# ZKTLabs/zkt-plonk

Measured on AMD Instinct MI355X. Metric: proofs/sec (withdraw, n=2^20), higher is better.
Workload: dtype u32 limbs (256-bit Montgomery); 1 GPU; full prove, WithdrawCircuit INPUTS=8 HEIGHT=64 Poseidon x5 (1019498 gates, 538 Poseidon gadgets), bn254, n=2^20, TABLE_SIZE=1024, 12 public inputs; parallelism=proofs sharded across 1 GPU(s), chained=True, distinct_witnesses=2, witness_on_device=True, table_cached=True, proof_bytes=802

## Files before the change

### include/zkt_plonk.h

```cpp
#ifndef ZKT_PLONK_H
#define ZKT_PLONK_H

#include <stddef.h>
#include <stdint.h>

#ifdef __cplusplus
extern "C" {
#endif

typedef struct zkt_ctx zkt_ctx;

enum {
    ZKT_CURVE_BN254 = 0,
    ZKT_CURVE_BLS12_381 = 1
};

enum {
    ZKT_OK = 0,
    ZKT_ERR_INVALID_ARGUMENT = 1,
    ZKT_ERR_INVALID_DOMAIN_SIZE = 2,
    ZKT_ERR_HIP = 3,
    ZKT_ERR_NO_DEVICE = 4,
    ZKT_ERR_TOO_MANY_COEFFICIENTS = 5,
    ZKT_ERR_ZERO_DENOMINATOR = 6,
// ... 22 lines not shown
    int (*all_gather)(void* user, const void* send, void* recv, size_t bytes, int on_device, void* hip_stream);
    int (*all_gather_async)(void* user, const void* d_send, void* d_recv, size_t bytes, void* hip_stream);
} zkt_comm_vtable;
#define ZKT_QUOTIENT_CHUNKS 4
int zkt_ctx_set_comm(zkt_ctx* ctx, const zkt_comm_vtable* comm);
int zkt_shard_range(size_t total, int rank, int world, size_t* lo, size_t* hi);
int zkt_comm_stats(zkt_ctx* ctx, uint64_t* calls, uint64_t* bytes_sent);
int zkt_comm_selftest(const zkt_comm_vtable* comm, const void* send, void* recv, size_t bytes);

int zkt_dev_alloc(zkt_ctx* ctx, size_t bytes, void** dptr);
int zkt_dev_free(zkt_ctx* ctx, void* dptr);
int zkt_dev_upload(zkt_ctx* ctx, void* dptr, const void* host, size_t bytes);
int zkt_dev_download(zkt_ctx* ctx, void* host, const void* dptr, size_t bytes);

int zkt_ntt(zkt_ctx* ctx, int log_n, int inverse, int coset, const uint64_t* in, size_t in_len, uint64_t* out);
int zkt_ntt_dev(zkt_ctx* ctx, int log_n, int inverse, int coset, const void* d_in, size_t in_len, void* d_out);
int zkt_ntt_class(zkt_ctx* ctx, int log_n, int log_big, int cls, const uint64_t* in, size_t in_len, uint64_t* out);
int zkt_domain_group_gen(zkt_ctx* ctx, int log_n, uint64_t* out4);

int zkt_srs_load(zkt_ctx* ctx, const uint64_t* g1_xy_mont, size_t count);
int zkt_srs_load_dev(zkt_ctx* ctx, const void* d_g1_xy_mont, size_t count);
int zkt_srs_generate(zkt_ctx* ctx, const uint64_t* tau_canonical4, size_t count);
int zkt_srs_download(zkt_ctx* ctx, size_t offset, size_t count, uint64_t* out_xy_mont);
int zkt_srs_generate_g2(int curve_id, const uint64_t* tau_canonical4, uint64_t* out_h, uint64_t* out_beta_h);
int zkt_srs_load_slice(zkt_ctx* ctx, const uint64_t* g1_xy_mont_slice, size_t offset, size_t count, size_t total);
int zkt_srs_generate_slice(zkt_ctx* ctx, const uint64_t* tau_canonical4, size_t offset, size_t count, size_t total);
int zkt_msm_g1(zkt_ctx* ctx, const uint64_t* scalars, size_t len, size_t base_offset, int scalars_montgomery,
               uint64_t* out_xy_mont, int* out_is_infinity);
int zkt_msm_g1_dev(zkt_ctx* ctx, const void* d_scalars, size_t len, size_t base_offset, int scalars_montgomery,
                   void* out_xy_mont_host);
int zkt_msm_enqueue_dev(zkt_ctx* ctx, const void* d_scalars, size_t len, size_t base_offset, int scalars_montgomery);
int zkt_msm_info(zkt_ctx* ctx, int* window_bits, int* windows, size_t* srs_count);

#define ZKT_MSM_BASES_MAX ((size_t)1 << 22)
int zkt_msm_g1_bases(zkt_ctx* ctx, const uint64_t* bases_xy_mont, const uint64_t* scalars, size_t n,
                     int scalars_montgomery, uint64_t* out_xy_mont, int* out_is_infinity);
int zkt_msm_g1_bases_dev(zkt_ctx* ctx, const void* d_bases_xy_mont, const void* d_scalars, size_t n,
                         int scalars_montgomery, uint64_t* out_xy_mont_host, int* out_is_infinity);
int zkt_msm_bases_info(zkt_ctx* ctx, size_t n, int scalars_montgomery, int* window_bits, int* windows);

#define ZKT_KZG_BATCH_MAX 32
int zkt_kzg_commit_batch(zkt_ctx* ctx, const uint64_t* const* coeffs, const size_t* lens, int k,
                         int scalars_montgomery, uint64_t* out_xy_mont, int* out_is_infinity);
int zkt_kzg_commit_batch_dev(zkt_ctx* ctx, const void* const* d_coeffs, const size_t* lens, int k,
                             int scalars_montgomery, uint64_t* out_xy_mont, int* out_is_infinity);
int zkt_kzg_open(zkt_ctx* ctx, const uint64_t* const* coeffs, const size_t* lens, int k,
                 const uint64_t* challenges_mont, const uint64_t* point_mont,
                 uint64_t* out_w_xy_mont, int* out_w_is_infinity, uint64_t* out_evals_mont);
int zkt_kzg_open_dev(zkt_ctx* ctx, const void* const* d_coeffs, const size_t* lens, int k,
                     const uint64_t* challenges_mont, const uint64_t* point_mont,
                     uint64_t* out_w_xy_mont, int* out_w_is_infinity, uint64_t* out_evals_mont);

int zkt_ctx_set_lagrange(zkt_ctx* ctx, int on);
int zkt_lagrange_info(zkt_ctx* ctx, int* log_n, size_t* bases);
int zkt_commit_evals_dev(zkt_ctx* ctx, const void* d_evals, const uint64_t* blinders, int k, int path, uint64_t* out_xy_mont,
                         int* out_is_infinity);

enum {
    ZKT_TRANSCRIPT_MERLIN = 0,
    ZKT_TRANSCRIPT_ETHEREUM = 1
};
typedef struct zkt_transcript zkt_transcript;
zkt_transcript* zkt_transcript_new(int kind, const char* label);
void zkt_transcript_free(zkt_transcript* t);
void zkt_transcript_append_u64(zkt_transcript* t, const char* label, uint64_t v);
void zkt_transcript_append_scalars(zkt_transcript* t, const char* label, const uint8_t* le32, size_t count, int single);
void zkt_transcript_append_commitment(zkt_transcript* t, const char* label, const uint8_t* x_le, const uint8_t* y_le,
                                      size_t fq_bytes, int is_infinity);
void zkt_transcript_challenge_scalar(zkt_transcript* t, const char* label, int fr_bits, uint8_t out_le32[32]);
void zkt_transcript_seed(zkt_transcript* t, uint64_t circuit_size, const uint8_t* xy_le, const uint8_t* is_infinity,
                         size_t fq_bytes);
int zkt_transcript_append_message(zkt_transcript* t, const char* label, const uint8_t* msg, size_t len);
int zkt_transcript_challenge_bytes(zkt_transcript* t, const char* label, uint8_t* out, size_t len);

typedef struct {
    void* user;
    void (*append_u64)(void* user, const char* label, uint64_t v);
    void (*append_scalars)(void* user, const char* label, const uint64_t* fr_mont, size_t count, int single);
    void (*append_commitment)(void* user, const char* label, const uint64_t* g1_xy_mont, int is_infinity);
    void (*challenge_scalar)(void* user, const char* label, uint64_t* fr_mont_out4);
} zkt_transcript_vtable;

int zkt_circuit_load(zkt_ctx* ctx, int log_n, const uint64_t* const* pk_polys, const size_t* pk_lens);

int zkt_circuit_setup(zkt_ctx* ctx, int log_n, const uint64_t* const* evals, const size_t* eval_lens, int evals_on_device,
                      uint64_t* out_commitments, int* out_is_infinity);

int zkt_circuit_sigma_dev(zkt_ctx* ctx, int log_n, const uint32_t* d_w_l, const uint32_t* d_w_r, const uint32_t* d_w_o,
                          size_t n_rows, size_t n_vars, void* const* d_sigma);
int zkt_circuit_setup_wiring(zkt_ctx* ctx, int log_n, const uint64_t* const* evals, const size_t* eval_lens,
                             int evals_on_device, const uint32_t* w_l, const uint32_t* w_r, const uint32_t* w_o,
                             size_t n_rows, size_t n_vars, int wiring_on_device,
                             uint64_t* out_commitments, int* out_is_infinity);

typedef struct {
    const uint64_t* a_evals;
    const uint64_t* b_evals;
    const uint64_t* c_evals;
    size_t n_rows;
    const uint64_t* table;
    size_t table_len;
    const size_t* pi_pos;
    const uint64_t* pi_vals;
    size_t n_pi;
    const uint64_t* blinders;
    int wires_on_device;
// ... 98 lines not shown

int zkt_verify_batch(int curve_id, const zkt_verify_inputs* ins, zkt_transcript* const* transcripts, size_t count,
                     const uint64_t* h_g2_mont, const uint64_t* beta_h_g2_mont, int* accepted);

#define ZKT_G1_DECOMPRESS_MAX ((size_t)1 << 22)
enum {
    ZKT_G1_VALID = 0,
    ZKT_G1_IDENTITY = 1,
    ZKT_G1_NOT_CANONICAL = 2,
    ZKT_G1_BOTH_FLAGS = 3,
    ZKT_G1_NOT_ON_CURVE = 4,
    ZKT_G1_NOT_IN_SUBGROUP = 5
};
int zkt_g1_decompress(zkt_ctx* ctx, const uint8_t* compressed, size_t n, uint64_t* out_xy_mont, uint8_t* out_status);
int zkt_g1_decompress_dev(zkt_ctx* ctx, const void* d_compressed, size_t n, void* d_out_xy_mont, void* d_out_status);

#define ZKT_VERIFY_BATCH_DEV_MAX (ZKT_MSM_BASES_MAX / 24)
int zkt_verify_batch_prepare_dev(zkt_ctx* ctx, const zkt_verify_inputs* ins, zkt_transcript* const* transcripts, size_t count,
                                 const uint64_t* h_g2_mont, const uint64_t* beta_h_g2_mont, uint64_t* out_ab,
                                 int* out_ab_is_infinity, uint64_t* out_rho);
int zkt_verify_batch_dev(zkt_ctx* ctx, const zkt_verify_inputs* ins, zkt_transcript* const* transcripts, size_t count,
                         const uint64_t* h_g2_mont, const uint64_t* beta_h_g2_mont, int* accepted);

int zkt_g1_msm_host(int curve_id, const uint64_t* points_xy_mont, const uint64_t* scalars, size_t n, int scalars_montgomery,
                    uint64_t* out_xy_mont, int* out_is_infinity);

int zkt_keyfile_committer_key(const char* path, int curve_id, size_t max_powers, uint64_t* out_xy_mont, size_t* n_powers);
int zkt_keyfile_prover_key(const char* path, int curve_id, uint64_t* const* out_polys, size_t* lens10);
int zkt_keyfile_verifier_key(const char* path, int curve_id, uint64_t* n, uint64_t* pi_roots_mont, size_t pi_cap, size_t* n_pi,
                             uint64_t* commitments_xy_mont, int* is_infinity10);
#define ZKT_EPK_VECTORS 17
int zkt_keyfile_extended_prover_key(const char* path, int curve_id, int which, uint64_t* out_mont, size_t cap, size_t* lens17);
int zkt_circuit_check_epk_file(zkt_ctx* ctx, const char* epk_path, int* first_mismatch_vector, size_t* mismatch_at);
int zkt_srs_load_file(zkt_ctx* ctx, const char* ck_path, size_t max_powers);
int zkt_circuit_load_file(zkt_ctx* ctx, const char* pk_path, int log_n);

int zkt_debug_params(zkt_ctx* ctx, int which, uint32_t* out, size_t out_words);
int zkt_host_field_op(int curve_id, int which, int op, const uint32_t* a, const uint32_t* b, uint32_t* out);
int zkt_g1_sum_host(int curve_id, const uint64_t* points_xy_mont, size_t count, uint64_t* out_xy_mont, int* out_is_infinity);
int zkt_debug_fr_mul(zkt_ctx* ctx, const uint64_t* a, const uint64_t* b, size_t n, uint64_t* out);
int zkt_debug_ntt_batch(zkt_ctx* ctx, int log_n, int inverse, int coset, int nb, const void* const* d_in, const size_t* in_len,
                        void* const* d_out);
int zkt_debug_ntt_split(zkt_ctx* ctx, int npass, const int* log_r);
int zkt_debug_pairing_selftest(int curve_id);
int zkt_debug_quotient(zkt_ctx* ctx, const uint64_t* challenges, const uint64_t* const* wit, const uint64_t* pi_pos,
                       const uint64_t* pi_vals, size_t n_pi, uint64_t* out);
int zkt_debug_grand_products(zkt_ctx* ctx, const uint64_t* challenges, const uint64_t* const* vectors, uint64_t* out_z1,
                             uint64_t* out_z2);
int zkt_debug_combine_split(zkt_ctx* ctx, const uint64_t* table, size_t table_len, const uint64_t* f, int fresh,
                            uint64_t* h1_out, uint64_t* h2_out);
int zkt_debug_commit_wires_dev(zkt_ctx* ctx, const void* d_variables, size_t n_vars, const uint32_t* d_w_l, const uint32_t* d_w_r,
                               const uint32_t* d_w_o, size_t n_rows, const uint64_t* blinders, int route, uint64_t* out_xy_mont,
                               int* out_is_infinity, int* out_route);
int zkt_debug_open_witness(zkt_ctx* ctx, const uint64_t* coeffs, size_t len, const uint64_t* z4, uint64_t* out);
int zkt_debug_eval_lincomb(zkt_ctx* ctx, const uint64_t* const* polys, const size_t* lens, int k, const uint64_t* points,
                           const uint64_t* scalars, uint64_t* out_evals, uint64_t* out_lincomb, size_t out_len);

enum zkt_fx_op {
    ZKT_FX_UNPACK = 0, ZKT_FX_UNPACK_SHIFT = 1, ZKT_FX_PACK = 2, ZKT_FX_FROM_ARK = 3, ZKT_FX_TO_ARK = 4,
    ZKT_FX_NORMALIZE = 5, ZKT_FX_ADD = 6, ZKT_FX_DBL = 7, ZKT_FX_SUB_1 = 8, ZKT_FX_SUB_2 = 9, ZKT_FX_SUB_4 = 10,
    ZKT_FX_SUB_8 = 11, ZKT_FX_SUB2_6 = 12, ZKT_FX_ADD_LAZY = 13, ZKT_FX_SUB_LAZY_3 = 14, ZKT_FX_SUB_LAZY_4 = 15,
    ZKT_FX_SUB_LAZY_5 = 16, ZKT_FX_SUB_LAZY_9 = 17, ZKT_FX_SUB_LAZY_WIDE_8_30 = 18, ZKT_FX_MUL = 19, ZKT_FX_MUL_INL = 20,
    ZKT_FX_SQR = 21, ZKT_FX_SQR_INL = 22, ZKT_FX_MUL2_INL = 23, ZKT_FX_MUL_SHOUP = 24 ,
    ZKT_FX_MUL_LOW = 25, ZKT_FX_REDUCE_SMALL = 26, ZKT_FX_REDUCE_LAZY = 27 ,
    ZKT_FX_COND_SUB_P = 28, ZKT_FX_CANON = 29, ZKT_FX_IS_ZERO_CANON = 30, ZKT_FX_IS_ZERO_LT2P = 31, ZKT_FX_OP_COUNT = 32
};
enum zkt_xyzz_op {
    ZKT_XYZZ_ADD_MIXED = 0, ZKT_XYZZ_ADD_MIXED_INL = 1, ZKT_XYZZ_ADD = 2, ZKT_XYZZ_ADD_INL = 3, ZKT_XYZZ_DOUBLE = 4,
    ZKT_XYZZ_DOUBLE_AFFINE = 5, ZKT_XYZZ_OP_COUNT = 6
};
int zkt_debug_fx_layout(int curve_id, int which, int* limbs, int* limb_bits, int* sh);
int zkt_host_fx_op(int curve_id, int which, int op, const uint32_t* in, size_t n, uint32_t* out);
int zkt_debug_fx_op(zkt_ctx* ctx, int which, int op, const uint32_t* in, size_t n, uint32_t* out);
int zkt_host_xyzz_op(int curve_id, int op, const uint32_t* in, size_t n, uint32_t* out);
int zkt_debug_xyzz_op(zkt_ctx* ctx, int op, const uint32_t* in, size_t n, uint32_t* out);

#ifdef __cplusplus
}
#endif
#endif
```

### shim/src/ffi.rs

```rust
use std::os::raw::{c_char, c_int, c_void};

#[repr(C)]
pub struct ZktCtx {
    _private: [u8; 0],
}

#[repr(C)]
pub struct ZktTranscriptVtable {
    pub user: *mut c_void,
    pub append_u64: extern "C" fn(*mut c_void, *const c_char, u64),
    pub append_scalars: extern "C" fn(*mut c_void, *const c_char, *const u64, usize, c_int),
    pub append_commitment: extern "C" fn(*mut c_void, *const c_char, *const u64, c_int),
    pub challenge_scalar: extern "C" fn(*mut c_void, *const c_char, *mut u64),
}

#[repr(C)]
pub struct ZktCommVtable {
    pub user: *mut c_void,
    pub rank: c_int,
    pub world: c_int,
    pub device_buffers: c_int,
    pub all_gather: extern "C" fn(*mut c_void, *const c_void, *mut c_void, usize, c_int, *mut c_void) -> c_int,
    pub all_gather_async: Option<extern "C" fn(*mut c_void, *const c_void, *mut c_void, usize, *mut c_void) -> c_int>,
}
// ... 16 lines not shown
    pub w_l: *const u32,
    pub w_r: *const u32,
    pub w_o: *const u32,
}

#[repr(C)]
pub struct ZktWitnessReport {
    pub satisfied: c_int,
    pub checked: c_int,
    pub n_arithmetic: u64,
    pub first_arithmetic: u64,
    pub residual: [u64; 4],
    pub n_lookup: u64,
    pub first_lookup: u64,
    pub n_wiring: u64,
    pub first_wiring_row: u64,
    pub first_wiring_column: c_int,
}

pub const ZKT_CHECK_WIRING: c_int = 1;
pub const ZKT_CHECK_NONE: u64 = u64::MAX;
pub const ZKT_VARIABLE_ZERO: u32 = 0xFFFF_FFFF;
pub const ZKT_CURVE_BN254: c_int = 0;
pub const ZKT_CURVE_BLS12_381: c_int = 1;
pub const ZKT_KZG_BATCH_MAX: usize = 32;

extern "C" {
    pub fn zkt_ctx_create(curve_id: c_int, device_id: c_int, out: *mut *mut ZktCtx) -> c_int;
    pub fn zkt_ctx_destroy(ctx: *mut ZktCtx);
    pub fn zkt_last_error(ctx: *const ZktCtx) -> *const c_char;
    pub fn zkt_ctx_set_comm(ctx: *mut ZktCtx, comm: *const ZktCommVtable) -> c_int;
    pub fn zkt_shard_range(total: usize, rank: c_int, world: c_int, lo: *mut usize, hi: *mut usize) -> c_int;
    pub fn zkt_ntt(ctx: *mut ZktCtx, log_n: c_int, inverse: c_int, coset: c_int, input: *const u64, in_len: usize,
                   out: *mut u64) -> c_int;
    pub fn zkt_srs_load(ctx: *mut ZktCtx, g1_xy_mont: *const u64, count: usize) -> c_int;
    pub fn zkt_srs_load_slice(ctx: *mut ZktCtx, g1_xy_mont: *const u64, offset: usize, count: usize, total: usize) -> c_int;
    pub fn zkt_srs_load_file(ctx: *mut ZktCtx, ck_path: *const c_char, max_powers: usize) -> c_int;
    pub fn zkt_msm_g1(ctx: *mut ZktCtx, scalars: *const u64, len: usize, base_offset: usize, scalars_montgomery: c_int,
                      out_xy_mont: *mut u64, out_is_infinity: *mut c_int) -> c_int;
    pub fn zkt_ctx_fork(ctx: *mut ZktCtx, out: *mut *mut ZktCtx) -> c_int;
    pub fn zkt_kzg_commit_batch(ctx: *mut ZktCtx, coeffs: *const *const u64, lens: *const usize, k: c_int,
                                scalars_montgomery: c_int, out_xy_mont: *mut u64, out_is_infinity: *mut c_int) -> c_int;
    pub fn zkt_kzg_commit_batch_dev(ctx: *mut ZktCtx, d_coeffs: *const *const c_void, lens: *const usize, k: c_int,
                                    scalars_montgomery: c_int, out_xy_mont: *mut u64, out_is_infinity: *mut c_int) -> c_int;
    pub fn zkt_kzg_open(ctx: *mut ZktCtx, coeffs: *const *const u64, lens: *const usize, k: c_int, challenges_mont: *const u64,
                        point_mont: *const u64, out_w_xy_mont: *mut u64, out_w_is_infinity: *mut c_int,
                        out_evals_mont: *mut u64) -> c_int;
    pub fn zkt_kzg_open_dev(ctx: *mut ZktCtx, d_coeffs: *const *const c_void, lens: *const usize, k: c_int,
                            challenges_mont: *const u64, point_mont: *const u64, out_w_xy_mont: *mut u64,
                            out_w_is_infinity: *mut c_int, out_evals_mont: *mut u64) -> c_int;
    pub fn zkt_commit_evals_dev(ctx: *mut ZktCtx, d_evals: *const c_void, blinders: *const u64, k: c_int, path: c_int,
                                out_xy_mont: *mut u64, out_is_infinity: *mut c_int) -> c_int;
    pub fn zkt_ctx_set_lagrange(ctx: *mut ZktCtx, on: c_int) -> c_int;
    pub fn zkt_lagrange_info(ctx: *mut ZktCtx, log_n: *mut c_int, bases: *mut usize) -> c_int;
    pub fn zkt_circuit_load(ctx: *mut ZktCtx, log_n: c_int, pk_polys: *const *const u64, pk_lens: *const usize) -> c_int;
    pub fn zkt_circuit_load_file(ctx: *mut ZktCtx, pk_path: *const c_char, log_n: c_int) -> c_int;
    pub fn zkt_keyfile_extended_prover_key(path: *const c_char, curve_id: c_int, which: c_int, out_mont: *mut u64, cap: usize,
                                           lens17: *mut usize) -> c_int;
    pub fn zkt_circuit_check_epk_file(ctx: *mut ZktCtx, epk_path: *const c_char, first_mismatch_vector: *mut c_int,
                                      mismatch_at: *mut usize) -> c_int;
    pub fn zkt_circuit_setup(ctx: *mut ZktCtx, log_n: c_int, evals: *const *const u64, eval_lens: *const usize,
                             evals_on_device: c_int, out_commitments: *mut u64, out_is_infinity: *mut c_int) -> c_int;
    pub fn zkt_circuit_sigma_dev(ctx: *mut ZktCtx, log_n: c_int, d_w_l: *const u32, d_w_r: *const u32, d_w_o: *const u32,
                                 n_rows: usize, n_vars: usize, d_sigma: *const *mut c_void) -> c_int;
    pub fn zkt_circuit_setup_wiring(ctx: *mut ZktCtx, log_n: c_int, evals: *const *const u64, eval_lens: *const usize,
                                    evals_on_device: c_int, w_l: *const u32, w_r: *const u32, w_o: *const u32, n_rows: usize,
                                    n_vars: usize, wiring_on_device: c_int, out_commitments: *mut u64,
                                    out_is_infinity: *mut c_int) -> c_int;
    pub fn zkt_prove_with(ctx: *mut ZktCtx, inputs: *const ZktProveInputs, transcript: *const ZktTranscriptVtable,
                          proof_out: *mut u8, proof_cap: usize, proof_len: *mut usize) -> c_int;
    pub fn zkt_prove_set_next(ctx: *mut ZktCtx, next: *const ZktProveInputs) -> c_int;
    pub fn zkt_circuit_check_witness(ctx: *mut ZktCtx, inputs: *const ZktProveInputs, flags: c_int,
                                     out: *mut ZktWitnessReport) -> c_int;
    pub fn zkt_g1_msm_host(curve_id: c_int, points_xy_mont: *const u64, scalars: *const u64, n: usize, scalars_montgomery: c_int,
                           out_xy_mont: *mut u64, out_is_infinity: *mut c_int) -> c_int;
    pub fn zkt_msm_g1_bases(ctx: *mut ZktCtx, bases_xy_mont: *const u64, scalars: *const u64, n: usize,
                            scalars_montgomery: c_int, out_xy_mont: *mut u64, out_is_infinity: *mut c_int) -> c_int;
    pub fn zkt_msm_g1_bases_dev(ctx: *mut ZktCtx, d_bases_xy_mont: *const c_void, d_scalars: *const c_void, n: usize,
                                scalars_montgomery: c_int, out_xy_mont_host: *mut u64, out_is_infinity: *mut c_int) -> c_int;
    pub fn zkt_verify(curve_id: c_int, inputs: *const ZktVerifyInputs, transcript: *mut c_void, h_g2_mont: *const u64,
                      beta_h_g2_mont: *const u64, accepted: *mut c_int) -> c_int;
    pub fn zkt_verify_batch(curve_id: c_int, inputs: *const ZktVerifyInputs, transcripts: *const *mut c_void, count: usize,
                            h_g2_mont: *const u64, beta_h_g2_mont: *const u64, accepted: *mut c_int) -> c_int;
    pub fn zkt_verify_batch_prepare_dev(ctx: *mut ZktCtx, inputs: *const ZktVerifyInputs, transcripts: *const *mut c_void, count: usize,
                                        h_g2_mont: *const u64, beta_h_g2_mont: *const u64, out_ab: *mut u64,
                                        out_ab_is_infinity: *mut c_int, out_rho: *mut u64) -> c_int;
    pub fn zkt_verify_batch_dev(ctx: *mut ZktCtx, inputs: *const ZktVerifyInputs, transcripts: *const *mut c_void, count: usize,
                                h_g2_mont: *const u64, beta_h_g2_mont: *const u64, accepted: *mut c_int) -> c_int;
    pub fn zkt_g1_decompress(ctx: *mut ZktCtx, compressed: *const u8, n: usize, out_xy_mont: *mut u64, out_status: *mut u8) -> c_int;
    pub fn zkt_g1_decompress_dev(ctx: *mut ZktCtx, d_compressed: *const c_void, n: usize, d_out_xy_mont: *mut c_void,
                                 d_out_status: *mut c_void) -> c_int;
    pub fn zkt_poseidon_load(ctx: *mut ZktCtx, params: *const ZktPoseidonParams, out: *mut *mut c_void) -> c_int;
    pub fn zkt_poseidon_free(ctx: *mut ZktCtx, params: *mut c_void);
    pub fn zkt_poseidon_hash_batch_dev(ctx: *mut ZktCtx, params: *const c_void, d_inputs: *const c_void, batch: usize,
                                       arity: c_int, d_out_hashes: *mut c_void, d_out_states: *mut c_void) -> c_int;
    pub fn zkt_poseidon_gadget_vars_per_hash(params: *const c_void) -> usize;
    pub fn zkt_poseidon_gadget_witness_dev(ctx: *mut ZktCtx, params: *const c_void, args: *const ZktPoseidonGadgetArgs) -> c_int;
    pub fn zkt_poseidon_gadget_check(ctx: *mut ZktCtx, params: *const c_void) -> c_int;
    pub fn zkt_merkle_path_vars_per_level(params: *const c_void) -> usize;
    pub fn zkt_poseidon_merkle_path_witness_dev(ctx: *mut ZktCtx, params: *const c_void, args: *const ZktMerklePathArgs) -> c_int;
    pub fn zkt_poseidon_merkle_path_validate(ctx: *mut ZktCtx, params: *const c_void, args: *const ZktMerklePathArgs) -> c_int;
    pub fn zkt_dev_alloc(ctx: *mut ZktCtx, bytes: usize, dptr: *mut *mut c_void) -> c_int;
    pub fn zkt_dev_free(ctx: *mut ZktCtx, dptr: *mut c_void) -> c_int;
    pub fn zkt_dev_upload(ctx: *mut ZktCtx, dptr: *mut c_void, host: *const c_void, bytes: usize) -> c_int;
}

// ... 61 lines not shown
```

### zkt-plonk_amd/_lib.py

```python
from __future__ import annotations

import ctypes
import os
import re
from typing import Optional

import numpy as np

_HERE = os.path.dirname(os.path.abspath(__file__))
_LIB = os.environ.get("ZKT_LIB_PATH") or os.path.join(_HERE, "libzkt_plonk_hip.so")
_HEADER = os.path.join(_HERE, "..", "include", "zkt_plonk.h")

MSM_BASES_MAX = 1 << 22
G1_DECOMPRESS_MAX = 1 << 22
VERIFY_BATCH_DEV_MAX = MSM_BASES_MAX // 24
KZG_BATCH_MAX = 32
CURVE_BN254 = 0
CURVE_BLS12_381 = 1
_CURVES = {"bn254": 0, "bls12_381": 1, "bls12-381": 1, 0: 0, 1: 1}

_lib = None


class ZktError(RuntimeError):
# ... 462 lines not shown
def host_fx_op(curve, which: int, op: int, records) -> np.ndarray:
    L_ = fx_layout(curve, which)[0]
    rec = _records(records, 4 * L_)
    out = np.zeros_like(rec)
    rc = lib().zkt_host_fx_op(curve_id(curve), which, op, _u32p(rec), rec.shape[0], _u32p(out))
    if rc:
        raise ZktError(rc, "zkt_host_fx_op")
    return out


def host_xyzz_op(curve, op: int, records) -> np.ndarray:
    w = 4 * fx_layout(curve, 1)[0] + 1
    rec = _records(records, 2 * w)
    out = np.zeros((rec.shape[0], w), dtype=np.uint32)
    rc = lib().zkt_host_xyzz_op(curve_id(curve), op, _u32p(rec), rec.shape[0], _u32p(out))
    if rc:
        raise ZktError(rc, "zkt_host_xyzz_op")
    return out


def srs_generate_g2(curve, tau: int):
    L = lib()
    cid = curve_id(curve)
    words = 8 if cid == CURVE_BN254 else 12
    t = np.array([(int(tau) >> (64 * i)) & 0xFFFFFFFFFFFFFFFF for i in range(4)], dtype=np.uint64)
    h = np.zeros(2 * words, dtype=np.uint64)
    bh = np.zeros(2 * words, dtype=np.uint64)
    P64 = ctypes.POINTER(ctypes.c_uint64)
    L.zkt_srs_generate_g2.argtypes = [ctypes.c_int, P64, P64, P64]
    rc = L.zkt_srs_generate_g2(cid, u64p(t), u64p(h), u64p(bh))
    if rc:
        raise ZktError(rc, "zkt_srs_generate_g2")
    return h, bh


def g1_msm_host(curve, points, scalars, montgomery: bool = True) -> tuple:
    L = lib()
    cid = curve_id(curve)
    words = 8 if cid == CURVE_BN254 else 12
    pts = np.ascontiguousarray(points, dtype=np.uint64).reshape(-1, words)
    sc = np.ascontiguousarray(scalars, dtype=np.uint64).reshape(-1, 4)
    assert pts.shape[0] == sc.shape[0]
    out = np.zeros(words, dtype=np.uint64)
    inf = ctypes.c_int(0)
    P64 = ctypes.POINTER(ctypes.c_uint64)
    L.zkt_g1_msm_host.argtypes = [ctypes.c_int, P64, P64, ctypes.c_size_t, ctypes.c_int, P64, ctypes.POINTER(ctypes.c_int)]
    rc = L.zkt_g1_msm_host(cid, u64p(pts) if pts.size else None, u64p(sc) if sc.size else None, pts.shape[0], int(montgomery),
                           u64p(out), ctypes.byref(inf))
    if rc:
        raise ZktError(rc, "zkt_g1_msm_host")
    return out, bool(inf.value)


class Transcript:

    def __init__(self, kind: str = "merlin", label: str = "ZKT Plonk", fr_bits: int = 254, fq_bytes: int = 32):
        self._L = lib()
        self._h = ctypes.c_void_p(self._L.zkt_transcript_new(0 if kind == "merlin" else 1, label.encode()))
        self.fr_bits = fr_bits
        self.fq_bytes = fq_bytes

    def __del__(self):
        if getattr(self, "_h", None):
            self._L.zkt_transcript_free(self._h)
            self._h = None

    @property
    def handle(self):
        return self._h

    def append_u64(self, label: str, v: int):
        self._L.zkt_transcript_append_u64(self._h, label.encode(), v)

    def append_scalar(self, label: str, v: int):
        self._L.zkt_transcript_append_scalars(self._h, label.encode(), int(v).to_bytes(32, "little"), 1, 1)

    def append_scalars(self, label: str, vals):
        vals = list(vals)
        self._L.zkt_transcript_append_scalars(self._h, label.encode(),
                                              b"".join(int(v).to_bytes(32, "little") for v in vals), len(vals), 0)

    def append_commitment(self, label: str, point):
        nb = self.fq_bytes
        if point is None:
            self._L.zkt_transcript_append_commitment(self._h, label.encode(), bytes(nb), bytes(nb), nb, 1)
        else:
            self._L.zkt_transcript_append_commitment(self._h, label.encode(), int(point[0]).to_bytes(nb, "little"),
                                                     int(point[1]).to_bytes(nb, "little"), nb, 0)

    def seed(self, circuit_size: int, points):
        nb = self.fq_bytes
        buf = b"".join(bytes(2 * nb) if p is None else int(p[0]).to_bytes(nb, "little") + int(p[1]).to_bytes(nb, "little")
                       for p in points)
        inf = bytes(1 if p is None else 0 for p in points)
        self._L.zkt_transcript_seed(self._h, circuit_size, buf, inf, nb)

    def challenge_scalar(self, label: str) -> int:
        out = (ctypes.c_uint8 * 32)()
        self._L.zkt_transcript_challenge_scalar(self._h, label.encode(), self.fr_bits, out)
        return int.from_bytes(bytes(out), "little")

    def append_message(self, label: bytes, msg: bytes):
        assert self._L.zkt_transcript_append_message(self._h, label, msg, len(msg)) == 0

    def challenge_bytes(self, label: bytes, n: int) -> bytes:
        out = (ctypes.c_uint8 * n)()
# ... 327 lines not shown
    @staticmethod
    def _kzg_lens(lens):
        return (ctypes.c_size_t * max(len(lens), 1))(*[int(n) for n in lens])

    def _kzg_points(self, out, inf, k):
        W = 2 * self.fq_limbs
        return [(out[j * W:(j + 1) * W].copy(), bool(inf[j])) for j in range(k)]

    def kzg_commit_batch(self, polys, montgomery: bool = True):
        arrs, ptrs, lens = self._kzg_polys(polys)
        k = len(arrs)
        out = np.zeros(max(k, 1) * 2 * self.fq_limbs, dtype=np.uint64)
        inf = (ctypes.c_int * max(k, 1))()
        self.check(self._L.zkt_kzg_commit_batch(self._h, ptrs, lens, k, int(montgomery), u64p(out), inf))
        return self._kzg_points(out, inf, k)

    def kzg_commit_batch_dev(self, d_ptrs, lens, montgomery: bool = True):
        k = len(lens)
        ptrs = (ctypes.c_void_p * max(k, 1))(*[int(d) if d else None for d in d_ptrs])
        out = np.zeros(max(k, 1) * 2 * self.fq_limbs, dtype=np.uint64)
        inf = (ctypes.c_int * max(k, 1))()
        self.check(self._L.zkt_kzg_commit_batch_dev(self._h, ptrs, self._kzg_lens(lens), k, int(montgomery), u64p(out), inf))
        return self._kzg_points(out, inf, k)

    def _kzg_open_call(self, fn, ptrs, lens, k, challenges, z, evals):
        ch = np.ascontiguousarray(challenges, dtype=np.uint64).reshape(-1, 4)
        if ch.shape[0] != k:
            raise ValueError("kzg_open: %d polynomials, %d challenges" % (k, ch.shape[0]))
        zz = np.ascontiguousarray(z, dtype=np.uint64).reshape(4)
        w = np.zeros(2 * self.fq_limbs, dtype=np.uint64)
        inf = ctypes.c_int(0)
        ev = np.zeros((max(k, 1), 4), dtype=np.uint64)
        self.check(fn(self._h, ptrs, lens, k, u64p(ch) if k else None, u64p(zz), u64p(w), ctypes.byref(inf),
                      u64p(ev) if evals else None))
        return (w, bool(inf.value)), (ev[:k].copy() if evals else None)

    def kzg_open(self, polys, challenges, z, evals: bool = True):
        arrs, ptrs, lens = self._kzg_polys(polys)
        return self._kzg_open_call(self._L.zkt_kzg_open, ptrs, lens, len(arrs), challenges, z, evals)

    def kzg_open_dev(self, d_ptrs, lens, challenges, z, evals: bool = True):
        k = len(lens)
        ptrs = (ctypes.c_void_p * max(k, 1))(*[int(d) if d else None for d in d_ptrs])
        return self._kzg_open_call(self._L.zkt_kzg_open_dev, ptrs, self._kzg_lens(lens), k, challenges, z, evals)

    def msm_info(self):
        c, w, n = ctypes.c_int(0), ctypes.c_int(0), ctypes.c_size_t(0)
        self.check(self._L.zkt_msm_info(self._h, ctypes.byref(c), ctypes.byref(w), ctypes.byref(n)))
        return dict(window_bits=c.value, windows=w.value, srs_count=n.value)

    def set_lagrange(self, on: bool = True):
        self._L.zkt_ctx_set_lagrange.argtypes = [ctypes.c_void_p, ctypes.c_int]
        self.check(self._L.zkt_ctx_set_lagrange(self._h, int(on)))

    def lagrange_info(self):
        self._L.zkt_lagrange_info.argtypes = [ctypes.c_void_p, ctypes.POINTER(ctypes.c_int), ctypes.POINTER(ctypes.c_size_t)]
        lg, nb = ctypes.c_int(0), ctypes.c_size_t(0)
        self.check(self._L.zkt_lagrange_info(self._h, ctypes.byref(lg), ctypes.byref(nb)))
        return dict(log_n=lg.value, bases=nb.value)

    def commit_evals_dev(self, d_evals: int, blinders=None, path: int = 1):
        self._L.zkt_commit_evals_dev.argtypes = [ctypes.c_void_p, ctypes.c_void_p, ctypes.POINTER(ctypes.c_uint64), ctypes.c_int,
                                                 ctypes.c_int, ctypes.POINTER(ctypes.c_uint64), ctypes.POINTER(ctypes.c_int)]
        k = 0 if blinders is None else int(np.asarray(blinders).reshape(-1, 4).shape[0])
        bl = np.ascontiguousarray(blinders, dtype=np.uint64).reshape(-1, 4) if k else None
        out = np.zeros(2 * self.fq_limbs, dtype=np.uint64)
        inf = ctypes.c_int(0)
        self.check(self._L.zkt_commit_evals_dev(self._h, ctypes.c_void_p(d_evals), u64p(bl) if k else None, k, int(path),
                                                u64p(out), ctypes.byref(inf)))
        return out, bool(inf.value)

    def circuit_load(self, log_n: int, pk_polys):
        arrs = [np.ascontiguousarray(p, dtype=np.uint64).reshape(-1, 4) for p in pk_polys]
        assert len(arrs) == 10
        ptrs = (ctypes.POINTER(ctypes.c_uint64) * 10)(*[u64p(a) if a.size else ctypes.POINTER(ctypes.c_uint64)() for a in arrs])
        lens = (ctypes.c_size_t * 10)(*[a.shape[0] for a in arrs])
        self.check(self._L.zkt_circuit_load(self._h, log_n, ptrs, lens))
        self.circuit_log_n = log_n

    def circuit_setup(self, log_n: int, evals):
        arrs = [np.ascontiguousarray(p, dtype=np.uint64).reshape(-1, 4) for p in evals]
        assert len(arrs) == 10
        ptrs = (ctypes.POINTER(ctypes.c_uint64) * 10)(*[u64p(a) if a.size else ctypes.POINTER(ctypes.c_uint64)() for a in arrs])
        lens = (ctypes.c_size_t * 10)(*[a.shape[0] for a in arrs])
        out = np.zeros((10, 2 * self.fq_limbs), dtype=np.uint64)
        inf = (ctypes.c_int * 10)()
        self.check(self._L.zkt_circuit_setup(self._h, log_n, ptrs, lens, 0, u64p(out), inf))
        self.circuit_log_n = log_n
        return out, np.array([bool(x) for x in inf])

    def circuit_sigma(self, log_n: int, d_w_l: int, d_w_r: int, d_w_o: int, n_rows: int, n_vars: int, d_sigma=None):
        n = 1 << log_n if 0 <= log_n <= 25 else 0
        own = d_sigma is None
        if own:
            d_sigma = [self.alloc(max(n, 1) * 32) for _ in range(3)]
        try:
            ptrs = (ctypes.c_void_p * 3)(*d_sigma)
            self.check(self._L.zkt_circuit_sigma_dev(self._h, log_n, ctypes.c_void_p(d_w_l), ctypes.c_void_p(d_w_r),
                                                     ctypes.c_void_p(d_w_o), n_rows, n_vars, ptrs))
            return [self.download(p, (n, 4)) for p in d_sigma] if own else None
        finally:
            if own:
                for p in d_sigma:
                    self.free(p)

    def circuit_setup_wiring(self, log_n: int, evals, w_l, w_r, w_o, n_vars: int, n_rows: int = None):
# ... 96 lines not shown
        lens = (ctypes.c_size_t * len(in_len))(*in_len)
        self.check(self._L.zkt_debug_ntt_batch(self._h, log_n, int(inverse), int(coset), nb, ins, lens, outs))

    def debug_ntt_split(self, log_r=()):
        lr = (ctypes.c_int * max(len(log_r), 3))(*log_r)
        self.check(self._L.zkt_debug_ntt_split(self._h, len(log_r), lr))

    def debug_fr_mul(self, a: np.ndarray, b: np.ndarray) -> np.ndarray:
        a = np.ascontiguousarray(a, dtype=np.uint64).reshape(-1, 4)
        b = np.ascontiguousarray(b, dtype=np.uint64).reshape(-1, 4)
        out = np.empty_like(a)
        self.check(self._L.zkt_debug_fr_mul(self._h, u64p(a), u64p(b), a.shape[0], u64p(out)))
        return out

    def debug_fx_op(self, which: int, op: int, records) -> np.ndarray:
        L_ = fx_layout(self.curve, which)[0]
        rec = _records(records, 4 * L_)
        out = np.zeros_like(rec)
        self.check(self._L.zkt_debug_fx_op(self._h, which, op, _u32p(rec), rec.shape[0], _u32p(out)))
        return out

    def debug_xyzz_op(self, op: int, records) -> np.ndarray:
        w = 4 * fx_layout(self.curve, 1)[0] + 1
        rec = _records(records, 2 * w)
        out = np.zeros((rec.shape[0], w), dtype=np.uint32)
        self.check(self._L.zkt_debug_xyzz_op(self._h, op, _u32p(rec), rec.shape[0], _u32p(out)))
        return out

    def debug_grand_products(self, n: int, challenges, vectors):
        ch = np.ascontiguousarray(challenges, dtype=np.uint64).reshape(4, 4)
        keep = [np.ascontiguousarray(w, dtype=np.uint64).reshape(n, 4) for w in vectors]
        assert len(keep) == 7
        ptrs = (ctypes.c_void_p * 7)(*[w.ctypes.data for w in keep])
        z1, z2 = np.empty((n, 4), dtype=np.uint64), np.empty((n, 4), dtype=np.uint64)
        self._L.zkt_debug_grand_products.argtypes = [ctypes.c_void_p, ctypes.POINTER(ctypes.c_uint64), ctypes.POINTER(ctypes.c_void_p),
                                                     ctypes.POINTER(ctypes.c_uint64), ctypes.POINTER(ctypes.c_uint64)]
        self.check(self._L.zkt_debug_grand_products(self._h, u64p(ch), ptrs, u64p(z1), u64p(z2)))
        return z1, z2

    def debug_combine_split(self, table, f, fresh: bool = True):
        t = np.ascontiguousarray(table, dtype=np.uint64).reshape(-1, 4)
        ff = np.ascontiguousarray(f, dtype=np.uint64).reshape(-1, 4)
        if self.circuit_log_n is None or ff.shape[0] != 1 << self.circuit_log_n:
            raise ValueError("f must hold the n elements of a circuit loaded through this Context")
        n = ff.shape[0]
        h1, h2 = np.empty((n, 4), dtype=np.uint64), np.empty((n, 4), dtype=np.uint64)
        P64 = ctypes.POINTER(ctypes.c_uint64)
        self._L.zkt_debug_combine_split.argtypes = [ctypes.c_void_p, P64, ctypes.c_size_t, P64, ctypes.c_int, P64, P64]
        self.check(self._L.zkt_debug_combine_split(self._h, u64p(t) if t.shape[0] else None, t.shape[0], u64p(ff),
                                                   1 if fresh else 0, u64p(h1), u64p(h2)))
        return h1, h2

    def debug_commit_wires_dev(self, d_variables: int, n_vars: int, d_w_l: int, d_w_r: int, d_w_o: int, n_rows: int, blinders,
                               route: int = 1):
        bl = np.ascontiguousarray(blinders, dtype=np.uint64).reshape(6, 4)
        out = np.zeros((3, 2 * self.fq_limbs), dtype=np.uint64)
        inf = (ctypes.c_int * 3)()
        took = (ctypes.c_int * 3)()
        self._L.zkt_debug_commit_wires_dev.argtypes = [ctypes.c_void_p, ctypes.c_void_p, ctypes.c_size_t, ctypes.c_void_p,
                                                       ctypes.c_void_p, ctypes.c_void_p, ctypes.c_size_t,
                                                       ctypes.POINTER(ctypes.c_uint64), ctypes.c_int,
                                                       ctypes.POINTER(ctypes.c_uint64), ctypes.POINTER(ctypes.c_int),
                                                       ctypes.POINTER(ctypes.c_int)]
        self.check(self._L.zkt_debug_commit_wires_dev(self._h, ctypes.c_void_p(d_variables), n_vars, ctypes.c_void_p(d_w_l),
                                                      ctypes.c_void_p(d_w_r), ctypes.c_void_p(d_w_o), n_rows, u64p(bl), int(route),
                                                      u64p(out), inf, took))
        return out, [bool(x) for x in inf], [int(x) for x in took]

    def check_epk_file(self, path: str):
        self._L.zkt_circuit_check_epk_file.argtypes = [ctypes.c_void_p, ctypes.c_char_p, ctypes.POINTER(ctypes.c_int),
                                                       ctypes.POINTER(ctypes.c_size_t)]
        vec, at = ctypes.c_int(0), ctypes.c_size_t(0)
        self.check(self._L.zkt_circuit_check_epk_file(self._h, path.encode(), ctypes.byref(vec), ctypes.byref(at)))
        if vec.value < 0:
            return None
        return vec.value, (-1 if at.value == ctypes.c_size_t(-1).value else at.value)

    def debug_eval_lincomb(self, polys, points, scalars, out_len: int):
        keep = [np.ascontiguousarray(p_, dtype=np.uint64).reshape(-1, 4) for p_ in polys]
        k = len(keep)
        P64 = ctypes.POINTER(ctypes.c_uint64)
        ptrs = (P64 * k)(*[u64p(a) for a in keep])
        lens = (ctypes.c_size_t * k)(*[a.shape[0] for a in keep])
        pts = np.ascontiguousarray(points, dtype=np.uint64).reshape(k, 4)
        scs = np.ascontiguousarray(scalars, dtype=np.uint64).reshape(k, 4)
        ev = np.empty((k, 4), dtype=np.uint64)
        lc = np.empty((out_len, 4), dtype=np.uint64)
        self._L.zkt_debug_eval_lincomb.argtypes = [ctypes.c_void_p, ctypes.POINTER(P64), ctypes.POINTER(ctypes.c_size_t), ctypes.c_int,
                                                   P64, P64, P64, P64, ctypes.c_size_t]
        self.check(self._L.zkt_debug_eval_lincomb(self._h, ptrs, lens, k, u64p(pts), u64p(scs), u64p(ev), u64p(lc), out_len))
        return ev, lc

    def debug_open_witness(self, coeffs, z) -> np.ndarray:
        p_ = np.ascontiguousarray(coeffs, dtype=np.uint64).reshape(-1, 4)
        zz = np.ascontiguousarray(z, dtype=np.uint64).reshape(4)
        out = np.empty((p_.shape[0] - 1, 4), dtype=np.uint64)
        self._L.zkt_debug_open_witness.argtypes = [ctypes.c_void_p, ctypes.POINTER(ctypes.c_uint64), ctypes.c_size_t,
                                                   ctypes.POINTER(ctypes.c_uint64), ctypes.POINTER(ctypes.c_uint64)]
        self.check(self._L.zkt_debug_open_witness(self._h, u64p(p_), p_.shape[0], u64p(zz), u64p(out)))
        return out

    def debug_quotient(self, n: int, challenges, wit, pi_pos=(), pi_vals=None) -> np.ndarray:
        ch = np.ascontiguousarray(challenges, dtype=np.uint64).reshape(5, 4)
        keep = [None if w is None else np.ascontiguousarray(w, dtype=np.uint64).reshape(4 * n, 4) for w in wit]
        assert len(keep) == 9
        ptrs = (ctypes.c_void_p * 9)(*[None if w is None else w.ctypes.data for w in keep])
        pos = np.ascontiguousarray(list(pi_pos), dtype=np.uint64)
        vals = np.ascontiguousarray(pi_vals if len(pos) else np.zeros((0, 4)), dtype=np.uint64).reshape(-1, 4)
        out = np.empty((4 * n, 4), dtype=np.uint64)
        self.check(self._L.zkt_debug_quotient(self._h, u64p(ch), ptrs, u64p(pos) if len(pos) else None,
                                              u64p(vals) if len(pos) else None, len(pos), u64p(out)))
# ... 2 lines not shown
```

### zkt-plonk_amd/csrc/capi.hip

```cpp
#include "ctx.hpp"

#include <cstdlib>
#include "hostinv.hpp"
#include "ec.hpp"
#include "hostec.hpp"
#include "fx_test.hpp"
#include "msm.hpp"

#include <cstring>

namespace zkt {

const char* exp_env(const char* name) {
#ifdef ZKT_EXPERIMENTS
    return getenv(name);
#else
    (void)name;
    return nullptr;
#endif
}

int set_err(zkt_ctx* c, int code, const std::string& msg) {
    if (c) c->err = msg;
    return code;
// ... 149 lines not shown

template <class P>
static int dump_params(uint32_t* out, size_t words) {
    const int N = P::N;
    if (words < (size_t)(3 * N + 1)) return -1;
    for (int i = 0; i < N; ++i) out[i] = P::mod(i);
    out[N] = P::INV;
    for (int i = 0; i < N; ++i) out[N + 1 + i] = P::one(i);
    for (int i = 0; i < N; ++i) out[2 * N + 1 + i] = P::r2(i);
    return N;
}

}

using namespace zkt;

extern "C" {

const char* zkt_version(void) { return "zkt-plonk_amd 0.1 (gfx950)"; }

int zkt_ctx_create(int curve_id, int device_id, zkt_ctx** out) {
    if (!out) return ZKT_ERR_INVALID_ARGUMENT;
    *out = nullptr;
    if (curve_id != ZKT_CURVE_BN254 && curve_id != ZKT_CURVE_BLS12_381) return ZKT_ERR_INVALID_ARGUMENT;
    int count = 0;
    if (hipGetDeviceCount(&count) != hipSuccess || count <= 0 || device_id < 0 || device_id >= count)
        return ZKT_ERR_NO_DEVICE;
    if (hipSetDevice(device_id) != hipSuccess) return ZKT_ERR_NO_DEVICE;
    zkt_ctx* c = new zkt_ctx();
    c->batch_off = exp_env("ZKT_MSM_NO_BATCH") != nullptr;
    c->aux_off = exp_env("ZKT_NO_AUX") != nullptr;
    c->curve = curve_id;
    c->device = device_id;
    if (hipStreamCreateWithFlags(&c->stream, hipStreamNonBlocking) != hipSuccess) {
        delete c;
        return ZKT_ERR_HIP;
    }
    c->own_stream = true;
    *out = c;
    return ZKT_OK;
}

int zkt_ctx_fork(zkt_ctx* parent, zkt_ctx** out) {
    if (!parent || !out) return ZKT_ERR_INVALID_ARGUMENT;
    *out = nullptr;
    if (parent->sharded()) return set_err(parent, ZKT_ERR_INVALID_ARGUMENT, "zkt_ctx_fork: not for a context with a communicator");
    if (parent->zombie) return set_err(parent, ZKT_ERR_INVALID_ARGUMENT, "zkt_ctx_fork: the context has been destroyed");
    zkt_ctx* root = parent->parent ? parent->parent : parent;
    zkt_ctx* c = nullptr;
    int rc = zkt_ctx_create(parent->curve, parent->device, &c);
    if (rc) return rc;
    (void)hipStreamSynchronize(parent->stream);
    c->lagrange_off = parent->lagrange_off;
    c->batch_off = parent->batch_off;
    c->aux_off = parent->aux_off;
    c->ntt_plans = parent->ntt_plans;
    c->parent = root;
    root->forks.fetch_add(1);
    if ((rc = msm_fork(c, parent)) || (rc = circuit_fork(c, parent))) {
        parent->err = c->err;
        zkt_ctx_destroy(c);
        return rc;
    }
    *out = c;
    return ZKT_OK;
}

void zkt_ctx_destroy(zkt_ctx* c) {
    if (!c) return;
    (void)hipSetDevice(c->device);
    (void)hipStreamSynchronize(c->stream);
    if (c->forks.load() > 0) {
        c->zombie = true;
        return;
    }
    zkt_ctx* const owner = c->parent;
    circuit_release(c);
    msm_release(c);
    prof_resolve(c);
    for (hipEvent_t e : c->event_pool) (void)hipEventDestroy(e);
    c->event_pool.clear();
    c->ntt_plans.clear();
    c->msm.reset();
    c->msmb.reset();
    c->kzg.reset();
    c->circuit.reset();
    if (c->comm.pinned) (void)hipHostFree(c->comm.pinned);
    for (void* p : c->owned) (void)hipFree(p);
    c->owned.clear();
    if (c->own_stream && c->stream) (void)hipStreamDestroy(c->stream);
    delete c;
    if (owner && owner->forks.fetch_sub(1) == 1 && owner->zombie) {
        owner->zombie = false;
        zkt_ctx_destroy(owner);
    }
}

int zkt_ctx_set_comm(zkt_ctx* c, const zkt_comm_vtable* comm) {
    if (!c) return ZKT_ERR_INVALID_ARGUMENT;
    if (int rf = refuse_if_forked(c, "zkt_ctx_set_comm")) return rf;
    if (c->parent && comm && comm->world > 1) return set_err(c, ZKT_ERR_INVALID_ARGUMENT, "a forked context cannot take a communicator");
    if (comm && comm->world > 1) {
        const int w = comm->world;
        if ((w != 2 && w != 4 && w != 8) || comm->rank < 0 || comm->rank >= w || !comm->all_gather)
            return set_err(c, ZKT_ERR_INVALID_ARGUMENT, "communicator: world must be 1, 2, 4 or 8 with a valid rank and callback");
    }
// ... 372 lines not shown
```

### zkt-plonk_amd/csrc/check.hip

```cpp
#include "poly.hpp"

#include <algorithm>
#include <cstring>
#include <numeric>
#include <vector>

namespace zkt {

constexpr int CK_THREADS = 256;
constexpr int CK_ROWS_PER_THREAD = 4;
constexpr unsigned CK_MAX_BLOCKS = 2048;
constexpr uint32_t CK_NONE32 = 0xFFFFFFFFu;
enum { CK_N_ARITH = 0, CK_FIRST_ARITH, CK_N_LOOKUP, CK_FIRST_LOOKUP, CK_N_WIRING, CK_FIRST_WIRING, CK_BAD_INDEX, CK_PAD, CK_RESIDUAL,
       CK_WORDS = CK_RESIDUAL + 4 };

struct CheckArgs {
    const void *q_m, *q_l, *q_r, *q_o, *q_c, *q_lookup;
    const void *a, *b, *c;
    const void* variables;
    const uint32_t *w_l, *w_r, *w_o;
    uint32_t n, n_rows, n_vars;
    const uint32_t* pi_pos;
    const void* pi_vals;
    uint32_t n_pi;
// ... 94 lines not shown
                while (lo < hi) {
                    const uint32_t mid = lo + (hi - lo) / 2;
                    if (ck_cmp<P>(fe_load<P>(tab + mid), f) < 0) lo = mid + 1;
                    else hi = mid;
                }
                if (lo >= q.table_len || ck_cmp<P>(fe_load<P>(tab + lo), f) != 0) {
                    ++n_lookup;
                    first_lookup = i < first_lookup ? i : first_lookup;
                }
            }
        }
    }
    ck_block_reduce(n_arith, first_arith, q.status + CK_N_ARITH, q.status + CK_FIRST_ARITH, sh_cnt, sh_min);
    ck_block_reduce(n_lookup, first_lookup, q.status + CK_N_LOOKUP, q.status + CK_FIRST_LOOKUP, sh_cnt, sh_min);
}

template <class P, bool VARS>
__global__ void k_check_residual(CheckArgs q) {
    if (blockIdx.x || threadIdx.x) return;
    const unsigned long long first = q.status[CK_FIRST_ARITH];
    if (first >= q.n) return;
    const uint32_t i = (uint32_t)first;
    const Fe<P> t = ck_gate<P>(q, i, ck_wire<P, VARS>(q, q.a, q.w_l, i), ck_wire<P, VARS>(q, q.b, q.w_r, i),
                               ck_wire<P, VARS>(q, q.c, q.w_o, i));
#pragma unroll
    for (int k = 0; k < 4; ++k) q.status[CK_RESIDUAL + k] = (unsigned long long)t.v[2 * k] | ((unsigned long long)t.v[2 * k + 1] << 32);
}

template <class P>
__global__ __launch_bounds__(CK_THREADS) void k_check_sigma(const Fe<P>* m0, const Fe<P>* m1, const Fe<P>* m2, const Fe<P>* k0,
                                                            const Fe<P>* k1, const Fe<P>* k2, uint32_t n, unsigned long long* status) {
    __shared__ uint32_t sh_cnt[CK_THREADS / 64], sh_min[CK_THREADS / 64];
    const Fe<P>* const made[3] = {m0, m1, m2};
    const Fe<P>* const key[3] = {k0, k1, k2};
    uint32_t cnt = 0, first = CK_NONE32;
    const uint32_t stride = gridDim.x * CK_THREADS;
#pragma unroll 1
    for (uint32_t g = blockIdx.x * CK_THREADS + threadIdx.x; g < n; g += stride) {
#pragma unroll
        for (uint32_t col = 0; col < 3; ++col) {
            if (!fe_eq<P>(fe_load<P>(made[col] + g), fe_load<P>(key[col] + g))) {
                ++cnt;
                const uint32_t p = 3 * g + col;
                first = p < first ? p : first;
            }
        }
    }
    ck_block_reduce(cnt, first, status + CK_N_WIRING, status + CK_FIRST_WIRING, sh_cnt, sh_min);
}

static unsigned ck_blocks(size_t n) {
    const size_t per = (size_t)CK_THREADS * CK_ROWS_PER_THREAD;
    return (unsigned)std::min<size_t>(std::max<size_t>((n + per - 1) / per, 1), CK_MAX_BLOCKS);
}

template <class P>
static int witness_check_t(zkt_ctx* c, const WitnessCheckKeys& K, const zkt_prove_inputs& in, int flags, zkt_witness_report* out) {
    using F = Fe<P>;
    static_assert(sizeof(F) == 32, "scalar field element = 8 words");
    const int log_n = K.log_n;
    const size_t n = (size_t)1 << log_n;
    const bool vars = in.a_evals == nullptr;
    const bool wiring = (flags & ZKT_CHECK_WIRING) != 0;
    const bool on_device = in.wires_on_device != 0;
    const size_t rows = in.n_rows, n_pi = in.n_pi, tl = in.table_len;

    std::vector<F> sorted(tl);
    if (tl) {
        const F* t = reinterpret_cast<const F*>(in.table);
        std::vector<uint32_t> order(tl);
        std::iota(order.begin(), order.end(), 0u);
        std::sort(order.begin(), order.end(), [&](uint32_t x, uint32_t y) { return ck_cmp<P>(t[x], t[y]) < 0; });
        for (size_t i = 0; i < tl; ++i) sorted[i] = t[order[i]];
        for (size_t i = 1; i < tl; ++i)
            if (ck_cmp<P>(sorted[i - 1], sorted[i]) == 0)
                return set_err(c, ZKT_ERR_INVALID_ARGUMENT, "lookup table holds a repeated value");
    }
    std::vector<uint32_t> pos(n_pi);
    std::vector<F> pvals(n_pi);
    if (n_pi) {
        std::vector<uint32_t> order(n_pi);
        std::iota(order.begin(), order.end(), 0u);
        std::stable_sort(order.begin(), order.end(), [&](uint32_t x, uint32_t y) { return in.pi_pos[x] < in.pi_pos[y]; });
        for (size_t i = 0; i < n_pi; ++i) {
            pos[i] = (uint32_t)in.pi_pos[order[i]];
            pvals[i] = reinterpret_cast<const F*>(in.pi_vals)[order[i]];
        }
    }

    size_t at = 0;
    auto take = [&](size_t bytes) {
        const size_t here = at;
        at += (bytes + 255) / 256 * 256;
        return here;
    };
    const size_t o_status = take(CK_WORDS * 8);
    size_t o_sel[5];
    for (size_t& o : o_sel) o = take(n * 32);
    const size_t o_pos = take(n_pi * 4), o_pvals = take(n_pi * 32), o_table = take(tl * 32);
    size_t o_wit[3] = {}, o_vars = 0, o_idx[3] = {};
    if (!on_device) {
        if (vars) {
            o_vars = take(in.n_vars * 32);
            for (size_t& o : o_idx) o = take(rows * 4);
        } else {
            for (size_t& o : o_wit) o = take(rows * 32);
// ... 7 lines not shown
    int rc = ensure_buffer(c, &c->check_scratch, &c->check_scratch_bytes, at);
    if (rc) return rc;
    char* const base = (char*)c->check_scratch;
    unsigned long long* const d_status = (unsigned long long*)(base + o_status);

    unsigned long long h_status[CK_WORDS] = {};
    struct Drain {
        zkt_ctx* c;
        bool done = false;
        ~Drain() {
            if (!done) (void)hipStreamSynchronize(c->stream);
        }
    } drain{c};
    h_status[CK_FIRST_ARITH] = h_status[CK_FIRST_LOOKUP] = h_status[CK_FIRST_WIRING] = ~0ull;
    ZKT_HIP(c, hipMemcpyAsync(d_status, h_status, sizeof(h_status), hipMemcpyHostToDevice, c->stream));
    if (n_pi) {
        ZKT_HIP(c, hipMemcpyAsync(base + o_pos, pos.data(), n_pi * 4, hipMemcpyHostToDevice, c->stream));
        ZKT_HIP(c, hipMemcpyAsync(base + o_pvals, pvals.data(), n_pi * 32, hipMemcpyHostToDevice, c->stream));
    }
    if (tl) ZKT_HIP(c, hipMemcpyAsync(base + o_table, sorted.data(), tl * 32, hipMemcpyHostToDevice, c->stream));

    CheckArgs q{};
    q.a = in.a_evals; q.b = in.b_evals; q.c = in.c_evals;
    q.variables = in.variables;
    q.w_l = in.w_l; q.w_r = in.w_r; q.w_o = in.w_o;
    if (!on_device) {
        if (vars) {
            if (in.n_vars) ZKT_HIP(c, hipMemcpyAsync(base + o_vars, in.variables, in.n_vars * 32, hipMemcpyHostToDevice, c->stream));
            q.variables = base + o_vars;
            const uint32_t* src[3] = {in.w_l, in.w_r, in.w_o};
            const uint32_t** dst[3] = {&q.w_l, &q.w_r, &q.w_o};
            for (int k = 0; k < 3; ++k) {
                if (rows) ZKT_HIP(c, hipMemcpyAsync(base + o_idx[k], src[k], rows * 4, hipMemcpyHostToDevice, c->stream));
                *dst[k] = (const uint32_t*)(base + o_idx[k]);
            }
        } else {
            const uint64_t* src[3] = {in.a_evals, in.b_evals, in.c_evals};
            const void** dst[3] = {&q.a, &q.b, &q.c};
            for (int k = 0; k < 3; ++k) {
                if (rows) ZKT_HIP(c, hipMemcpyAsync(base + o_wit[k], src[k], rows * 32, hipMemcpyHostToDevice, c->stream));
                *dst[k] = base + o_wit[k];
            }
        }
    }
    q.q_m = base + o_sel[0]; q.q_l = base + o_sel[1]; q.q_r = base + o_sel[2]; q.q_o = base + o_sel[3]; q.q_c = base + o_sel[4];
    q.q_lookup = K.q_lookup_ev;
    q.n = (uint32_t)n; q.n_rows = (uint32_t)rows; q.n_vars = (uint32_t)in.n_vars;
    q.pi_pos = (const uint32_t*)(base + o_pos); q.pi_vals = base + o_pvals; q.n_pi = (uint32_t)n_pi;
    q.table = base + o_table; q.table_len = (uint32_t)tl;
    q.status = d_status;

    {
        ProfScope prof(c, "check_witness");
        const void* ins[5];
        void* outs[5];
        size_t lens[5];
        for (int k = 0; k < 5; ++k) {
            ins[k] = K.pk[k];
            lens[k] = n;
            outs[k] = base + o_sel[k];
        }
        static_assert(NTT_MAX_BATCH >= 4, "four selectors in one batch");
        if ((rc = ntt_run_batch(c, log_n, 0, 0, 4, ins, lens, outs))) return rc;
        if ((rc = ntt_run_batch(c, log_n, 0, 0, 1, ins + 4, lens + 4, outs + 4))) return rc;

        if (vars) {
            hipLaunchKernelGGL((k_check_gates<P, true>), dim3(ck_blocks(n)), dim3(CK_THREADS), 0, c->stream, q);
            hipLaunchKernelGGL((k_check_residual<P, true>), dim3(1), dim3(64), 0, c->stream, q);
        } else {
            hipLaunchKernelGGL((k_check_gates<P, false>), dim3(ck_blocks(n)), dim3(CK_THREADS), 0, c->stream, q);
            hipLaunchKernelGGL((k_check_residual<P, false>), dim3(1), dim3(64), 0, c->stream, q);
        }
        ZKT_HIP(c, hipGetLastError());
        if (wiring) {
            void* made[3] = {base + o_made[0], base + o_made[1], base + o_made[2]};
            if ((rc = sigma_enqueue(c, log_n, q.w_l, q.w_r, q.w_o, rows, in.n_vars, made, base + o_sigma,
                                    (uint32_t*)(d_status + CK_BAD_INDEX))))
                return rc;
            hipLaunchKernelGGL(k_check_sigma<P>, dim3(ck_blocks(n)), dim3(CK_THREADS), 0, c->stream, (const F*)made[0], (const F*)made[1],
                               (const F*)made[2], (const F*)K.sigma_ev[0], (const F*)K.sigma_ev[1], (const F*)K.sigma_ev[2], (uint32_t)n,
                               d_status);
            ZKT_HIP(c, hipGetLastError());
        }
    }
    ZKT_HIP(c, hipMemcpyAsync(h_status, d_status, sizeof(h_status), hipMemcpyDeviceToHost, c->stream));
    ZKT_HIP(c, hipStreamSynchronize(c->stream));
    drain.done = true;
    if (h_status[CK_BAD_INDEX])
        return set_err(c, ZKT_ERR_INVALID_ARGUMENT, "wire index outside the variable map: every entry must be < n_vars or ZKT_VARIABLE_ZERO");

    zkt_witness_report r;
    memset(&r, 0, sizeof(r));
    r.checked = 3 | (wiring ? 4 : 0);
    r.n_arithmetic = h_status[CK_N_ARITH];
    r.first_arithmetic = h_status[CK_FIRST_ARITH];
    for (int k = 0; k < 4; ++k) r.residual[k] = h_status[CK_RESIDUAL + k];
    r.n_lookup = h_status[CK_N_LOOKUP];
    r.first_lookup = h_status[CK_FIRST_LOOKUP];
    r.n_wiring = h_status[CK_N_WIRING];
    r.first_wiring_row = ZKT_CHECK_NONE;
    r.first_wiring_column = -1;
    if (h_status[CK_FIRST_WIRING] != ~0ull) {
        r.first_wiring_row = h_status[CK_FIRST_WIRING] / 3;
        r.first_wiring_column = (int)(h_status[CK_FIRST_WIRING] % 3);
    }
    r.satisfied = !r.n_arithmetic && !r.n_lookup && !r.n_wiring;
    memcpy(out, &r, sizeof(r));
    return ZKT_OK;
}

int witness_check(zkt_ctx* c, const WitnessCheckKeys& keys, const zkt_prove_inputs& in, int flags, zkt_witness_report* out) {
    return c->curve == ZKT_CURVE_BN254 ? witness_check_t<Bn254Fr>(c, keys, in, flags, out)
                                       : witness_check_t<Bls381Fr>(c, keys, in, flags, out);
}

}
```

### zkt-plonk_amd/csrc/ctx.hpp

```cpp
#pragma once
#include <hip/hip_runtime.h>
#include <stdint.h>
#include <stddef.h>
#include <map>
#include <string>
#include <tuple>
#include <vector>
#include <memory>
#include <atomic>

#include "../../include/zkt_plonk.h"
#include "fp.hpp"
#include "fx.hpp"
#include "ntt.hpp"

namespace zkt {

struct MsmState;
struct MsmBasesState;
struct KzgState;
struct CircuitState;

}

struct zkt_ctx {
    int curve = 0;
    int device = 0;
    hipStream_t stream = nullptr;
    bool own_stream = false;
    std::string err;

    std::map<std::tuple<int, int, int, int>, std::shared_ptr<void>> ntt_plans;
    int ntt_split_npass = 0;
    int ntt_split_log_r[3] = {0, 0, 0};
    void* ntt_scratch = nullptr;
    size_t ntt_scratch_bytes = 0;
    void* io_a = nullptr;
    size_t io_a_bytes = 0;
    void* io_b = nullptr;
    size_t io_b_bytes = 0;
    void* check_scratch = nullptr;
    size_t check_scratch_bytes = 0;
    void* verify_scratch = nullptr;
    size_t verify_scratch_bytes = 0;

    int prof_on = 0;
    struct ProfSlot {
        std::vector<std::pair<hipEvent_t, hipEvent_t>> pending;
        double total_ms = 0.0;
        uint64_t calls = 0;
        uint64_t launches = 0;
    };
    std::map<std::string, ProfSlot> prof;
    std::vector<hipEvent_t> event_pool;

    struct Comm {
        zkt_comm_vtable vt{};
        void* pinned = nullptr;
        size_t pinned_bytes = 0;
        uint64_t calls = 0, bytes = 0;
    } comm;
    bool sharded() const { return comm.vt.world > 1; }

    std::shared_ptr<zkt::MsmState> msm;
    std::shared_ptr<zkt::MsmBasesState> msmb;
    std::shared_ptr<zkt::KzgState> kzg;
    uint64_t msm_epoch = 0;
    uint64_t srs_generation = 0;
    zkt_ctx* parent = nullptr;
    std::atomic<int> forks{0};
    bool zombie = false;
    bool aux_off = false;
    bool batch_off = false;
    bool lagrange_off = false;
    std::shared_ptr<zkt::CircuitState> circuit;
    std::vector<void*> owned;
};

namespace zkt {

const char* exp_env(const char* name);

int set_err(zkt_ctx* c, int code, const std::string& msg);
int refuse_if_forked(zkt_ctx* c, const char* what);
int hip_fail(zkt_ctx* c, hipError_t e, const char* what);

#define ZKT_HIP(c, call)                                        \
    do {                                                        \
        hipError_t _e = (call);                                 \
        if (_e != hipSuccess) return zkt::hip_fail((c), _e, #call); \
    } while (0)

struct ProfScope {
    zkt_ctx* c;
    zkt_ctx::ProfSlot* slot = nullptr;
    hipEvent_t e0 = nullptr, e1 = nullptr;
    hipStream_t stream = nullptr;
    uint64_t count = 1;
    ProfScope(zkt_ctx* ctx, const char* name, hipStream_t on_stream = nullptr, uint64_t units = 1);
    ~ProfScope();
};

int comm_all_gather_host(zkt_ctx* c, const void* send, void* recv, size_t bytes);
int comm_all_gather_dev(zkt_ctx* c, const void* d_send, void* d_recv, size_t bytes);
bool comm_async_available(const zkt_ctx* c);
int comm_all_gather_async(zkt_ctx* c, const void* d_send, void* d_recv, size_t bytes, hipStream_t st);

int ensure_buffer(zkt_ctx* c, void** p, size_t* cur, size_t bytes);
struct DevBuf {
    void* p = nullptr;
    size_t bytes = 0;
};
inline int grow(zkt_ctx* c, DevBuf& b, size_t bytes) { return ensure_buffer(c, &b.p, &b.bytes, bytes); }
int dev_alloc(zkt_ctx* c, void** p, size_t bytes);
void dev_free(zkt_ctx* c, void* p);

template <class P>
Fe<P> root_of_unity(int log_n);
int ntt_run(zkt_ctx* c, int log_n, int inverse, int coset, const void* d_in, size_t in_len, void* d_out);
int ntt_run_batch(zkt_ctx* c, int log_n, int inverse, int coset, int nb, const void* const* d_in, const size_t* in_len,
                  void* const* d_out);
int ntt_class_code(int log_big, int cls);
int ntt_force_split(zkt_ctx* c, int npass, const int* log_r);
int ntt_run_class(zkt_ctx* c, int log_n, int log_big, int cls, const void* d_in, size_t in_len, void* d_out, void* d_fold);

void circuit_release(zkt_ctx* c);
int circuit_fork(zkt_ctx* child, const zkt_ctx* parent);
// ... 3 lines not shown
```

### zkt-plonk_amd/csrc/lagrange.hip

```cpp
#include "ctx.hpp"
#include "ec.hpp"
#include "hostec.hpp"
#include "msm.hpp"

#include <algorithm>
#include <cstdio>
#include <cstdlib>
#include <vector>

namespace zkt {

template <class C>
__global__ void k_lag_init(const Affine<typename C::Fq>* table, Xyzz<typename C::Fq>* A, size_t n) {
    using Q = typename C::Fq;
    const size_t j = (size_t)blockIdx.x * blockDim.x + threadIdx.x;
    if (j >= n) return;
    Affine<Q> p = aff_load<Q>(table + j);
    if (!aff_is_inf<Q>(p)) {
        p.x = fx_to_ark<Q>(fx_unpack<Q>(p.x));
        p.y = fx_to_ark<Q>(fx_unpack<Q>(p.y));
    }
    xyzz_store<Q>(A + j, xyzz_from_affine<Q>(p));
}

template <class R>
__global__ void k_lag_twiddles(Fe<R>* tw, size_t half, Fe<R> w) {
    const size_t j = (size_t)blockIdx.x * blockDim.x + threadIdx.x;
    if (j >= half) return;
    fe_store<R>(tw + j, fe_from_mont<R>(fe_pow_u64<R>(w, (uint64_t)j)));
}

template <class Q>
ZKT_HD Xyzz<Q> xyzz_neg(const Xyzz<Q>& p) {
    Xyzz<Q> r = p;
    r.y = fe_neg<Q>(p.y);
    return r;
}

template <class Q, class R>
ZKT_D Xyzz<Q> xyzz_scalar_mul(const Xyzz<Q>& P, const Fe<R>& k) {
    constexpr int N = R::N;
    uint32_t h[N + 1];
    uint32_t carry = 0;
#pragma unroll
    for (int i = 0; i < N; ++i) {
        const uint64_t t = (uint64_t)k.v[i] * 3u + carry;
        h[i] = (uint32_t)t;
        carry = (uint32_t)(t >> 32);
    }
    h[N] = carry;
    const Xyzz<Q> Pn = xyzz_neg<Q>(P);
    Xyzz<Q> acc = xyzz_identity<Q>();
#pragma unroll 1
    for (int li = N; li >= 0; --li) {
        const uint32_t hw = h[li], kw = li < N ? k.v[li] : 0u;
        if (li == N && hw == 0u) continue;
#pragma unroll 1
        for (int b = (li == N ? 1 : 31); b >= (li == 0 ? 1 : 0); --b) {
            acc = xyzz_double<Q>(acc);
// ... 202 lines not shown
        const Affine<Q> hi = wire_load_base<Q>(pre + i);
        if (!aff_is_inf<Q>(hi)) acc = xyzz_add_mixed<Q>(acc, hi);
        if (i) {
            Affine<Q> lo = wire_load_base<Q>(pre + i - 1);
            if (!aff_is_inf<Q>(lo)) {
                lo.y = fe_neg<Q>(lo.y);
                acc = xyzz_add_mixed<Q>(acc, lo);
            }
        }
    }
    if (xyzz_is_identity<Q>(acc)) atomicOr(bad, 1u);
    aff_store<Q>(out + j, xyzz_to_affine<Q>(acc));
}
template <class C>
__global__ void k_wire_blinder_points(const Affine<typename C::Fq>* pre, size_t n, size_t cnt, Affine<typename C::Fq>* out) {
    using Q = typename C::Fq;
    if (threadIdx.x < 2) aff_store<Q>(out + cnt + threadIdx.x, wire_load_base<Q>(pre + n + threadIdx.x));
}

ZKT_HD uint64_t wire_mix(uint64_t x) {
    x ^= x >> 30; x *= 0xbf58476d1ce4e5b9ull;
    x ^= x >> 27; x *= 0x94d049bb133111ebull;
    return x ^ (x >> 31);
}
__global__ __launch_bounds__(256) void k_wire_digest(const uint32_t* w0, const uint32_t* w1, const uint32_t* w2, size_t rows,
                                                     unsigned long long* out) {
    __shared__ unsigned long long sh[2][256];
    unsigned long long a = 0, b = 0;
    const size_t total = 3 * rows;
    for (size_t e = (size_t)blockIdx.x * blockDim.x + threadIdx.x; e < total; e += (size_t)gridDim.x * blockDim.x) {
        const size_t k = e / rows, i = e - k * rows;
        const uint32_t v = (k == 0 ? w0 : k == 1 ? w1 : w2)[i];
        const uint64_t x = ((uint64_t)e << 32) | v;
        a += wire_mix(x + 0x9e3779b97f4a7c15ull);
        b += wire_mix(~x * 0xd6e8feb86659fd93ull);
    }
    sh[0][threadIdx.x] = a;
    sh[1][threadIdx.x] = b;
    __syncthreads();
    for (unsigned s = 128; s; s >>= 1) {
        if (threadIdx.x < s) {
            sh[0][threadIdx.x] += sh[0][threadIdx.x + s];
            sh[1][threadIdx.x] += sh[1][threadIdx.x + s];
        }
        __syncthreads();
    }
    if (threadIdx.x == 0) {
        atomicAdd(out, sh[0][0]);
        atomicAdd(out + 1, sh[1][0]);
    }
}

template <class P>
__global__ void k_wire_scalars(const Fe<P>* vars, const uint32_t* u, size_t cnt, const Fe<P>* bl, Fe<P> ninv, Fe<P>* out) {
    const size_t j = (size_t)blockIdx.x * blockDim.x + threadIdx.x;
    if (j >= cnt + 2) return;
    fe_store<P>(out + j, j < cnt ? fe_mul<P>(fe_load<P>(vars + u[j]), ninv) : fe_load<P>(bl + (j - cnt)));
}

void wire_bases_drop(zkt_ctx* c) {
    if (!c->msm) return;
    WireBases& wb = c->msm->wb;
    if (!wb.borrowed && wb.built) {
        (void)hipStreamSynchronize(c->stream);
        for (int k = 0; k < 3; ++k) {
            dev_free(c, wb.table[k]);
            dev_free(c, wb.u[k]);
        }
    }
    wb = WireBases{};
}

static int wire_digest_enqueue(zkt_ctx* c, const uint32_t* const* d_idx, size_t n_rows) {
    MsmState& st = *c->msm;
    if (!st.wb_dig)
        if (int rc = dev_alloc(c, (void**)&st.wb_dig, 16)) return rc;
    if (!st.wb_pin) ZKT_HIP(c, hipHostMalloc((void**)&st.wb_pin, 64));
    ZKT_HIP(c, hipMemsetAsync(st.wb_dig, 0, 16, c->stream));
    if (n_rows) {
        const size_t blocks = std::min<size_t>((3 * n_rows + 2047) / 2048, 4096);
        hipLaunchKernelGGL(k_wire_digest, dim3((unsigned)blocks), dim3(256), 0, c->stream, d_idx[0], d_idx[1], d_idx[2], n_rows,
                           (unsigned long long*)st.wb_dig);
        ZKT_HIP(c, hipGetLastError());
    }
    ZKT_HIP(c, hipMemcpyAsync(st.wb_pin, st.wb_dig, 16, hipMemcpyDeviceToHost, c->stream));
    return ZKT_OK;
}

template <class C>
static int wire_bases_build_wire(zkt_ctx* c, int log_n, int k, const uint32_t* d_idx, size_t n_rows, size_t n_vars, double frac) {
    using Q = typename C::Fq;
    MsmState& st = *c->msm;
    WireBases& wb = st.wb;
    const size_t n = (size_t)1 << log_n;
    void *d_cnt = nullptr, *d_start = nullptr, *d_grouped = nullptr, *d_ofs = nullptr, *d_bad = nullptr, *table = nullptr, *d_u = nullptr;
    auto done = [&](bool keep) {
        dev_free(c, d_cnt); dev_free(c, d_start); dev_free(c, d_grouped); dev_free(c, d_ofs); dev_free(c, d_bad);
        if (!keep) { dev_free(c, table); dev_free(c, d_u); }
        (void)hipGetLastError();
        return ZKT_OK;
    };
    if (dev_alloc(c, &d_cnt, (n_vars + 1) * 4)) return done(false);
    ZKT_HIP(c, hipMemsetAsync(d_cnt, 0, (n_vars + 1) * 4, c->stream));
    const unsigned rb = (unsigned)((n_rows + 255) / 256);
    if (n_rows) hipLaunchKernelGGL(k_wire_count, dim3(rb), dim3(256), 0, c->stream, d_idx, n_rows, (uint32_t)n_vars, (uint32_t*)d_cnt);
    std::vector<uint32_t> cnt(n_vars + 1);
    if (hipMemcpyAsync(cnt.data(), d_cnt, n_vars * 4, hipMemcpyDeviceToHost, c->stream) != hipSuccess ||
        hipStreamSynchronize(c->stream) != hipSuccess)
        return done(false);
    std::vector<uint32_t> u, ofs;
    uint32_t at = 0;
    for (size_t v = 0; v < n_vars; ++v) {
        const uint32_t m = cnt[v];
        cnt[v] = at;
        if (m) {
            u.push_back((uint32_t)v);
            ofs.push_back(at);
            at += m;
        }
    }
    ofs.push_back(at);
    const size_t d = u.size();
    if ((double)d >= frac * (double)n_rows || (uint64_t)st.plan.W * (d + 2) >= ((uint64_t)1 << 31)) return done(false);
    if (dev_alloc(c, &table, (size_t)st.plan.W * (d + 2) * sizeof(Affine<Q>)) || dev_alloc(c, &d_u, (d + 1) * 4) ||
        dev_alloc(c, &d_start, (n_vars + 1) * 4) || dev_alloc(c, &d_grouped, ((size_t)at + 1) * 4) || dev_alloc(c, &d_ofs, (d + 1) * 4) ||
        dev_alloc(c, &d_bad, 4))
        return done(false);
    ZKT_HIP(c, hipMemcpyAsync(d_start, cnt.data(), n_vars * 4, hipMemcpyHostToDevice, c->stream));
    ZKT_HIP(c, hipMemcpyAsync(d_u, u.data(), d * 4, hipMemcpyHostToDevice, c->stream));
    ZKT_HIP(c, hipMemcpyAsync(d_ofs, ofs.data(), (d + 1) * 4, hipMemcpyHostToDevice, c->stream));
    ZKT_HIP(c, hipMemsetAsync(d_cnt, 0, (n_vars + 1) * 4, c->stream));
    ZKT_HIP(c, hipMemsetAsync(d_bad, 0, 4, c->stream));
    if (n_rows)
        hipLaunchKernelGGL(k_wire_fill, dim3(rb), dim3(256), 0, c->stream, d_idx, n_rows, (uint32_t)n_vars, (const uint32_t*)d_start,
                           (uint32_t*)d_cnt, (uint32_t*)d_grouped);
    if (d)
        hipLaunchKernelGGL(k_wire_sum<C>, dim3((unsigned)((d + 63) / 64)), dim3(64), 0, c->stream, (const Affine<Q>*)st.table2,
                           (const uint32_t*)d_grouped, (const uint32_t*)d_ofs, d, (Affine<Q>*)table, (uint32_t*)d_bad);
    hipLaunchKernelGGL(k_wire_blinder_points<C>, dim3(1), dim3(64), 0, c->stream, (const Affine<Q>*)st.table2, n, d, (Affine<Q>*)table);
    uint32_t bad = 0;
    if (hipGetLastError() != hipSuccess || hipMemcpyAsync(&bad, d_bad, 4, hipMemcpyDeviceToHost, c->stream) != hipSuccess ||
        hipStreamSynchronize(c->stream) != hipSuccess)
        return done(false);
    if (bad || msm_table_finish(c, table, d + 2)) return done(false);
    wb.table[k] = table;
    wb.u[k] = (uint32_t*)d_u;
    wb.cnt[k] = d;
    wb.use[k] = true;
    return done(true);
}

int wire_bases_prepare(zkt_ctx* c, int log_n, const uint32_t* const* d_idx, size_t n_rows, size_t n_vars) {
    if (!c->msm) return ZKT_OK;
    MsmState& st = *c->msm;
    WireBases& wb = st.wb;
    const size_t n = (size_t)1 << log_n;
    const bool possible = lagrange_ready(c, log_n) && !c->sharded() && !c->lagrange_off && st.count2 >= n + 2 && n_rows <= n &&
                          n_vars <= 0xFFFFFFFEull && !(exp_env("ZKT_WIRE_BASES") && atoi(exp_env("ZKT_WIRE_BASES")) == 0);
    const bool same = wb.built && !wb.stale && wb.w[0] == d_idx[0] && wb.w[1] == d_idx[1] && wb.w[2] == d_idx[2] &&
                      wb.n_rows == n_rows && wb.n_vars == n_vars && wb.log_n == log_n && wb.srs_generation == c->srs_generation;
    if (possible && same) return ZKT_OK;
    if (wb.built && !wb.borrowed && c->forks.load() > 0) {
        if (!same || !possible) wb.stale = true;
        return ZKT_OK;
    }
    wire_bases_drop(c);
    if (!possible) return ZKT_OK;
    double frac = WIRE_BASES_MAX_FRAC;
    if (const char* e = exp_env("ZKT_WIRE_BASES_FRAC")) frac = atof(e);
    hipEvent_t e0 = nullptr, e1 = nullptr;
    const bool trace = exp_env("ZKT_HOST_TRACE") != nullptr;
    if (trace) {
        (void)hipEventCreate(&e0); (void)hipEventCreate(&e1);
        (void)hipEventRecord(e0, c->stream);
    }
    for (int k = 0; k < 3; ++k) {
        const int rc = c->curve == ZKT_CURVE_BN254 ? wire_bases_build_wire<Bn254Curve>(c, log_n, k, d_idx[k], n_rows, n_vars, frac)
                                                    : wire_bases_build_wire<Bls381Curve>(c, log_n, k, d_idx[k], n_rows, n_vars, frac);
        if (rc) return rc;
    }
    if (int rc = wire_digest_enqueue(c, d_idx, n_rows)) return rc;
    ZKT_HIP(c, hipStreamSynchronize(c->stream));
    if (trace) {
        float ms = 0;
        (void)hipEventRecord(e1, c->stream); (void)hipEventSynchronize(e1); (void)hipEventElapsedTime(&ms, e0, e1);
        fprintf(stderr, "[zkt host] wire base tables: %zu / %zu / %zu distinct of %zu rows (0 = dense), %.1f ms\n",
                wb.use[0] ? wb.cnt[0] : 0, wb.use[1] ? wb.cnt[1] : 0, wb.use[2] ? wb.cnt[2] : 0, n_rows, ms);
        (void)hipEventDestroy(e0); (void)hipEventDestroy(e1);
    }
    wb.digest[0] = st.wb_pin[0];
    wb.digest[1] = st.wb_pin[1];
    for (int k = 0; k < 3; ++k) wb.w[k] = d_idx[k];
    wb.n_rows = n_rows; wb.n_vars = n_vars; wb.log_n = log_n; wb.srs_generation = c->srs_generation;
    wb.built = true;
    ++c->msm_epoch;
    return ZKT_OK;
}

bool wire_bases_use(const zkt_ctx* c, int k) {
    return c->msm && c->msm->wb.built && !c->msm->wb.stale && c->msm->wb.use[k];
}
int wire_bases_digest(zkt_ctx* c, const uint32_t* const* d_idx, size_t n_rows) { return wire_digest_enqueue(c, d_idx, n_rows); }
int wire_bases_lens(zkt_ctx* c, const uint32_t* d_lens) {
    ZKT_HIP(c, hipMemcpyAsync(c->msm->wb_pin + 2, d_lens, 12, hipMemcpyDeviceToHost, c->stream));
    return ZKT_OK;
}

template <class C>
static int wire_scalars_t(zkt_ctx* c, int k, const void* d_vars, const void* d_bl, size_t n, const void** out, size_t* len) {
    using R = typename C::Fr;
    MsmState& st = *c->msm;
    const size_t cnt = st.wb.cnt[k];
    if (int rc = grow(c, st.wb_scalars[k], (cnt + 2) * sizeof(Fe<R>))) return rc;
    Fe<R> nn = fe_zero<R>();
    nn.v[0] = (uint32_t)(n & 0xffffffffu);
    nn.v[1] = (uint32_t)((uint64_t)n >> 32);
    const Fe<R> ninv = fe_inv_host<R>(fe_to_mont<R>(nn));
    hipLaunchKernelGGL(k_wire_scalars<R>, dim3((unsigned)((cnt + 2 + 255) / 256)), dim3(256), 0, c->stream, (const Fe<R>*)d_vars,
                       (const uint32_t*)st.wb.u[k], cnt, (const Fe<R>*)d_bl, ninv, (Fe<R>*)st.wb_scalars[k].p);
    ZKT_HIP(c, hipGetLastError());
    *out = st.wb_scalars[k].p;
    *len = cnt + 2;
    return ZKT_OK;
}
int wire_bases_scalars(zkt_ctx* c, int k, const void* d_vars, const void* d_blinders, size_t n, const void** out, size_t* len) {
    if (c->curve == ZKT_CURVE_BN254) return wire_scalars_t<Bn254Curve>(c, k, d_vars, d_blinders, n, out, len);
    return wire_scalars_t<Bls381Curve>(c, k, d_vars, d_blinders, n, out, len);
}

bool wire_bases_check(zkt_ctx* c, int k, size_t n) {
    MsmState& st = *c->msm;
    if (st.wb_pin[0] != st.wb.digest[0] || st.wb_pin[1] != st.wb.digest[1]) {
        st.wb.stale = true;
        return false;
    }
    return ((const uint32_t*)(st.wb_pin + 2))[k] == (uint32_t)n;
}

}
```

### zkt-plonk_amd/csrc/msm.hpp

```cpp
#pragma once
#include "ctx.hpp"

#include <functional>

namespace zkt {

constexpr int MSM_CHUNK_MIN = 16;
constexpr int MSM_R2_BLOCKS = 1;
constexpr int MSM_MAX_Y = 24;

struct MsmWindows {
    int W;
    uint8_t width[40];
    uint16_t start[40];
};

struct MsmPlan {
    MsmWindows win{};
    int W = 0, c = 0;
    int dig = 0;
    uint32_t Bw = 0;
    uint32_t keys = 0;
    uint32_t lb = 8;
    int lcols = 8;
    bool packed = false;
    uint32_t nb1 = 0;
    uint32_t l1_scalars = 0;
    uint32_t l2_items = 0;
};

constexpr int MSM_BATCH = 3;
struct MsmBatch {
    const void* scalars[MSM_BATCH];
    uint64_t n[MSM_BATCH];
    uint64_t base_off[MSM_BATCH];
    const void* table[MSM_BATCH];
    uint64_t tcount[MSM_BATCH];
    uint32_t* heavy[MSM_BATCH];
    uint32_t* params[MSM_BATCH];
    uint32_t* offsets[MSM_BATCH];
    void* pieces[MSM_BATCH];
    uint64_t s_bin_offs, s_bin_aux, s_bin, s_tile_desc, s_cnt, s_pairs_bytes, s_vals, s_chunk;
    uint32_t vb_stride;
};

constexpr int MSM_TAIL_BATCH = 6;
struct MsmTailBatch {
    const uint32_t* offsets[MSM_TAIL_BATCH];
    const uint32_t* params[MSM_TAIL_BATCH];
    const void* pieces[MSM_TAIL_BATCH];
    void* buckets[MSM_TAIL_BATCH];
    uint32_t* heavy[MSM_TAIL_BATCH];
    void* rowcol[MSM_TAIL_BATCH];
    void* partials[MSM_TAIL_BATCH];
};

constexpr int MSM_HEAVY = 32;
constexpr int MSM_HEAVY_BLOCKS = 64;

struct WireBases {
    void* table[3] = {};
    uint32_t* u[3] = {};
    size_t cnt[3] = {};
    bool use[3] = {};
    bool built = false;
    bool borrowed = false;
    bool stale = false;
    const void* w[3] = {};
    size_t n_rows = 0, n_vars = 0;
    int log_n = -1;
    uint64_t srs_generation = 0;
    uint64_t digest[2] = {};
};
constexpr int MSM_TBL_WIRE = 2;

struct MsmState {
    size_t count = 0;
    size_t slice_off = 0, total = 0;
    MsmPlan plan;
    uint32_t* heavy[11] = {};
    void* table = nullptr;
    void* table2 = nullptr;
    size_t count2 = 0;
    int lag_log_n = -1;
    bool lag_failed = false;
    bool table_borrowed = false, table2_borrowed = false;
    WireBases wb;
    DevBuf wb_scalars[3];
    uint64_t* wb_dig = nullptr;
    uint64_t* wb_pin = nullptr;
    const void* tbl_table(int tbl) const { return tbl >= MSM_TBL_WIRE ? wb.table[tbl - MSM_TBL_WIRE] : tbl ? table2 : table; }
    size_t tbl_count(int tbl) const { return tbl >= MSM_TBL_WIRE ? wb.cnt[tbl - MSM_TBL_WIRE] + 2 : tbl ? count2 : count; }
    uint32_t* params[11] = {};
    uint32_t* vals2 = nullptr;
    void* pairs = nullptr;
    uint32_t* bin_offs = nullptr;
    uint32_t* bin_aux = nullptr;
    uint32_t *bin_start = nullptr, *tile_start = nullptr;
    void* tile_desc = nullptr;
    uint32_t *cnt2 = nullptr, *pos2 = nullptr;
    uint32_t* chunk_bucket = nullptr;
    MsmBatch strides{};
    uint32_t* offsets[11] = {};
    void* pieces[11] = {};
    static constexpr int SLOTS = 11;
    void* buckets[SLOTS] = {};
    void* rowcol[SLOTS] = {};
    void* host_result[SLOTS] = {};
    void* host_result_dev[SLOTS] = {};
    size_t acc_lds = 0;
    size_t acc_threads = 196608;
    hipStream_t side = nullptr;
    hipEvent_t ev_main[SLOTS] = {}, ev_done[SLOTS] = {};
    bool pending[SLOTS] = {};
    bool defer_tails = false;
    int tail_wait[SLOTS] = {};
    int n_tail_wait = 0;
    ~MsmState() {
        for (int i = 0; i < SLOTS; ++i) {
            if (host_result[i]) (void)hipHostFree(host_result[i]);
            if (ev_main[i]) (void)hipEventDestroy(ev_main[i]);
            if (ev_done[i]) (void)hipEventDestroy(ev_done[i]);
        }
        if (side) (void)hipStreamDestroy(side);
        if (wb_pin) (void)hipHostFree(wb_pin);
    }
};

struct MsmBasesState {
    DevBuf bases;
    DevBuf scalars;
    DevBuf vals, pairs, bin_offs, bin_aux, bin_start, tile_start, tile_desc, cnt2, pos2, chunk_bucket;
    DevBuf offsets, heavy, params, pieces, buckets, rowcol;
    void* partials = nullptr;
    void* partials_dev = nullptr;
    size_t acc_lds = 0, acc_threads = 0;
    ~MsmBasesState() {
        if (partials) (void)hipHostFree(partials);
    }
};

constexpr size_t MSM_DEFER_MAX = ((size_t)1 << 16) + 64;
constexpr size_t MSM_TAIL_INL_MAX = ((size_t)1 << 18) + 64;

int srs_load(zkt_ctx* c, const void* src, size_t count, bool on_device, size_t slice_off = 0, size_t total = 0);
int srs_generate(zkt_ctx* c, const uint64_t* tau4, size_t count, size_t slice_off = 0, size_t total = 0);
void msm_release(zkt_ctx* c);
int msm_table_finish(zkt_ctx* c, void* table, size_t count);
int msm_fork(zkt_ctx* child, const zkt_ctx* parent);
void msm_slice(zkt_ctx* c, size_t* off, size_t* count, size_t* total);
int msm_g1_dev(zkt_ctx* c, const void* d_scalars, size_t n, size_t base_off, int mont, uint64_t* out_xy, int* out_inf);
int msm_bases(zkt_ctx* c, const void* bases, bool bases_on_device, const void* scalars, bool scalars_on_device, size_t n, int mont,
              uint64_t* out_xy, int* out_inf);
int msm_begin(zkt_ctx* c, const void* d_scalars, size_t n, size_t base_off, int mont, int slot, int tbl = 0);
int msm_begin_batch(zkt_ctx* c, int k, const void* const* d_scalars, const size_t* ns, int mont, const int* slots, const int* tbls);
int msm_begin_many(zkt_ctx* c, int k, const void* const* d_scalars, const size_t* ns, int mont, const int* slots, const int* tbls,
                   bool grouped, const std::function<int(int)>& ready = {});
int msm_end(zkt_ctx* c, int slot, uint64_t* out_xy);
int msm_end_sharded(zkt_ctx* c, const int* slots, const bool* have, int k, uint64_t* out_xy );
int msm_flush_tails(zkt_ctx* c);
bool msm_defers_tails(const zkt_ctx* c);
bool msm_batches_grouping(const zkt_ctx* c);

int lagrange_ensure(zkt_ctx* c, int log_n);
bool lagrange_ready(const zkt_ctx* c, int log_n);
size_t lagrange_bases(const zkt_ctx* c);
int wire_bases_prepare(zkt_ctx* c, int log_n, const uint32_t* const* d_idx, size_t n_rows, size_t n_vars);
bool wire_bases_use(const zkt_ctx* c, int k);
int wire_bases_digest(zkt_ctx* c, const uint32_t* const* d_idx, size_t n_rows);
int wire_bases_lens(zkt_ctx* c, const uint32_t* d_lens);
int wire_bases_scalars(zkt_ctx* c, int k, const void* d_vars, const void* d_blinders, size_t n, const void** out, size_t* len);
bool wire_bases_check(zkt_ctx* c, int k, size_t n);
void wire_bases_drop(zkt_ctx* c);

}
```

### zkt-plonk_amd/csrc/poly.hpp

```cpp
#pragma once
#include "ctx.hpp"

namespace zkt {

constexpr int LC_MAX_TERMS = 16;
struct LinCombArgs {
    const void* poly[LC_MAX_TERMS];
    uint64_t len[LC_MAX_TERMS];
    uint32_t scalar[LC_MAX_TERMS][8];
    int nterms;
};

constexpr int EVAL_MAX = 16;
struct EvalArgs {
    const void* poly[EVAL_MAX];
    uint64_t len[EVAL_MAX];
    uint32_t point[EVAL_MAX][8];
    int count;
};

struct QuotientArgs {
    const void *a, *b, *c, *pi, *z1, *z2, *t, *h1, *h2;
    const void *q_m, *q_l, *q_r, *q_o, *q_c, *q_lookup, *q_table, *sigma1, *sigma2, *sigma3, *x, *l1;
    void* out;
// ... 7 lines not shown
    uint64_t first, count;
};
constexpr int QUOTIENT_PI_DIRECT_MAX = 16;

struct ZTermsArgs {
    const void *a, *b, *c, *s1, *s2, *s3, *roots;
    const void *f, *t, *h1, *h2;
    void *num, *den;
    uint32_t beta[8], gamma[8], delta[8], epsilon[8];
    uint64_t n;
};

int poly_mul_vec(zkt_ctx* c, const void* a, const void* b, void* out, size_t n);
int poly_set_zero(zkt_ctx* c, void* p, size_t n_elems);
int poly_trim_len(zkt_ctx* c, const void* p, size_t n, uint32_t* d_len, void* zero_at = nullptr, int zero_count = 0);
int poly_copy_pad(zkt_ctx* c, const void* d_in, size_t len, void* out, size_t n);
int poly_gather_pad(zkt_ctx* c, const void* d_values, size_t n_vars, const uint32_t* d_idx, size_t rows, void* out, size_t n,
                    uint32_t* d_status);
int poly_add_blinders(zkt_ctx* c, void* p, const uint32_t* d_len, const void* d_blinders, int k, size_t cap);
int poly_lincomb(zkt_ctx* c, const LinCombArgs& a, void* out, size_t n);
int lagrange_scalars(zkt_ctx* c, const void* ev, size_t n, const uint32_t* d_len, const void* d_blinders, int k, const void* d_roots,
                     void* out);
int poly_eval_many(zkt_ctx* c, const EvalArgs& a, void* d_partials, void* d_results, void* d_powers);
int z1_terms(zkt_ctx* c, const ZTermsArgs& a);
int z2_terms(zkt_ctx* c, const ZTermsArgs& a);
int scan_mul(zkt_ctx* c, const void* in, void* out, size_t n, bool reverse, void* d_tmp );
int scan_add(zkt_ctx* c, const void* in, void* out, size_t n, bool reverse, void* d_tmp);
int z_combine(zkt_ctx* c, const void* pn, const void* sd, const uint32_t inv_total[8], void* out, size_t n);
int quotient_pointwise(zkt_ctx* c, const QuotientArgs& a);
int to_hat_form(zkt_ctx* c, void* v, size_t n, int k32);
int quotient_interleave(zkt_ctx* c, const void* in, void* out, size_t n4, uint32_t G, uint32_t chunks = 1);
int quotient_split_blind(zkt_ctx* c, const void* q, size_t n, const void* d_b0b1, void* q_lo, void* q_mid, void* q_hi,
                         uint32_t* d_status);
int open_witness(zkt_ctx* c, const void* p, size_t len, const uint32_t z[8], const uint32_t z_inv[8], void* d_tmp_a, void* d_tmp_b,
                 void* d_scan_tmp, void* out, void* d_powers );
size_t open_witness_powers(size_t maxlen);
constexpr int OPEN_PW_ROW = 257;
int open_elems(size_t len);
size_t open_blocks(size_t len);
int open_pow_tables(zkt_ctx* c, const uint32_t z[8], const uint32_t z_inv[8], void* d_powers, size_t len);
int open_divide(zkt_ctx* c, const void* t, size_t len, void* d_tmp, void* d_scan_tmp, void* out, const void* d_powers);
int poly_sum_rows(zkt_ctx* c, const void* d_partials, int nblk, int rows, void* d_out);
int sigma_build(zkt_ctx* c, int log_n, const uint32_t* d_w_l, const uint32_t* d_w_r, const uint32_t* d_w_o, size_t n_rows, size_t n_vars,
                void* const* d_sigma);
size_t sigma_scratch_bytes(int log_n, size_t n_rows);
int sigma_enqueue(zkt_ctx* c, int log_n, const uint32_t* d_w_l, const uint32_t* d_w_r, const uint32_t* d_w_o, size_t n_rows, size_t n_vars,
                  void* const* d_sigma, void* d_scratch, uint32_t* d_flag);
struct WitnessCheckKeys {
    int log_n;
    const void* pk[5];
    const void* q_lookup_ev;
    const void* sigma_ev[3];
};
int witness_check(zkt_ctx* c, const WitnessCheckKeys& keys, const zkt_prove_inputs& in, int flags, zkt_witness_report* out);
int gen_powers(zkt_ctx* c, void* out, size_t n, const uint32_t base[8], const uint32_t scale[8]);
int lookup_count(zkt_ctx* c, const void* f, size_t n, const void* d_sorted_keys, const uint32_t* d_perm, uint32_t nkeys,
                 uint32_t* d_counts, uint32_t* d_status);
int lookup_starts(zkt_ctx* c, const uint32_t* d_base_counts, uint32_t* d_hits, uint32_t nkeys, size_t n, uint32_t* d_even,
                  uint32_t* d_odd, uint32_t* d_status);
int lookup_expand(zkt_ctx* c, const void* d_keys_insertion, const uint32_t* d_starts, uint32_t nkeys, void* out, size_t n);

}
```

### zkt-plonk_amd/csrc/prover.hip

```cpp
#include "ctx.hpp"
#include "hostinv.hpp"
#include <chrono>
#include <cstdio>
#include <cstdlib>
#include "ec.hpp"
#include "keyfile.hpp"
#include "msm.hpp"
#include "poly.hpp"
#include "transcript.hpp"

#include <algorithm>
#include <functional>
#include <cstring>
#include <memory>
#include <optional>
#include <vector>

namespace zkt {

enum { PK_QM = 0, PK_QL, PK_QR, PK_QO, PK_QC, PK_S1, PK_S2, PK_S3, PK_QLOOKUP, PK_QTABLE, PK_COUNT };
enum { CS_QM = 0, CS_QL, CS_QR, CS_QO, CS_QC, CS_QLOOKUP, CS_QTABLE, CS_S1, CS_S2, CS_S3, CS_X, CS_L1, CS_COUNT };
enum { W_A = 0, W_B, W_C, W_PI, W_Z1, W_Z2, W_T, W_H1, W_H2, W_COUNT };

struct CircuitState {
// ... 2 lines not shown
    int G = 1, cls = 0, log_m = 0;
    size_t m = 0;
    void* wnext[4] = {};
    void* fold = nullptr;
    void* qgather = nullptr;
    bool have[16] = {};
    void* pk[PK_COUNT] = {};
    size_t pk_len[PK_COUNT] = {};
    void* coset[CS_COUNT] = {};
    void* sigma_ev[3] = {};
    void* q_lookup_ev = nullptr;
    void* roots = nullptr;
    uint32_t zh_inv[4][8] = {};
    void* ev[8] = {};
    void* sc[4] = {};
    void* scan_tmp = nullptr;
    void* poly[13] = {};
    void* wcos[W_COUNT] = {};
    void* qev = nullptr;
    void* lag_scalars = nullptr;
    void* lag_scalars_q[3] = {};
    void* small = nullptr;
    uint32_t* status = nullptr;
    uint32_t* lk_u32 = nullptr;
    uint32_t lk_nkeys = 0;
    std::vector<uint32_t> lk_host_keys, lk_host_sorted, lk_host_counts, lk_host_order;
    bool has_next = false, prefetch_same_table = false;
    int prefetch_stage = 0;
    uint64_t prefetch_epoch = 0;
    zkt_prove_inputs next_in{}, prefetch_in{};
    void* poly_alt[3] = {};
    uint32_t* status_alt = nullptr;
    void* lk_keys = nullptr;
    size_t lk_cap = 0;
    void* pinned = nullptr;
    hipStream_t comm_stream = nullptr;
    hipEvent_t ev_piece[ZKT_QUOTIENT_CHUNKS] = {}, ev_gathered = nullptr;
    hipStream_t aux_stream = nullptr;
    hipEvent_t ev_aux_go = nullptr, ev_aux_done = nullptr;
    void* aux_scan_tmp = nullptr;
    void* aux_pw = nullptr;
    hipStream_t copy_stream = nullptr;
    hipEvent_t ev_copy[4] = {};
    void* pinned_pi = nullptr;
    uint32_t* pi_tab = nullptr;
    void* eval_pw = nullptr;
    std::vector<uint64_t> cached_table;
    bool t_cached = false, t_coset_valid = false;
    uint64_t t_srs_generation = 0;
    uint64_t t_commit_xy[12] = {};
    bool keys_borrowed = false;
    bool wire_route[3] = {};
    bool wire_dense_only = false;
};

template <class P>
struct HostF {
    using F = Fe<P>;
    static F from_words(const uint64_t* w) {
        F r;
        memcpy(r.v, w, 32);
        return r;
    }
    static void to_le_bytes(const F& mont, uint8_t out[32]) {
        F c = fe_from_mont<P>(mont);
        memcpy(out, c.v, 32);
    }
    static F from_le_bytes(const uint8_t in[32]) {
        F c;
        memcpy(c.v, in, 32);
        return fe_to_mont<P>(c);
    }
    static F pow_u64(F a, uint64_t e) { return fe_pow_u64<P>(a, e); }
};

template <class Q>
static void fq_to_le(const Fe<Q>& mont, uint8_t* out) {
    Fe<Q> c = fe_from_mont<Q>(mont);
    memcpy(out, c.v, Q::N * 4);
}

template <class Q>
static void serialize_point(const Affine<Q>& p, std::vector<uint8_t>& out) {
    const size_t nb = Q::N * 4;
    std::vector<uint8_t> b(nb, 0);
    if (aff_is_inf<Q>(p)) {
        b[nb - 1] |= 0x40;
    } else {
        fq_to_le<Q>(p.x, b.data());
        Fe<Q> y = fe_from_mont<Q>(p.y);
        Fe<Q> ny = fe_from_mont<Q>(fe_neg<Q>(p.y));
        bool greater = false;
        for (int i = Q::N - 1; i >= 0; --i) {
            if (y.v[i] != ny.v[i]) {
                greater = y.v[i] > ny.v[i];
                break;
            }
        }
        if (greater) b[nb - 1] |= 0x80;
    }
    out.insert(out.end(), b.begin(), b.end());
}

template <class C>
struct Prover {
    using R = typename C::Fr;
    using Q = typename C::Fq;
    using F = Fe<R>;
    using H = HostF<R>;

    zkt_ctx* c;
    CircuitState& S;
    HostTranscript& tr;
    Prover(zkt_ctx* ctx, CircuitState& st, HostTranscript& t) : c(ctx), S(st), tr(t) {
        trace_on = exp_env("ZKT_HOST_TRACE") != nullptr;
    }
    bool copy_fenced = false;
    bool trace_on = false;
    std::vector<std::pair<const char*, std::chrono::steady_clock::time_point>> marks;
    void mark(const char* what) {
        if (trace_on) marks.emplace_back(what, std::chrono::steady_clock::now());
    }
    void dump_marks() {
        if (!trace_on || marks.empty()) return;
        for (size_t i = 1; i < marks.size(); ++i)
            fprintf(stderr, "[zkt host] %-28s %8.1f us\n", marks[i].first,
                    std::chrono::duration<double, std::micro>(marks[i].second - marks[i - 1].second).count());
        marks.clear();
    }

    void tr_commit(const char* label, const Affine<Q>& p) {
        uint8_t x[64], y[64];
        bool inf = aff_is_inf<Q>(p);
        if (!inf) {
            fq_to_le<Q>(p.x, x);
            fq_to_le<Q>(p.y, y);
        }
        tr.append_commitment(label, x, y, Q::N * 4, inf);
    }
    void tr_scalar(const char* label, const F& v) {
        uint8_t b[32];
        H::to_le_bytes(v, b);
        tr.append_scalars(label, b, 1, 32, true);
    }
    F tr_challenge(const char* label) {
        uint8_t b[32];
        tr.challenge_scalar(label, R::BITS, b);
        return H::from_le_bytes(b);
    }
    static void put(uint32_t dst[8], const F& v) { memcpy(dst, v.v, 32); }

    std::optional<ProfScope> idle;
    void wait_begin() {
        if (c->prof_on && !idle) idle.emplace(c, "host_wait");
    }
    void wait_end() { idle.reset(); }
// ... 38 lines not shown
    int commit_begin_many(void* const* d_polys, const size_t* lens, const int* slots, int k) {
        for (int j = 0; j < k; ++j) {
            const int rc = queueing() ? commit_push(d_polys[j], lens[j], slots[j], 0) : commit_begin(d_polys[j], lens[j], slots[j]);
            if (rc) return rc;
        }
        return ZKT_OK;
    }
    int commit_evals_begin(const void* ev, const void* d_poly, int blinder_off, int k, int len_slot, int slot) {
        const bool q = queueing();
        if (!lagrange_ready(c, S.log_n) || c->lagrange_off)
            return q ? commit_push(d_poly, S.n + (size_t)k, slot, 0) : commit_begin(d_poly, S.n + (size_t)k, slot);
        if (q && n_lag_queued == 3)
            if (int rc0 = commit_flush()) return rc0;
        void* d = q ? S.lag_scalars_q[n_lag_queued] : S.lag_scalars;
        int rc = lagrange_scalars(c, ev, S.n, S.status + 8 + len_slot, (const char*)S.small + (size_t)blinder_off * 32, k, S.roots, d);
        if (rc) return rc;
        if (!q) return msm_begin(c, d, S.n + (size_t)k, 0, 1, slot, 1);
        ++n_lag_queued;
        return commit_push(d, S.n + (size_t)k, slot, 1);
    }
    int commit_collect(const int* slots, const bool* skip, int k, Affine<Q>* out) {
        wait_begin();
        if (!c->sharded()) {
            for (int j = 0; j < k; ++j) {
                if (skip && skip[j]) continue;
                uint64_t xy[12];
                int rc = msm_end(c, slots[j], xy);
                if (rc) return rc;
                memcpy(out[j].x.v, xy, Q::N * 4);
                memcpy(out[j].y.v, xy + Q::N / 2, Q::N * 4);
            }
            return ZKT_OK;
        }
        bool have[16];
        uint64_t xy[16 * 12];
        for (int j = 0; j < k; ++j) have[j] = !(skip && skip[j]) && S.have[slots[j]];
        int rc = msm_end_sharded(c, slots, have, k, xy);
        if (rc) return rc;
        for (int j = 0; j < k; ++j) {
            if (skip && skip[j]) continue;
            memcpy(out[j].x.v, xy + 12 * j, Q::N * 4);
            memcpy(out[j].y.v, xy + 12 * j + Q::N / 2, Q::N * 4);
        }
        return ZKT_OK;
    }

    int collect_wires(Affine<Q>* cm, int* took = nullptr) {
        for (int k = 0; k < 3; ++k) {
            const bool routed = S.wire_route[k];
            S.wire_route[k] = false;
            if (took) took[k] = 0;
            if (!routed) continue;
            if (wire_bases_check(c, k, S.n)) {
                if (took) took[k] = 1;
                continue;
            }
            static const int slot[1] = {0};
            int rc = msm_begin(c, S.poly[k], S.n + 2, 0, 1, 0);
            if (rc || (rc = commit_collect(slot, nullptr, 1, cm + k))) return rc;
        }
        return ZKT_OK;
    }

    struct PolyJob {
        const void* ev;
        void* poly;
        int blinder_off, k, len_slot;
    };
    int evals_to_blinded_polys(const PolyJob* jobs, int nb) {
        const size_t n = S.n;
        int rc;
        const void* ins[NTT_MAX_BATCH];
        void* outs[NTT_MAX_BATCH];
        size_t lens[NTT_MAX_BATCH];
        for (int y = 0; y < nb; ++y) {
            ins[y] = jobs[y].ev;
            outs[y] = jobs[y].poly;
            lens[y] = n;
        }
        if ((rc = ntt_run_batch(c, S.log_n, 1, 0, nb, ins, lens, outs))) return rc;
        for (int y = 0; y < nb; ++y) {
            void* poly = jobs[y].poly;
            if (jobs[y].k > 0) {
                if ((rc = poly_trim_len(c, poly, n, S.status + 8 + jobs[y].len_slot, (char*)poly + n * 32, 8))) return rc;
                if ((rc = poly_add_blinders(c, poly, S.status + 8 + jobs[y].len_slot,
                                            (const char*)S.small + (size_t)jobs[y].blinder_off * 32, jobs[y].k, n + 8)))
                    return rc;
            } else {
                ZKT_HIP(c, hipMemsetAsync((char*)poly + n * 32, 0, 8 * 32, c->stream));
            }
        }
        return ZKT_OK;
    }
    int evals_to_blinded_poly(const void* ev, void* poly, int blinder_off, int k, int len_slot) {
        const PolyJob j{ev, poly, blinder_off, k, len_slot};
        return evals_to_blinded_polys(&j, 1);
    }

    int check_status() {
        uint32_t st = 0;
        ZKT_HIP(c, hipMemcpyAsync(&st, S.status, 4, hipMemcpyDeviceToHost, c->stream));
        wait_begin();
        ZKT_HIP(c, hipStreamSynchronize(c->stream));
        if (st & 16u) return set_err(c, ZKT_ERR_INVALID_ARGUMENT, "wire index outside the variable map");
        if (st & 4u) return set_err(c, ZKT_ERR_NOT_IN_TABLE, "ElementNotIndexedInTable: a looked-up value is not in the table");
        if (st & 8u) return set_err(c, ZKT_ERR_INVALID_ARGUMENT, "combine_split: h1/h2 length differs from n");
        if (st & 2u) return set_err(c, ZKT_ERR_QUOTIENT_TOO_SHORT, "quotient degree exceeds 3n+5: the circuit is not satisfied");
// ... 103 lines not shown
        size_t lens[NTT_MAX_BATCH];
        int nb = 0;
        for (int k : ks) {
            ins[nb] = S.poly[coset_src[k]];
            outs[nb] = S.wcos[k];
            lens[nb] = S.n + 8;
            ++nb;
        }
        return nb ? ntt_run_batch(c, S.log_n + 2, 0, 1, nb, ins, lens, outs) : ZKT_OK;
    }

    void swap_work_sets() {
        for (int k = 0; k < 3; ++k) std::swap(S.poly[k], S.poly_alt[k]);
        std::swap(S.status, S.status_alt);
    }

    int enqueue_round_1(const zkt_prove_inputs& in) {
        const size_t n = S.n;
        int rc;
        ProfScope prof_round(c, "round1");
        if (in.n_rows > n) return set_err(c, ZKT_ERR_INVALID_ARGUMENT, "more rows than the circuit bound");
        if (in.table_len >= n) return set_err(c, ZKT_ERR_INVALID_ARGUMENT, "max table size is equal or larger than n");
        if (n < 8) return set_err(c, ZKT_ERR_INVALID_ARGUMENT, "circuit bound below 8");
        if (!in.blinders) return set_err(c, ZKT_ERR_INVALID_ARGUMENT, "null blinders");
        ZKT_HIP(c, hipMemsetAsync(S.status, 0, 64 * 4, c->stream));
        ZKT_HIP(c, hipMemcpyAsync(S.small, in.blinders, 19 * 32, hipMemcpyHostToDevice, c->stream));

        const uint64_t* wires[3] = {in.a_evals, in.b_evals, in.c_evals};
        const bool from_vars = in.a_evals == nullptr && in.variables != nullptr;
        const void* d_vars = in.variables;
        const uint32_t* d_idx[3] = {in.w_l, in.w_r, in.w_o};
        if (from_vars) {
            if (in.n_rows && (!in.w_l || !in.w_r || !in.w_o)) return set_err(c, ZKT_ERR_INVALID_ARGUMENT, "null wire index vector");
            if (in.n_vars > 0xFFFFFFFEull) return set_err(c, ZKT_ERR_INVALID_ARGUMENT, "too many variables");
            if (!in.wires_on_device) {
                if (in.n_vars > 4 * n || 3 * in.n_rows * 4 > (n + 8) * 32)
                    return set_err(c, ZKT_ERR_INVALID_ARGUMENT, "witness larger than the staging buffers");
                if (in.n_vars)
                    ZKT_HIP(c, hipMemcpyAsync(S.qev, in.variables, in.n_vars * 32, hipMemcpyHostToDevice, c->stream));
                d_vars = S.qev;
                for (int k = 0; k < 3; ++k) {
                    uint32_t* dst = (uint32_t*)S.poly[12] + (size_t)k * in.n_rows;
                    if (in.n_rows)
                        ZKT_HIP(c, hipMemcpyAsync(dst, d_idx[k], in.n_rows * 4, hipMemcpyHostToDevice, c->stream));
                    d_idx[k] = dst;
                }
            }
        }
        const bool host_wires = !from_vars && !in.wires_on_device;
        for (bool& r : S.wire_route) r = false;
        bool wire_tables = from_vars && in.wires_on_device && !c->sharded() && !c->lagrange_off && !S.wire_dense_only &&
                           lagrange_ready(c, S.log_n) && in.n_rows > 0;
        if (wire_tables) {
            if ((rc = wire_bases_prepare(c, S.log_n, d_idx, in.n_rows, in.n_vars))) return rc;
            wire_tables = wire_bases_use(c, 0) || wire_bases_use(c, 1) || wire_bases_use(c, 2);
            if (wire_tables && (rc = wire_bases_digest(c, d_idx, in.n_rows))) return rc;
        }
        if (host_wires) {
            if (!copy_fenced) {
                ZKT_HIP(c, hipEventRecord(S.ev_copy[3], c->stream));
                ZKT_HIP(c, hipStreamWaitEvent(S.copy_stream, S.ev_copy[3], 0));
            }
            copy_fenced = false;
            for (int k = 0; k < 3; ++k) {
                if (in.n_rows < n)
                    ZKT_HIP(c, hipMemsetAsync((char*)S.ev[k] + in.n_rows * 32, 0, (n - in.n_rows) * 32, S.copy_stream));
                if (in.n_rows)
                    ZKT_HIP(c, hipMemcpyAsync(S.ev[k], wires[k], in.n_rows * 32, hipMemcpyHostToDevice, S.copy_stream));
                ZKT_HIP(c, hipEventRecord(S.ev_copy[k], S.copy_stream));
                ZKT_HIP(c, hipStreamWaitEvent(c->stream, S.ev_copy[k], 0));
                if ((rc = evals_to_blinded_poly(S.ev[k], S.poly[k], 2 * k, 2, k))) return rc;
                if ((rc = commit_begin(S.poly[k], n + 2, k))) return rc;
            }
        } else {
            for (int k = 0; k < 3; ++k) {
                if (from_vars) {
                    if ((rc = poly_gather_pad(c, d_vars, in.n_vars, d_idx[k], in.n_rows, S.ev[k], n, S.status))) return rc;
                } else {
                    if ((rc = poly_copy_pad(c, wires[k], in.n_rows, S.ev[k], n))) return rc;
                }
            }
            const PolyJob jobs[3] = {{S.ev[0], S.poly[0], 0, 2, 0}, {S.ev[1], S.poly[1], 2, 2, 1}, {S.ev[2], S.poly[2], 4, 2, 2}};
            if ((rc = evals_to_blinded_polys(jobs, 3))) return rc;
            if (wire_tables && (rc = wire_bases_lens(c, S.status + 8))) return rc;
            for (int k = 0; k < 3; ++k) {
                const void* sc = S.poly[k];
                size_t len = n + 2;
                int tbl = 0;
                if (wire_tables && wire_bases_use(c, k)) {
                    if ((rc = wire_bases_scalars(c, k, d_vars, (const char*)S.small + (size_t)(2 * k) * 32, n, &sc, &len))) return rc;
                    tbl = MSM_TBL_WIRE + k;
                    S.wire_route[k] = true;
                }
                rc = queueing() ? commit_push(sc, len, k, tbl) : tbl ? msm_begin(c, sc, len, 0, 1, k, tbl) : commit_begin(sc, len, k);
                if (rc) return rc;
            }
        }
        if ((rc = commit_flush())) return rc;
        return to_coset_many({W_A, W_B, W_C});
    }

    bool table_is_cached(const zkt_prove_inputs& in) const {
        return S.t_cached && S.t_srs_generation == c->srs_generation && S.cached_table.size() == 4 * in.table_len &&
               (in.table_len == 0 || memcmp(S.cached_table.data(), in.table, in.table_len * 32) == 0);
    }
    int enqueue_table(const zkt_prove_inputs& in, bool with_coset) {
        const size_t n = S.n;
// ... 945 lines not shown
        return set_err(c, ZKT_ERR_INVALID_ARGUMENT,
                       "sharded proof: this rank must load powers zkt_shard_range(total, rank, world) with zkt_srs_load_slice");
    if (c->circuit && c->circuit->G != c->comm.vt.world)
        return set_err(c, ZKT_ERR_NOT_LOADED, "the circuit was loaded for another communicator");
    return ZKT_OK;
}

static int prove_impl(zkt_ctx* c, const zkt_prove_inputs* in, HostTranscript& tr, uint8_t* out, size_t cap, size_t* len) {
    if (!c->circuit) return set_err(c, ZKT_ERR_NOT_LOADED, "no circuit loaded (zkt_circuit_load)");
    if (!c->msm) return set_err(c, ZKT_ERR_NOT_LOADED, "no SRS loaded (zkt_srs_load)");
    if (int rc0 = check_sharded_key(c)) return rc0;
    (void)hipSetDevice(c->device);
    if (!c->lagrange_off)
        if (int rc1 = lagrange_ensure(c, c->circuit->log_n)) return rc1;
    std::vector<uint8_t> proof;
    int rc;
    if (c->curve == ZKT_CURVE_BN254) {
        Prover<Bn254Curve> p(c, *c->circuit, tr);
        rc = p.run(*in, proof);
        if (rc) {
            (void)hipStreamSynchronize(c->circuit->copy_stream);
            if (c->circuit->comm_stream) (void)hipStreamSynchronize(c->circuit->comm_stream);
            if (c->circuit->aux_stream) (void)hipStreamSynchronize(c->circuit->aux_stream);
            (void)hipStreamSynchronize(c->stream);
        }
    } else {
        Prover<Bls381Curve> p(c, *c->circuit, tr);
        rc = p.run(*in, proof);
        if (rc) {
            (void)hipStreamSynchronize(c->circuit->copy_stream);
            if (c->circuit->comm_stream) (void)hipStreamSynchronize(c->circuit->comm_stream);
            if (c->circuit->aux_stream) (void)hipStreamSynchronize(c->circuit->aux_stream);
            (void)hipStreamSynchronize(c->stream);
        }
    }
    if (rc) {
        c->circuit->has_next = false;
        c->circuit->prefetch_stage = 0;
        return rc;
    }
    if (len) *len = proof.size();
    if (proof.size() > cap) return set_err(c, ZKT_ERR_INVALID_ARGUMENT, "proof buffer too small");
    memcpy(out, proof.data(), proof.size());
    return ZKT_OK;
}

int zkt_ctx_set_lagrange(zkt_ctx* c, int on) {
    if (!c) return ZKT_ERR_INVALID_ARGUMENT;
    c->lagrange_off = !on;
    ++c->msm_epoch;
    return ZKT_OK;
}

int zkt_lagrange_info(zkt_ctx* c, int* log_n, size_t* bases) {
    if (!c) return ZKT_ERR_INVALID_ARGUMENT;
    const bool ready = c->circuit && lagrange_ready(c, c->circuit->log_n) && !c->lagrange_off;
    if (log_n) *log_n = ready ? c->circuit->log_n : -1;
    if (bases) *bases = ready ? lagrange_bases(c) : 0;
    return ZKT_OK;
}

int zkt_commit_evals_dev(zkt_ctx* c, const void* d_evals, const uint64_t* blinders, int k, int path, uint64_t* out_xy,
                         int* out_is_infinity) {
    if (!c || !d_evals || !out_xy || (k > 0 && !blinders)) return set_err(c, ZKT_ERR_INVALID_ARGUMENT, "null pointer");
    if (k < 0 || k > 3) return set_err(c, ZKT_ERR_INVALID_ARGUMENT, "0 .. 3 blinders");
    if (!c->circuit) return set_err(c, ZKT_ERR_NOT_LOADED, "no circuit loaded (the domain comes from it)");
    if (!c->msm) return set_err(c, ZKT_ERR_NOT_LOADED, "no SRS loaded (zkt_srs_load)");
    if (c->sharded()) return set_err(c, ZKT_ERR_INVALID_ARGUMENT, "not available on a sharded key");
    (void)hipSetDevice(c->device);
    CircuitState& S = *c->circuit;
    const size_t n = S.n;
    int rc;
    if (path == 1) {
        if ((rc = lagrange_ensure(c, S.log_n))) return rc;
        if (!lagrange_ready(c, S.log_n)) return set_err(c, ZKT_ERR_NOT_LOADED, "the key is too short for the Lagrange-basis table");
    } else if (path != 0) {
        return set_err(c, ZKT_ERR_INVALID_ARGUMENT, "path: 0 coefficients, 1 Lagrange basis");
    }
    c->circuit->prefetch_stage = 0;
    uint32_t* d_len = S.status + 8 + 12;
    void* d_bl = (char*)S.lag_scalars + (n + 8) * 32;
    void* poly = S.poly[12];
    ZKT_HIP(c, hipMemsetAsync(d_len, 0, 4, c->stream));
    if (k) ZKT_HIP(c, hipMemcpyAsync(d_bl, blinders, (size_t)k * 32, hipMemcpyHostToDevice, c->stream));
    if ((rc = ntt_run(c, S.log_n, 1, 0, d_evals, n, poly))) return rc;
    if ((rc = poly_trim_len(c, poly, n, d_len, (char*)poly + n * 32, 8))) return rc;
    if (k && (rc = poly_add_blinders(c, poly, d_len, d_bl, k, n + 8))) return rc;
    if (path == 0) return msm_g1_dev(c, poly, n + (size_t)k, 0, 1, out_xy, out_is_infinity);
    if ((rc = lagrange_scalars(c, d_evals, n, d_len, d_bl, k, S.roots, S.lag_scalars))) return rc;
    if ((rc = msm_begin(c, S.lag_scalars, n + (size_t)k, 0, 1, 0, 1))) return rc;
    uint64_t xy[12] = {};
    if ((rc = msm_end(c, 0, xy))) return rc;
    const size_t words = c->curve == ZKT_CURVE_BN254 ? 8 : 12;
    memcpy(out_xy, xy, words * 8);
    if (out_is_infinity) {
        bool any = false;
        for (size_t i = 0; i < words; ++i) any = any || xy[i] != 0;
        *out_is_infinity = any ? 0 : 1;
    }
    return ZKT_OK;
}

int zkt_circuit_setup(zkt_ctx* c, int log_n, const uint64_t* const* evals, const size_t* eval_lens, int evals_on_device,
                      uint64_t* out_commitments, int* out_is_infinity) {
    if (!c || !evals || !eval_lens || !out_commitments) return set_err(c, ZKT_ERR_INVALID_ARGUMENT, "null pointer");
    if (!c->msm) return set_err(c, ZKT_ERR_NOT_LOADED, "no SRS loaded (zkt_srs_load)");
// ... 215 lines not shown
        ea.len[j] = lc.len[j] = lens[j];
        memcpy(ea.point[j], points + 4 * j, 32);
        memcpy(lc.scalar[j], scalars + 4 * j, 32);
    }
    void* d_partials = (char*)S.small + 64 * 32;
    void* d_results = (char*)S.small + 32 * 32;
    int rc = poly_eval_many(c, ea, d_partials, d_results, S.eval_pw);
    if (rc) return rc;
    if ((rc = poly_lincomb(c, lc, S.sc[0], out_len))) return rc;
    ZKT_HIP(c, hipMemcpyAsync(out_evals, d_results, (size_t)k * 32, hipMemcpyDeviceToHost, c->stream));
    ZKT_HIP(c, hipMemcpyAsync(out_lincomb, S.sc[0], out_len * 32, hipMemcpyDeviceToHost, c->stream));
    ZKT_HIP(c, hipStreamSynchronize(c->stream));
    return ZKT_OK;
}

int zkt_debug_open_witness(zkt_ctx* c, const uint64_t* coeffs, size_t len, const uint64_t* z4, uint64_t* out) {
    if (!c || !coeffs || !z4 || !out) return set_err(c, ZKT_ERR_INVALID_ARGUMENT, "null pointer");
    if (!c->circuit) return set_err(c, ZKT_ERR_NOT_LOADED, "no circuit loaded (zkt_circuit_load)");
    CircuitState& S = *c->circuit;
    if (len < 2 || len > S.n + 8) return set_err(c, ZKT_ERR_INVALID_ARGUMENT, "2 .. n + 8 coefficients");
    (void)hipSetDevice(c->device);
    c->circuit->prefetch_stage = 0;
    uint32_t z[8], zi[8];
    memcpy(z, z4, 32);
    bool zero = true;
    for (int i = 0; i < 8; ++i) zero = zero && z[i] == 0;
    if (zero) return set_err(c, ZKT_ERR_ZERO_DENOMINATOR, "evaluation point is zero");
    if (c->curve == ZKT_CURVE_BN254) {
        Fe<Bn254Fr> x;
        memcpy(x.v, z, 32);
        x = fe_inv_host<Bn254Fr>(x);
        memcpy(zi, x.v, 32);
    } else {
        Fe<Bls381Fr> x;
        memcpy(x.v, z, 32);
        x = fe_inv_host<Bls381Fr>(x);
        memcpy(zi, x.v, 32);
    }
    ZKT_HIP(c, hipMemcpyAsync(S.sc[0], coeffs, len * 32, hipMemcpyHostToDevice, c->stream));
    int rc = open_witness(c, S.sc[0], len, z, zi, S.sc[1], S.sc[2], S.scan_tmp, S.sc[3], S.eval_pw);
    if (rc) return rc;
    ZKT_HIP(c, hipMemcpyAsync(out, S.sc[3], (len - 1) * 32, hipMemcpyDeviceToHost, c->stream));
    ZKT_HIP(c, hipStreamSynchronize(c->stream));
    return ZKT_OK;
}

extern "C++" template <class C>
static int debug_commit_wires_t(zkt_ctx* c, const zkt_prove_inputs& in, int route, uint64_t* out_xy, int* out_inf, int* out_route) {
    using Q = typename C::Fq;
    CircuitState& S = *c->circuit;
    MerlinHostTranscript tr("zkt_debug_commit_wires_dev");
    Prover<C> p(c, S, tr);
    S.wire_dense_only = route == 0;
    int rc = p.enqueue_round_1(in);
    S.wire_dense_only = false;
    Affine<Q> cm[3];
    static const int slots[3] = {0, 1, 2};
    int took[3] = {0, 0, 0};
    if (!rc) rc = p.commit_collect(slots, nullptr, 3, cm);
    if (!rc) rc = p.collect_wires(cm, took);
    p.wait_end();
    if (!rc) rc = p.check_status();
    if (rc) {
        for (bool& r : S.wire_route) r = false;
        (void)hipStreamSynchronize(c->stream);
        return rc;
    }
    for (int k = 0; k < 3; ++k) {
        memcpy(out_xy + (size_t)k * Q::N, cm[k].x.v, Q::N * 4);
        memcpy(out_xy + (size_t)k * Q::N + Q::N / 2, cm[k].y.v, Q::N * 4);
        if (out_inf) out_inf[k] = aff_is_inf<Q>(cm[k]) ? 1 : 0;
        if (out_route) out_route[k] = took[k];
    }
    return ZKT_OK;
}

int zkt_debug_commit_wires_dev(zkt_ctx* c, const void* d_variables, size_t n_vars, const uint32_t* d_w_l, const uint32_t* d_w_r,
                               const uint32_t* d_w_o, size_t n_rows, const uint64_t* blinders, int route, uint64_t* out_xy,
                               int* out_is_infinity, int* out_route) {
    if (!c || !d_variables || !blinders || !out_xy) return set_err(c, ZKT_ERR_INVALID_ARGUMENT, "null pointer");
    if (route != 0 && route != 1) return set_err(c, ZKT_ERR_INVALID_ARGUMENT, "route: 0 coefficients, 1 wire base tables");
    if (!c->circuit) return set_err(c, ZKT_ERR_NOT_LOADED, "no circuit loaded (the domain comes from it)");
    if (!c->msm) return set_err(c, ZKT_ERR_NOT_LOADED, "no SRS loaded (zkt_srs_load)");
    if (c->sharded()) return set_err(c, ZKT_ERR_INVALID_ARGUMENT, "not available on a sharded key");
    CircuitState& S = *c->circuit;
    if (S.has_next) return set_err(c, ZKT_ERR_INVALID_ARGUMENT, "zkt_debug_commit_wires_dev: a next proof is announced");
    (void)hipSetDevice(c->device);
    S.prefetch_stage = 0;
    if (route == 1 && !c->lagrange_off)
        if (int rc1 = lagrange_ensure(c, S.log_n)) return rc1;
    uint64_t bl[19 * 4] = {};
    memcpy(bl, blinders, 6 * 32);
    zkt_prove_inputs in{};
    in.variables = (const uint64_t*)d_variables;
    in.n_vars = n_vars;
    in.w_l = d_w_l; in.w_r = d_w_r; in.w_o = d_w_o;
    in.n_rows = n_rows;
    in.wires_on_device = 1;
    in.blinders = bl;
    if (c->curve == ZKT_CURVE_BN254) return debug_commit_wires_t<Bn254Curve>(c, in, route, out_xy, out_is_infinity, out_route);
    return debug_commit_wires_t<Bls381Curve>(c, in, route, out_xy, out_is_infinity, out_route);
}

int zkt_prove_set_next(zkt_ctx* c, const zkt_prove_inputs* next) {
    if (!c) return ZKT_ERR_INVALID_ARGUMENT;
    if (!c->circuit) return set_err(c, ZKT_ERR_NOT_LOADED, "no circuit loaded (zkt_circuit_load)");
    c->circuit->has_next = next != nullptr;
    if (next) c->circuit->next_in = *next;
    return ZKT_OK;
}

int zkt_prove(zkt_ctx* c, const zkt_prove_inputs* in, zkt_transcript* tr, uint8_t* proof_out, size_t proof_cap,
              size_t* proof_len) {
    if (!c || !in || !tr || !proof_out) return set_err(c, ZKT_ERR_INVALID_ARGUMENT, "null pointer");
    return prove_impl(c, in, *tr->impl, proof_out, proof_cap, proof_len);
}

int zkt_prove_with(zkt_ctx* c, const zkt_prove_inputs* in, const zkt_transcript_vtable* vt, uint8_t* proof_out,
                   size_t proof_cap, size_t* proof_len) {
    if (!c || !in || !vt || !proof_out) return set_err(c, ZKT_ERR_INVALID_ARGUMENT, "null pointer");
    if (c->curve == ZKT_CURVE_BN254) {
        VtableAdapter<Bn254Curve> a(vt);
        return prove_impl(c, in, a, proof_out, proof_cap, proof_len);
    }
    VtableAdapter<Bls381Curve> a(vt);
    return prove_impl(c, in, a, proof_out, proof_cap, proof_len);
}

}
```

Measured before the change: 55.38 proofs/s.

## Eliminate linearly-defined wire variables when building Lagrange wire base tables

Adds a host-side elimination pass that finds output wires defined by linear gates (q_m=0, q_o=±1) and rewrites them as short linear combinations of free variables plus a constant. The wire base tables are then built over the free variables only, with the constant carried as an extra scalar. The aim is to cut the number of distinct points in the wire commitment MSM. This is enabled automatically above a log_n threshold. In exchange it adds a host analysis pass, extra selector NTTs and table rebuild complexity, and these costs may fall on the prove path.

```diff
diff --git a/include/zkt_plonk.h b/include/zkt_plonk.h
--- a/include/zkt_plonk.h
+++ b/include/zkt_plonk.h
@@ -98,6 +98,7 @@
                      uint64_t* out_w_xy_mont, int* out_w_is_infinity, uint64_t* out_evals_mont);
 
 int zkt_ctx_set_lagrange(zkt_ctx* ctx, int on);
+int zkt_ctx_set_wire_elimination(zkt_ctx* ctx, int mode);
 int zkt_lagrange_info(zkt_ctx* ctx, int* log_n, size_t* bases);
 int zkt_commit_evals_dev(zkt_ctx* ctx, const void* d_evals, const uint64_t* blinders, int k, int path, uint64_t* out_xy_mont,
                          int* out_is_infinity);
@@ -302,6 +303,13 @@
 int zkt_debug_commit_wires_dev(zkt_ctx* ctx, const void* d_variables, size_t n_vars, const uint32_t* d_w_l, const uint32_t* d_w_r,
                                const uint32_t* d_w_o, size_t n_rows, const uint64_t* blinders, int route, uint64_t* out_xy_mont,
                                int* out_is_infinity, int* out_route);
+int zkt_debug_commit_wires_pi_dev(zkt_ctx* ctx, const void* d_variables, size_t n_vars, const uint32_t* d_w_l, const uint32_t* d_w_r,
+                                  const uint32_t* d_w_o, size_t n_rows, const uint64_t* blinders, int route, const size_t* pi_pos,
+                                  size_t n_pi, uint64_t* out_xy_mont, int* out_is_infinity, int* out_route);
+int zkt_debug_wire_elimination(int curve, const uint64_t* const* selectors, const uint32_t* w_l, const uint32_t* w_r, const uint32_t* w_o,
+                               size_t n_rows, size_t n_vars, const size_t* pi_pos, size_t n_pi, int K, uint8_t* out_kind,
+                               uint32_t* out_free, size_t* out_n_free, uint32_t* out_term_v, uint32_t* out_term_f,
+                               uint64_t* out_term_coef, size_t* out_n_terms, uint64_t* out_kappa);
 int zkt_debug_open_witness(zkt_ctx* ctx, const uint64_t* coeffs, size_t len, const uint64_t* z4, uint64_t* out);
 int zkt_debug_eval_lincomb(zkt_ctx* ctx, const uint64_t* const* polys, const size_t* lens, int k, const uint64_t* points,
                            const uint64_t* scalars, uint64_t* out_evals, uint64_t* out_lincomb, size_t out_len);
diff --git a/shim/src/ffi.rs b/shim/src/ffi.rs
--- a/shim/src/ffi.rs
+++ b/shim/src/ffi.rs
@@ -92,6 +92,7 @@
     pub fn zkt_commit_evals_dev(ctx: *mut ZktCtx, d_evals: *const c_void, blinders: *const u64, k: c_int, path: c_int,
                                 out_xy_mont: *mut u64, out_is_infinity: *mut c_int) -> c_int;
     pub fn zkt_ctx_set_lagrange(ctx: *mut ZktCtx, on: c_int) -> c_int;
+    pub fn zkt_ctx_set_wire_elimination(ctx: *mut ZktCtx, mode: c_int) -> c_int;
     pub fn zkt_lagrange_info(ctx: *mut ZktCtx, log_n: *mut c_int, bases: *mut usize) -> c_int;
     pub fn zkt_circuit_load(ctx: *mut ZktCtx, log_n: c_int, pk_polys: *const *const u64, pk_lens: *const usize) -> c_int;
     pub fn zkt_circuit_load_file(ctx: *mut ZktCtx, pk_path: *const c_char, log_n: c_int) -> c_int;
diff --git a/zkt-plonk_amd/_lib.py b/zkt-plonk_amd/_lib.py
--- a/zkt-plonk_amd/_lib.py
+++ b/zkt-plonk_amd/_lib.py
@@ -538,6 +538,35 @@
     return out, bool(inf.value)
 
 
+def wire_elimination(curve, selectors, w_l, w_r, w_o, n_vars: int, pi_pos=(), K: int = 16):
+    L = lib()
+    sel = [np.ascontiguousarray(q, dtype=np.uint64).reshape(-1, 4) for q in selectors]
+    w = [np.ascontiguousarray(x, dtype=np.uint32) for x in (w_l, w_r, w_o)]
+    n_rows = len(w[0])
+    assert len(sel) == 5 and all(q.shape[0] == n_rows for q in sel) and all(len(x) == n_rows for x in w)
+    pi = (ctypes.c_size_t * max(len(pi_pos), 1))(*[int(x) for x in pi_pos])
+    cap = max(K * n_vars, 1)
+    kind = np.zeros(max(n_vars, 1), dtype=np.uint8)
+    free = np.zeros(max(n_vars, 1), dtype=np.uint32)
+    tv, tf = np.zeros(cap, dtype=np.uint32), np.zeros(cap, dtype=np.uint32)
+    tc = np.zeros((cap, 4), dtype=np.uint64)
+    kappa = np.zeros((max(n_vars, 1), 4), dtype=np.uint64)
+    n_free, n_terms = ctypes.c_size_t(0), ctypes.c_size_t(0)
+    P64, P32 = ctypes.POINTER(ctypes.c_uint64), ctypes.POINTER(ctypes.c_uint32)
+    sp = (P64 * 5)(*[u64p(q) for q in sel])
+    L.zkt_debug_wire_elimination.argtypes = [ctypes.c_int, ctypes.POINTER(P64), P32, P32, P32, ctypes.c_size_t, ctypes.c_size_t,
+                                             ctypes.POINTER(ctypes.c_size_t), ctypes.c_size_t, ctypes.c_int,
+                                             ctypes.POINTER(ctypes.c_uint8), P32, ctypes.POINTER(ctypes.c_size_t), P32, P32, P64,
+                                             ctypes.POINTER(ctypes.c_size_t), P64]
+    rc = L.zkt_debug_wire_elimination(curve_id(curve), sp, _u32p(w[0]), _u32p(w[1]), _u32p(w[2]), n_rows, n_vars, pi, len(pi_pos),
+                                      int(K), kind.ctypes.data_as(ctypes.POINTER(ctypes.c_uint8)), _u32p(free), ctypes.byref(n_free),
+                                      _u32p(tv), _u32p(tf), u64p(tc), ctypes.byref(n_terms), u64p(kappa))
+    if rc:
+        raise ZktError(rc, "zkt_debug_wire_elimination")
+    nt = n_terms.value
+    return kind[:n_vars], free[:n_free.value].copy(), tv[:nt].copy(), tf[:nt].copy(), tc[:nt].copy(), kappa[:n_vars]
+
+
 class Transcript:
 
     def __init__(self, kind: str = "merlin", label: str = "ZKT Plonk", fr_bits: int = 254, fq_bytes: int = 32):
@@ -971,6 +1000,10 @@
     def set_lagrange(self, on: bool = True):
         self._L.zkt_ctx_set_lagrange.argtypes = [ctypes.c_void_p, ctypes.c_int]
         self.check(self._L.zkt_ctx_set_lagrange(self._h, int(on)))
+
+    def set_wire_elimination(self, mode: int = 1):
+        self._L.zkt_ctx_set_wire_elimination.argtypes = [ctypes.c_void_p, ctypes.c_int]
+        self.check(self._L.zkt_ctx_set_wire_elimination(self._h, int(mode)))
 
     def lagrange_info(self):
         self._L.zkt_lagrange_info.argtypes = [ctypes.c_void_p, ctypes.POINTER(ctypes.c_int), ctypes.POINTER(ctypes.c_size_t)]
@@ -1173,11 +1206,24 @@
         return h1, h2
 
     def debug_commit_wires_dev(self, d_variables: int, n_vars: int, d_w_l: int, d_w_r: int, d_w_o: int, n_rows: int, blinders,
-                               route: int = 1):
+                               route: int = 1, pi_pos=None):
         bl = np.ascontiguousarray(blinders, dtype=np.uint64).reshape(6, 4)
         out = np.zeros((3, 2 * self.fq_limbs), dtype=np.uint64)
         inf = (ctypes.c_int * 3)()
         took = (ctypes.c_int * 3)()
+        if route == 2 or pi_pos is not None:
+            pos = [int(x) for x in (pi_pos or ())]
+            pi = (ctypes.c_size_t * max(len(pos), 1))(*pos)
+            self._L.zkt_debug_commit_wires_pi_dev.argtypes = [ctypes.c_void_p, ctypes.c_void_p, ctypes.c_size_t, ctypes.c_void_p,
+                                                              ctypes.c_void_p, ctypes.c_void_p, ctypes.c_size_t,
+                                                              ctypes.POINTER(ctypes.c_uint64), ctypes.c_int,
+                                                              ctypes.POINTER(ctypes.c_size_t), ctypes.c_size_t,
+                                                              ctypes.POINTER(ctypes.c_uint64), ctypes.POINTER(ctypes.c_int),
+                                                              ctypes.POINTER(ctypes.c_int)]
+            self.check(self._L.zkt_debug_commit_wires_pi_dev(self._h, ctypes.c_void_p(d_variables), n_vars, ctypes.c_void_p(d_w_l),
+                                                             ctypes.c_void_p(d_w_r), ctypes.c_void_p(d_w_o), n_rows, u64p(bl),
+                                                             int(route), pi, len(pos), u64p(out), inf, took))
+            return out, [bool(x) for x in inf], [int(x) for x in took]
         self._L.zkt_debug_commit_wires_dev.argtypes = [ctypes.c_void_p, ctypes.c_void_p, ctypes.c_size_t, ctypes.c_void_p,
                                                        ctypes.c_void_p, ctypes.c_void_p, ctypes.c_size_t,
                                                        ctypes.POINTER(ctypes.c_uint64), ctypes.c_int,
diff --git a/zkt-plonk_amd/csrc/capi.hip b/zkt-plonk_amd/csrc/capi.hip
--- a/zkt-plonk_amd/csrc/capi.hip
+++ b/zkt-plonk_amd/csrc/capi.hip
@@ -225,6 +225,7 @@
     if (rc) return rc;
     (void)hipStreamSynchronize(parent->stream);
     c->lagrange_off = parent->lagrange_off;
+    c->wire_elim_mode = parent->wire_elim_mode;
     c->batch_off = parent->batch_off;
     c->aux_off = parent->aux_off;
     c->ntt_plans = parent->ntt_plans;
diff --git a/zkt-plonk_amd/csrc/check.hip b/zkt-plonk_amd/csrc/check.hip
--- a/zkt-plonk_amd/csrc/check.hip
+++ b/zkt-plonk_amd/csrc/check.hip
@@ -170,6 +170,15 @@
 static unsigned ck_blocks(size_t n) {
     const size_t per = (size_t)CK_THREADS * CK_ROWS_PER_THREAD;
     return (unsigned)std::min<size_t>(std::max<size_t>((n + per - 1) / per, 1), CK_MAX_BLOCKS);
+}
+
+int selector_evals_enqueue(zkt_ctx* c, int log_n, const void* const* pk, void* const* outs) {
+    const size_t n = (size_t)1 << log_n;
+    size_t lens[5];
+    for (size_t& l : lens) l = n;
+    static_assert(NTT_MAX_BATCH >= 4, "four selectors in one batch");
+    if (int rc = ntt_run_batch(c, log_n, 0, 0, 4, pk, lens, outs)) return rc;
+    return ntt_run_batch(c, log_n, 0, 0, 1, pk + 4, lens + 4, outs + 4);
 }
 
 template <class P>
@@ -283,17 +292,9 @@
 
     {
         ProfScope prof(c, "check_witness");
-        const void* ins[5];
         void* outs[5];
-        size_t lens[5];
-        for (int k = 0; k < 5; ++k) {
-            ins[k] = K.pk[k];
-            lens[k] = n;
-            outs[k] = base + o_sel[k];
-        }
-        static_assert(NTT_MAX_BATCH >= 4, "four selectors in one batch");
-        if ((rc = ntt_run_batch(c, log_n, 0, 0, 4, ins, lens, outs))) return rc;
-        if ((rc = ntt_run_batch(c, log_n, 0, 0, 1, ins + 4, lens + 4, outs + 4))) return rc;
+        for (int k = 0; k < 5; ++k) outs[k] = base + o_sel[k];
+        if ((rc = selector_evals_enqueue(c, log_n, K.pk, outs))) return rc;
 
         if (vars) {
             hipLaunchKernelGGL((k_check_gates<P, true>), dim3(ck_blocks(n)), dim3(CK_THREADS), 0, c->stream, q);
diff --git a/zkt-plonk_amd/csrc/ctx.hpp b/zkt-plonk_amd/csrc/ctx.hpp
--- a/zkt-plonk_amd/csrc/ctx.hpp
+++ b/zkt-plonk_amd/csrc/ctx.hpp
@@ -73,6 +73,7 @@
     bool aux_off = false;
     bool batch_off = false;
     bool lagrange_off = false;
+    int wire_elim_mode = 1;
     std::shared_ptr<zkt::CircuitState> circuit;
     std::vector<void*> owned;
 };
diff --git a/zkt-plonk_amd/csrc/lagrange.hip b/zkt-plonk_amd/csrc/lagrange.hip
--- a/zkt-plonk_amd/csrc/lagrange.hip
+++ b/zkt-plonk_amd/csrc/lagrange.hip
@@ -2,9 +2,13 @@
 #include "ec.hpp"
 #include "hostec.hpp"
 #include "msm.hpp"
+#include "poly.hpp"
+#include "wire_elim.hpp"
 
 #include <algorithm>
+#include <chrono>
 #include <cstdio>
+#include <cstring>
 #include <cstdlib>
 #include <vector>
 
@@ -313,10 +317,10 @@
 }
 
 template <class P>
-__global__ void k_wire_scalars(const Fe<P>* vars, const uint32_t* u, size_t cnt, const Fe<P>* bl, Fe<P> ninv, Fe<P>* out) {
+__global__ void k_wire_scalars(const Fe<P>* vars, const uint32_t* u, size_t cnt, size_t extra, const Fe<P>* bl, Fe<P> ninv, Fe<P>* out) {
     const size_t j = (size_t)blockIdx.x * blockDim.x + threadIdx.x;
-    if (j >= cnt + 2) return;
-    fe_store<P>(out + j, j < cnt ? fe_mul<P>(fe_load<P>(vars + u[j]), ninv) : fe_load<P>(bl + (j - cnt)));
+    if (j >= cnt + extra + 2) return;
+    fe_store<P>(out + j, j < cnt ? fe_mul<P>(fe_load<P>(vars + u[j]), ninv) : j < cnt + extra ? ninv : fe_load<P>(bl + (j - cnt - extra)));
 }
 
 void wire_bases_drop(zkt_ctx* c) {
@@ -348,62 +352,89 @@
     return ZKT_OK;
 }
 
+struct WireGroups {
+    void *d_cnt = nullptr, *d_start = nullptr, *d_grouped = nullptr, *d_ofs = nullptr, *d_bad = nullptr;
+    std::vector<uint32_t> start;
+    std::vector<uint32_t> u, ofs;
+    size_t d = 0;
+    uint32_t at = 0;
+};
+static void wire_groups_free(zkt_ctx* c, WireGroups& g) {
+    dev_free(c, g.d_cnt); dev_free(c, g.d_start); dev_free(c, g.d_grouped); dev_free(c, g.d_ofs); dev_free(c, g.d_bad);
+    g = WireGroups{};
+}
+static bool wire_groups_count(zkt_ctx* c, const uint32_t* d_idx, size_t n_rows, size_t n_vars, WireGroups& g) {
+    if (dev_alloc(c, &g.d_cnt, (n_vars + 1) * 4)) return false;
+    if (hipMemsetAsync(g.d_cnt, 0, (n_vars + 1) * 4, c->stream) != hipSuccess) return false;
+    const unsigned rb = (unsigned)((n_rows + 255) / 256);
+    if (n_rows) hipLaunchKernelGGL(k_wire_count, dim3(rb), dim3(256), 0, c->stream, d_idx, n_rows, (uint32_t)n_vars, (uint32_t*)g.d_cnt);
+    g.start.assign(n_vars + 1, 0);
+    if (hipMemcpyAsync(g.start.data(), g.d_cnt, n_vars * 4, hipMemcpyDeviceToHost, c->stream) != hipSuccess ||
+        hipStreamSynchronize(c->stream) != hipSuccess)
+        return false;
+    uint32_t at = 0;
+    for (size_t v = 0; v < n_vars; ++v) {
+        const uint32_t m = g.start[v];
+        g.start[v] = at;
+        if (m) {
+            g.u.push_back((uint32_t)v);
+            g.ofs.push_back(at);
+            at += m;
+        }
+    }
+    g.ofs.push_back(at);
+    g.at = at;
+    g.d = g.u.size();
+    return true;
+}
+template <class C>
+static bool wire_points(zkt_ctx* c, const uint32_t* d_idx, size_t n_rows, size_t n_vars, WireGroups& g, Affine<typename C::Fq>* out) {
+    using Q = typename C::Fq;
+    MsmState& st = *c->msm;
+    const size_t d = g.d;
+    if (dev_alloc(c, &g.d_start, (n_vars + 1) * 4) || dev_alloc(c, &g.d_grouped, ((size_t)g.at + 1) * 4) ||
+        dev_alloc(c, &g.d_ofs, (d + 1) * 4) || dev_alloc(c, &g.d_bad, 4))
+        return false;
+    if (hipMemcpyAsync(g.d_start, g.start.data(), n_vars * 4, hipMemcpyHostToDevice, c->stream) != hipSuccess ||
+        hipMemcpyAsync(g.d_ofs, g.ofs.data(), (d + 1) * 4, hipMemcpyHostToDevice, c->stream) != hipSuccess ||
+        hipMemsetAsync(g.d_cnt, 0, (n_vars + 1) * 4, c->stream) != hipSuccess || hipMemsetAsync(g.d_bad, 0, 4, c->stream) != hipSuccess)
+        return false;
+    const unsigned rb = (unsigned)((n_rows + 255) / 256);
+    if (n_rows)
+        hipLaunchKernelGGL(k_wire_fill, dim3(rb), dim3(256), 0, c->stream, d_idx, n_rows, (uint32_t)n_vars, (const uint32_t*)g.d_start,
+                           (uint32_t*)g.d_cnt, (uint32_t*)g.d_grouped);
+    if (d)
+        hipLaunchKernelGGL(k_wire_sum<C>, dim3((unsigned)((d + 63) / 64)), dim3(64), 0, c->stream, (const Affine<Q>*)st.table2,
+                           (const uint32_t*)g.d_grouped, (const uint32_t*)g.d_ofs, d, out, (uint32_t*)g.d_bad);
+    uint32_t bad = 0;
+    if (hipGetLastError() != hipSuccess || hipMemcpyAsync(&bad, g.d_bad, 4, hipMemcpyDeviceToHost, c->stream) != hipSuccess ||
+        hipStreamSynchronize(c->stream) != hipSuccess)
+        return false;
+    return bad == 0;
+}
+
 template <class C>
 static int wire_bases_build_wire(zkt_ctx* c, int log_n, int k, const uint32_t* d_idx, size_t n_rows, size_t n_vars, double frac) {
     using Q = typename C::Fq;
     MsmState& st = *c->msm;
     WireBases& wb = st.wb;
     const size_t n = (size_t)1 << log_n;
-    void *d_cnt = nullptr, *d_start = nullptr, *d_grouped = nullptr, *d_ofs = nullptr, *d_bad = nullptr, *table = nullptr, *d_u = nullptr;
+    WireGroups g;
+    void *table = nullptr, *d_u = nullptr;
     auto done = [&](bool keep) {
-        dev_free(c, d_cnt); dev_free(c, d_start); dev_free(c, d_grouped); dev_free(c, d_ofs); dev_free(c, d_bad);
+        wire_groups_free(c, g);
         if (!keep) { dev_free(c, table); dev_free(c, d_u); }
         (void)hipGetLastError();
         return ZKT_OK;
     };
-    if (dev_alloc(c, &d_cnt, (n_vars + 1) * 4)) return done(false);
-    ZKT_HIP(c, hipMemsetAsync(d_cnt, 0, (n_vars + 1) * 4, c->stream));
-    const unsigned rb = (unsigned)((n_rows + 255) / 256);
-    if (n_rows) hipLaunchKernelGGL(k_wire_count, dim3(rb), dim3(256), 0, c->stream, d_idx, n_rows, (uint32_t)n_vars, (uint32_t*)d_cnt);
-    std::vector<uint32_t> cnt(n_vars + 1);
-    if (hipMemcpyAsync(cnt.data(), d_cnt, n_vars * 4, hipMemcpyDeviceToHost, c->stream) != hipSuccess ||
-        hipStreamSynchronize(c->stream) != hipSuccess)
-        return done(false);
-    std::vector<uint32_t> u, ofs;
-    uint32_t at = 0;
-    for (size_t v = 0; v < n_vars; ++v) {
-        const uint32_t m = cnt[v];
-        cnt[v] = at;
-        if (m) {
-            u.push_back((uint32_t)v);
-            ofs.push_back(at);
-            at += m;
-        }
-    }
-    ofs.push_back(at);
-    const size_t d = u.size();
+    if (!wire_groups_count(c, d_idx, n_rows, n_vars, g)) return done(false);
+    const size_t d = g.d;
     if ((double)d >= frac * (double)n_rows || (uint64_t)st.plan.W * (d + 2) >= ((uint64_t)1 << 31)) return done(false);
-    if (dev_alloc(c, &table, (size_t)st.plan.W * (d + 2) * sizeof(Affine<Q>)) || dev_alloc(c, &d_u, (d + 1) * 4) ||
-        dev_alloc(c, &d_start, (n_vars + 1) * 4) || dev_alloc(c, &d_grouped, ((size_t)at + 1) * 4) || dev_alloc(c, &d_ofs, (d + 1) * 4) ||
-        dev_alloc(c, &d_bad, 4))
-        return done(false);
-    ZKT_HIP(c, hipMemcpyAsync(d_start, cnt.data(), n_vars * 4, hipMemcpyHostToDevice, c->stream));
-    ZKT_HIP(c, hipMemcpyAsync(d_u, u.data(), d * 4, hipMemcpyHostToDevice, c->stream));
-    ZKT_HIP(c, hipMemcpyAsync(d_ofs, ofs.data(), (d + 1) * 4, hipMemcpyHostToDevice, c->stream));
-    ZKT_HIP(c, hipMemsetAsync(d_cnt, 0, (n_vars + 1) * 4, c->stream));
-    ZKT_HIP(c, hipMemsetAsync(d_bad, 0, 4, c->stream));
-    if (n_rows)
-        hipLaunchKernelGGL(k_wire_fill, dim3(rb), dim3(256), 0, c->stream, d_idx, n_rows, (uint32_t)n_vars, (const uint32_t*)d_start,
-                           (uint32_t*)d_cnt, (uint32_t*)d_grouped);
-    if (d)
-        hipLaunchKernelGGL(k_wire_sum<C>, dim3((unsigned)((d + 63) / 64)), dim3(64), 0, c->stream, (const Affine<Q>*)st.table2,
-                           (const uint32_t*)d_grouped, (const uint32_t*)d_ofs, d, (Affine<Q>*)table, (uint32_t*)d_bad);
+    if (dev_alloc(c, &table, (size_t)st.plan.W * (d + 2) * sizeof(Affine<Q>)) || dev_alloc(c, &d_u, (d + 1) * 4)) return done(false);
+    if (hipMemcpyAsync(d_u, g.u.data(), d * 4, hipMemcpyHostToDevice, c->stream) != hipSuccess) return done(false);
+    if (!wire_points<C>(c, d_idx, n_rows, n_vars, g, (Affine<Q>*)table)) return done(false);
     hipLaunchKernelGGL(k_wire_blinder_points<C>, dim3(1), dim3(64), 0, c->stream, (const Affine<Q>*)st.table2, n, d, (Affine<Q>*)table);
-    uint32_t bad = 0;
-    if (hipGetLastError() != hipSuccess || hipMemcpyAsync(&bad, d_bad, 4, hipMemcpyDeviceToHost, c->stream) != hipSuccess ||
-        hipStreamSynchronize(c->stream) != hipSuccess)
-        return done(false);
-    if (bad || msm_table_finish(c, table, d + 2)) return done(false);
+    if (hipGetLastError() != hipSuccess || msm_table_finish(c, table, d + 2)) return done(false);
     wb.table[k] = table;
     wb.u[k] = (uint32_t*)d_u;
     wb.cnt[k] = d;
@@ -411,15 +442,261 @@
     return done(true);
 }
 
-int wire_bases_prepare(zkt_ctx* c, int log_n, const uint32_t* const* d_idx, size_t n_rows, size_t n_vars) {
+constexpr uint32_t WIRE_NONE = 0xFFFFFFFFu;
+constexpr uint32_t WIRE_FOLD_PIECE = 32;
+
+template <class C>
+ZKT_D Xyzz<typename C::Fq> wire_fold_range(const Affine<typename C::Fq>* T, const uint32_t* pos, const uint32_t* ent_v,
+                                           const Fe<typename C::Fr>* ent_c, uint32_t lo, uint32_t hi) {
+    using Q = typename C::Fq;
+    using R = typename C::Fr;
+    const Fe<R> one = fe_one<R>();
+    Xyzz<Q> acc = xyzz_identity<Q>();
+#pragma unroll 1
+    for (uint32_t e = lo; e < hi; ++e) {
+        const uint32_t j = pos[ent_v[e]];
+        if (j == WIRE_NONE) continue;
+        const Affine<Q> p = aff_load<Q>(T + j);
+        const Fe<R> cm = fe_load<R>(ent_c + e);
+        if (fe_eq<R>(cm, one)) acc = xyzz_add_mixed<Q>(acc, p);
+        else acc = xyzz_add<Q>(acc, xyzz_scalar_mul<Q, R>(xyzz_from_affine<Q>(p), fe_from_mont<R>(cm)));
+    }
+    return acc;
+}
+template <class C>
+__global__ __launch_bounds__(64) void k_wire_fold(const Affine<typename C::Fq>* T, const uint32_t* pos, const uint32_t* ent_v,
+                                                   const Fe<typename C::Fr>* ent_c, const uint2* piece, size_t np,
+                                                   Xyzz<typename C::Fq>* part) {
+    using Q = typename C::Fq;
+    const size_t t = (size_t)blockIdx.x * blockDim.x + threadIdx.x;
+    if (t >= np) return;
+    const uint2 pc = piece[t];
+    xyzz_store<Q>(part + t, wire_fold_range<C>(T, pos, ent_v, ent_c, pc.x, pc.y));
+}
+template <class C>
+__global__ __launch_bounds__(64) void k_wire_fold_sum(const Xyzz<typename C::Fq>* part, const uint32_t* pstart, size_t cnt, size_t groups,
+                                                       Affine<typename C::Fq>* out, uint32_t* flags) {
+    using Q = typename C::Fq;
+    const size_t j = (size_t)blockIdx.x * blockDim.x + threadIdx.x;
+    if (j >= groups) return;
+    Xyzz<Q> acc = xyzz_identity<Q>();
+#pragma unroll 1
+    for (uint32_t t = pstart[j]; t < pstart[j + 1]; ++t) acc = xyzz_add<Q>(acc, xyzz_load<Q>(part + t));
+    const bool none = xyzz_is_identity<Q>(acc);
+    if (j < cnt ? none : !none) atomicOr(flags + (j < cnt ? 0 : 1), 1u);
+    aff_store<Q>(out + j, xyzz_to_affine<Q>(acc));
+}
+
+struct WireElimShared {
+    std::vector<uint32_t> free_vars, ofs, ent_v;
+    size_t n_defined = 0, n_const = 0;
+    void *d_ent_v = nullptr, *d_ent_c = nullptr;
+};
+static void wire_elim_shared_free(zkt_ctx* c, WireElimShared& D) {
+    dev_free(c, D.d_ent_v); dev_free(c, D.d_ent_c);
+    D = WireElimShared{};
+}
+
+template <class C>
+static bool wire_elim_host(zkt_ctx* c, int log_n, const uint32_t* const* d_idx, size_t n_rows, size_t n_vars, const WireElimKeys& ew,
+                           WireElimShared& D) {
+    using R = typename C::Fr;
+    using F = Fe<R>;
+    const size_t n = (size_t)1 << log_n;
+    void* d_sel[5] = {};
+    std::vector<F> sel_h[5];
+    std::vector<uint32_t> w_h[3];
+    bool ok = true;
+    for (int k = 0; k < 5 && ok; ++k) ok = dev_alloc(c, &d_sel[k], n * sizeof(F)) == ZKT_OK;
+    if (ok) ok = selector_evals_enqueue(c, log_n, ew.pk, d_sel) == ZKT_OK;
+    for (int k = 0; k < 5 && ok; ++k) {
+        sel_h[k].resize(n_rows);
+        ok = hipMemcpyAsync(sel_h[k].data(), d_sel[k], n_rows * sizeof(F), hipMemcpyDeviceToHost, c->stream) == hipSuccess;
+    }
+    for (int k = 0; k < 3 && ok; ++k) {
+        w_h[k].resize(n_rows);
+        ok = hipMemcpyAsync(w_h[k].data(), d_idx[k], n_rows * 4, hipMemcpyDeviceToHost, c->stream) == hipSuccess;
+    }
+    if (hipStreamSynchronize(c->stream) != hipSuccess) ok = false;
+    for (void* p : d_sel) dev_free(c, p);
+    if (!ok) {
+        (void)hipGetLastError();
+        return false;
+    }
+    WireElim<R> E;
+    {
+        const F* sp[5] = {sel_h[0].data(), sel_h[1].data(), sel_h[2].data(), sel_h[3].data(), sel_h[4].data()};
+        const uint32_t* wp[3] = {w_h[0].data(), w_h[1].data(), w_h[2].data()};
+        wire_eliminate<R>(sp, wp, n_rows, n_vars, ew.pi_pos, ew.n_pi, WIRE_ELIM_K, E);
+    }
+    const size_t nf = E.free_vars.size(), nd = E.def_vars.size();
+    if (!nf || !nd) return false;
+    size_t nk = 0;
+    for (const F& k : E.kappa) nk += !fe_is_zero<R>(k);
+    const uint64_t total = (uint64_t)nf + E.term_f.size() + nk;
+    if (total >= 0xFFFFFFFFull) return false;
+    std::vector<uint32_t> fid(n_vars, 0), cur(nf + 1, 0);
+    for (size_t g = 0; g < nf; ++g) fid[E.free_vars[g]] = (uint32_t)g;
+    D.ofs.assign(nf + 2, 0);
+    for (size_t g = 0; g < nf; ++g) D.ofs[g + 1] = 1;
+    for (uint32_t f : E.term_f) ++D.ofs[fid[f] + 1];
+    D.ofs[nf + 1] = (uint32_t)nk;
+    for (size_t g = 0; g <= nf; ++g) D.ofs[g + 1] += D.ofs[g];
+    D.ent_v.resize(total);
+    std::vector<F> ent_c(total);
+    const F one = fe_one<R>();
+    for (size_t g = 0; g < nf; ++g) {
+        cur[g] = D.ofs[g];
+        D.ent_v[cur[g]] = E.free_vars[g];
+        ent_c[cur[g]++] = one;
+    }
+    cur[nf] = D.ofs[nf];
+    for (size_t d = 0; d < nd; ++d) {
+        for (uint64_t t = E.def_start[d]; t < E.def_start[d + 1]; ++t) {
+            const uint32_t g = fid[E.term_f[t]];
+            D.ent_v[cur[g]] = E.def_vars[d];
+            ent_c[cur[g]++] = E.term_c[t];
+        }
+        if (!fe_is_zero<R>(E.kappa[d])) {
+            D.ent_v[cur[nf]] = E.def_vars[d];
+            ent_c[cur[nf]++] = E.kappa[d];
+        }
+    }
+    D.free_vars.swap(E.free_vars);
+    D.n_defined = nd;
+    D.n_const = nk;
+    ok = !dev_alloc(c, &D.d_ent_v, total * 4) && !dev_alloc(c, &D.d_ent_c, total * sizeof(F));
+    ok = ok && hipMemcpyAsync(D.d_ent_v, D.ent_v.data(), total * 4, hipMemcpyHostToDevice, c->stream) == hipSuccess &&
+         hipMemcpyAsync(D.d_ent_c, ent_c.data(), total * sizeof(F), hipMemcpyHostToDevice, c->stream) == hipSuccess;
+    if (hipStreamSynchronize(c->stream) != hipSuccess) ok = false;
+    if (!ok) {
+        (void)hipGetLastError();
+        wire_elim_shared_free(c, D);
+    }
+    return ok;
+}
+
+template <class C>
+static bool wire_elim_build_wire(zkt_ctx* c, int log_n, int k, const uint32_t* d_idx, size_t n_rows, size_t n_vars, double frac,
+                                 const WireElimShared& D, size_t* nonzeros) {
+    using Q = typename C::Fq;
+    using R = typename C::Fr;
+    MsmState& st = *c->msm;
+    WireBases& wb = st.wb;
+    const size_t n = (size_t)1 << log_n;
+    WireGroups g;
+    void *d_T = nullptr, *d_pos = nullptr, *d_piece = nullptr, *d_pstart = nullptr, *d_part = nullptr, *d_flag = nullptr, *table = nullptr,
+         *d_u = nullptr;
+    auto done = [&](bool keep) {
+        wire_groups_free(c, g);
+        dev_free(c, d_T); dev_free(c, d_pos); dev_free(c, d_piece); dev_free(c, d_pstart); dev_free(c, d_part); dev_free(c, d_flag);
+        if (!keep) { dev_free(c, table); dev_free(c, d_u); }
+        (void)hipGetLastError();
+        return keep;
+    };
+    *nonzeros = 0;
+    if (!wire_groups_count(c, d_idx, n_rows, n_vars, g)) return done(false);
+    const size_t d = g.d;
+    if (!d) return done(false);
+    const size_t present = (double)d < frac * (double)n_rows ? d : n_rows;
+    std::vector<uint32_t> pos(n_vars, WIRE_NONE), u, pstart(1, 0);
+    std::vector<uint2> piece;
+    for (size_t j = 0; j < d; ++j) pos[g.u[j]] = (uint32_t)j;
+    const size_t nf = D.free_vars.size();
+    auto cut = [&](size_t grp) {
+        for (uint32_t lo = D.ofs[grp]; lo < D.ofs[grp + 1]; lo += WIRE_FOLD_PIECE)
+            piece.push_back(make_uint2(lo, std::min(lo + WIRE_FOLD_PIECE, D.ofs[grp + 1])));
+        pstart.push_back((uint32_t)piece.size());
+    };
+    for (size_t f = 0; f < nf; ++f) {
+        size_t here = 0;
+        for (uint32_t e = D.ofs[f]; e < D.ofs[f + 1]; ++e) here += pos[D.ent_v[e]] != WIRE_NONE;
+        if (here) {
+            u.push_back(D.free_vars[f]);
+            cut(f);
+            *nonzeros += here;
+        }
+    }
+    const size_t cnt = u.size();
+    if (!cnt || (double)(cnt + 1) >= frac * (double)present || (uint64_t)st.plan.W * (cnt + 3) >= ((uint64_t)1 << 31)) return done(false);
+    if (D.n_const) cut(nf);
+    const size_t groups = pstart.size() - 1, np = piece.size();
+    if (dev_alloc(c, &d_T, d * sizeof(Affine<Q>)) || dev_alloc(c, &d_pos, n_vars * 4) || dev_alloc(c, &d_piece, np * sizeof(uint2)) ||
+        dev_alloc(c, &d_pstart, (groups + 1) * 4) || dev_alloc(c, &d_u, (cnt + 1) * 4) || dev_alloc(c, &d_part, np * sizeof(Xyzz<Q>)) ||
+        dev_alloc(c, &d_flag, 8) || dev_alloc(c, &table, (size_t)st.plan.W * (cnt + 3) * sizeof(Affine<Q>)))
+        return done(false);
+    if (hipMemcpyAsync(d_pos, pos.data(), n_vars * 4, hipMemcpyHostToDevice, c->stream) != hipSuccess ||
+        hipMemcpyAsync(d_piece, piece.data(), np * sizeof(uint2), hipMemcpyHostToDevice, c->stream) != hipSuccess ||
+        hipMemcpyAsync(d_pstart, pstart.data(), (groups + 1) * 4, hipMemcpyHostToDevice, c->stream) != hipSuccess ||
+        hipMemcpyAsync(d_u, u.data(), cnt * 4, hipMemcpyHostToDevice, c->stream) != hipSuccess ||
+        hipMemsetAsync(d_flag, 0, 8, c->stream) != hipSuccess)
+        return done(false);
+    if (!wire_points<C>(c, d_idx, n_rows, n_vars, g, (Affine<Q>*)d_T)) return done(false);
+    hipLaunchKernelGGL(k_wire_fold<C>, dim3((unsigned)((np + 63) / 64)), dim3(64), 0, c->stream, (const Affine<Q>*)d_T,
+                       (const uint32_t*)d_pos, (const uint32_t*)D.d_ent_v, (const Fe<R>*)D.d_ent_c, (const uint2*)d_piece, np,
+                       (Xyzz<Q>*)d_part);
+    hipLaunchKernelGGL(k_wire_fold_sum<C>, dim3((unsigned)((groups + 63) / 64)), dim3(64), 0, c->stream, (const Xyzz<Q>*)d_part,
+                       (const uint32_t*)d_pstart, cnt, groups, (Affine<Q>*)table, (uint32_t*)d_flag);
+    uint32_t flags[2] = {0, 0};
+    if (hipGetLastError() != hipSuccess || hipMemcpyAsync(flags, d_flag, 8, hipMemcpyDeviceToHost, c->stream) != hipSuccess ||
+        hipStreamSynchronize(c->stream) != hipSuccess)
+        return done(false);
+    if (flags[0]) return done(false);
+    const size_t has_c = flags[1] ? 1 : 0;
+    hipLaunchKernelGGL(k_wire_blinder_points<C>, dim3(1), dim3(64), 0, c->stream, (const Affine<Q>*)st.table2, n, cnt + has_c,
+                       (Affine<Q>*)table);
+    if (hipGetLastError() != hipSuccess || msm_table_finish(c, table, cnt + has_c + 2)) return done(false);
+    wb.table[k] = table;
+    wb.u[k] = (uint32_t*)d_u;
+    wb.cnt[k] = cnt;
+    wb.use[k] = true;
+    wb.elim[k] = true;
+    wb.has_c[k] = has_c != 0;
+    return done(true);
+}
+
+template <class C>
+static int wire_bases_build_all(zkt_ctx* c, int log_n, const uint32_t* const* d_idx, size_t n_rows, size_t n_vars, double frac,
+                                const WireElimKeys* ew, bool trace) {
+    using clk = std::chrono::steady_clock;
+    auto ms = [](clk::time_point a, clk::time_point b) { return std::chrono::duration<double, std::milli>(b - a).count(); };
+    WireElimShared D;
+    bool elim = false;
+    const auto t0 = clk::now();
+    if (ew) elim = wire_elim_host<C>(c, log_n, d_idx, n_rows, n_vars, *ew, D);
+    const auto t1 = clk::now();
+    size_t nz[3] = {};
+    int rc = ZKT_OK;
+    for (int k = 0; k < 3 && !rc; ++k)
+        if (!elim || !wire_elim_build_wire<C>(c, log_n, k, d_idx[k], n_rows, n_vars, frac, D, &nz[k]))
+            rc = wire_bases_build_wire<C>(c, log_n, k, d_idx[k], n_rows, n_vars, frac);
+    if (trace && ew) {
+        const WireBases& wb = c->msm->wb;
+        fprintf(stderr, "[zkt host] wire elimination%s: %zu free, %zu defined (%zu with a constant); non-zeros per wire %zu / %zu / %zu; "
+                "routes %d / %d / %d (2 = free variables); host pass %.1f ms, device build %.1f ms\n", elim ? "" : " (not possible)",
+                D.free_vars.size(), D.n_defined, D.n_const, nz[0], nz[1], nz[2], wb.use[0] + wb.elim[0], wb.use[1] + wb.elim[1],
+                wb.use[2] + wb.elim[2], ms(t0, t1), ms(t1, clk::now()));
+    }
+    wire_elim_shared_free(c, D);
+    return rc;
+}
+
+int wire_bases_prepare(zkt_ctx* c, int log_n, const uint32_t* const* d_idx, size_t n_rows, size_t n_vars, const WireElimKeys* ew) {
     if (!c->msm) return ZKT_OK;
     MsmState& st = *c->msm;
     WireBases& wb = st.wb;
     const size_t n = (size_t)1 << log_n;
     const bool possible = lagrange_ready(c, log_n) && !c->sharded() && !c->lagrange_off && st.count2 >= n + 2 && n_rows <= n &&
                           n_vars <= 0xFFFFFFFEull && !(exp_env("ZKT_WIRE_BASES") && atoi(exp_env("ZKT_WIRE_BASES")) == 0);
+    if (ew && exp_env("ZKT_WIRE_ELIM") && atoi(exp_env("ZKT_WIRE_ELIM")) == 0) ew = nullptr;
+    std::vector<size_t> pi;
+    if (ew) {
+        pi.assign(ew->pi_pos, ew->pi_pos + ew->n_pi);
+        std::sort(pi.begin(), pi.end());
+    }
     const bool same = wb.built && !wb.stale && wb.w[0] == d_idx[0] && wb.w[1] == d_idx[1] && wb.w[2] == d_idx[2] &&
-                      wb.n_rows == n_rows && wb.n_vars == n_vars && wb.log_n == log_n && wb.srs_generation == c->srs_generation;
+                      wb.n_rows == n_rows && wb.n_vars == n_vars && wb.log_n == log_n && wb.srs_generation == c->srs_generation &&
+                      wb.elim_wanted == (ew != nullptr) && wb.pi_pos == pi;
     if (possible && same) return ZKT_OK;
     if (wb.built && !wb.borrowed && c->forks.load() > 0) {
         if (!same || !possible) wb.stale = true;
@@ -435,17 +712,15 @@
         (void)hipEventCreate(&e0); (void)hipEventCreate(&e1);
         (void)hipEventRecord(e0, c->stream);
     }
-    for (int k = 0; k < 3; ++k) {
-        const int rc = c->curve == ZKT_CURVE_BN254 ? wire_bases_build_wire<Bn254Curve>(c, log_n, k, d_idx[k], n_rows, n_vars, frac)
-                                                    : wire_bases_build_wire<Bls381Curve>(c, log_n, k, d_idx[k], n_rows, n_vars, frac);
-        if (rc) return rc;
-    }
+    if (int rc = c->curve == ZKT_CURVE_BN254 ? wire_bases_build_all<Bn254Curve>(c, log_n, d_idx, n_rows, n_vars, frac, ew, trace)
+                                             : wire_bases_build_all<Bls381Curve>(c, log_n, d_idx, n_rows, n_vars, frac, ew, trace))
+        return rc;
     if (int rc = wire_digest_enqueue(c, d_idx, n_rows)) return rc;
     ZKT_HIP(c, hipStreamSynchronize(c->stream));
     if (trace) {
         float ms = 0;
         (void)hipEventRecord(e1, c->stream); (void)hipEventSynchronize(e1); (void)hipEventElapsedTime(&ms, e0, e1);
-        fprintf(stderr, "[zkt host] wire base tables: %zu / %zu / %zu distinct of %zu rows (0 = dense), %.1f ms\n",
+        fprintf(stderr, "[zkt host] wire base tables: %zu / %zu / %zu bases of %zu rows (0 = dense), %.1f ms\n",
                 wb.use[0] ? wb.cnt[0] : 0, wb.use[1] ? wb.cnt[1] : 0, wb.use[2] ? wb.cnt[2] : 0, n_rows, ms);
         (void)hipEventDestroy(e0); (void)hipEventDestroy(e1);
     }
@@ -453,6 +728,8 @@
     wb.digest[1] = st.wb_pin[1];
     for (int k = 0; k < 3; ++k) wb.w[k] = d_idx[k];
     wb.n_rows = n_rows; wb.n_vars = n_vars; wb.log_n = log_n; wb.srs_generation = c->srs_generation;
+    wb.elim_wanted = ew != nullptr;
+    wb.pi_pos.swap(pi);
     wb.built = true;
     ++c->msm_epoch;
     return ZKT_OK;
@@ -461,6 +738,7 @@
 bool wire_bases_use(const zkt_ctx* c, int k) {
     return c->msm && c->msm->wb.built && !c->msm->wb.stale && c->msm->wb.use[k];
 }
+int wire_bases_route(const zkt_ctx* c, int k) { return !wire_bases_use(c, k) ? 0 : c->msm->wb.elim[k] ? 2 : 1; }
 int wire_bases_digest(zkt_ctx* c, const uint32_t* const* d_idx, size_t n_rows) { return wire_digest_enqueue(c, d_idx, n_rows); }
 int wire_bases_lens(zkt_ctx* c, const uint32_t* d_lens) {
     ZKT_HIP(c, hipMemcpyAsync(c->msm->wb_pin + 2, d_lens, 12, hipMemcpyDeviceToHost, c->stream));
@@ -471,17 +749,17 @@
 static int wire_scalars_t(zkt_ctx* c, int k, const void* d_vars, const void* d_bl, size_t n, const void** out, size_t* len) {
     using R = typename C::Fr;
     MsmState& st = *c->msm;
-    const size_t cnt = st.wb.cnt[k];
-    if (int rc = grow(c, st.wb_scalars[k], (cnt + 2) * sizeof(Fe<R>))) return rc;
+    const size_t cnt = st.wb.cnt[k], extra = st.wb.has_c[k] ? 1 : 0;
+    if (int rc = grow(c, st.wb_scalars[k], (cnt + extra + 2) * sizeof(Fe<R>))) return rc;
     Fe<R> nn = fe_zero<R>();
     nn.v[0] = (uint32_t)(n & 0xffffffffu);
     nn.v[1] = (uint32_t)((uint64_t)n >> 32);
     const Fe<R> ninv = fe_inv_host<R>(fe_to_mont<R>(nn));
-    hipLaunchKernelGGL(k_wire_scalars<R>, dim3((unsigned)((cnt + 2 + 255) / 256)), dim3(256), 0, c->stream, (const Fe<R>*)d_vars,
-                       (const uint32_t*)st.wb.u[k], cnt, (const Fe<R>*)d_bl, ninv, (Fe<R>*)st.wb_scalars[k].p);
+    hipLaunchKernelGGL(k_wire_scalars<R>, dim3((unsigned)((cnt + extra + 2 + 255) / 256)), dim3(256), 0, c->stream, (const Fe<R>*)d_vars,
+                       (const uint32_t*)st.wb.u[k], cnt, extra, (const Fe<R>*)d_bl, ninv, (Fe<R>*)st.wb_scalars[k].p);
     ZKT_HIP(c, hipGetLastError());
     *out = st.wb_scalars[k].p;
-    *len = cnt + 2;
+    *len = cnt + extra + 2;
     return ZKT_OK;
 }
 int wire_bases_scalars(zkt_ctx* c, int k, const void* d_vars, const void* d_blinders, size_t n, const void** out, size_t* len) {
@@ -498,4 +776,54 @@
     return ((const uint32_t*)(st.wb_pin + 2))[k] == (uint32_t)n;
 }
 
-}
+template <class R>
+static int debug_wire_elimination_t(const uint64_t* const* selectors, const uint32_t* const* w, size_t n_rows, size_t n_vars,
+                                    const size_t* pi_pos, size_t n_pi, int K, uint8_t* out_kind, uint32_t* out_free, size_t* out_n_free,
+                                    uint32_t* out_term_v, uint32_t* out_term_f, uint64_t* out_term_coef, size_t* out_n_terms,
+                                    uint64_t* out_kappa) {
+    using F = Fe<R>;
+    static_assert(sizeof(F) == 32, "scalar field element = 4 x 64-bit words");
+    const F* sel[5];
+    for (int k = 0; k < 5; ++k) sel[k] = reinterpret_cast<const F*>(selectors[k]);
+    WireElim<R> E;
+    wire_eliminate<R>(sel, w, n_rows, n_vars, pi_pos, n_pi, K, E);
+    if (n_vars) memcpy(out_kind, E.kind.data(), n_vars);
+    if (!E.free_vars.empty()) memcpy(out_free, E.free_vars.data(), E.free_vars.size() * 4);
+    *out_n_free = E.free_vars.size();
+    memset(out_kappa, 0, n_vars * 32);
+    size_t t = 0;
+    for (size_t d = 0; d < E.def_vars.size(); ++d) {
+        memcpy(out_kappa + 4 * (size_t)E.def_vars[d], E.kappa[d].v, 32);
+        for (uint64_t e = E.def_start[d]; e < E.def_start[d + 1]; ++e, ++t) {
+            out_term_v[t] = E.def_vars[d];
+            out_term_f[t] = E.term_f[e];
+            memcpy(out_term_coef + 4 * t, E.term_c[e].v, 32);
+        }
+    }
+    *out_n_terms = t;
+    return ZKT_OK;
+}
+
+}
+
+using namespace zkt;
+
+int zkt_debug_wire_elimination(int curve, const uint64_t* const* selectors, const uint32_t* w_l, const uint32_t* w_r, const uint32_t* w_o,
+                               size_t n_rows, size_t n_vars, const size_t* pi_pos, size_t n_pi, int K, uint8_t* out_kind,
+                               uint32_t* out_free, size_t* out_n_free, uint32_t* out_term_v, uint32_t* out_term_f,
+                               uint64_t* out_term_coef, size_t* out_n_terms, uint64_t* out_kappa) {
+    if (!selectors || !out_kind || !out_free || !out_n_free || !out_term_v || !out_term_f || !out_term_coef || !out_n_terms || !out_kappa ||
+        (n_pi && !pi_pos) || (n_rows && (!w_l || !w_r || !w_o)))
+        return ZKT_ERR_INVALID_ARGUMENT;
+    for (int k = 0; k < 5; ++k)
+        if (n_rows && !selectors[k]) return ZKT_ERR_INVALID_ARGUMENT;
+    if (K < 1 || K > WIRE_ELIM_K_MAX || n_vars > 0xFFFFFFFEull) return ZKT_ERR_INVALID_ARGUMENT;
+    const uint32_t* w[3] = {w_l, w_r, w_o};
+    if (curve == ZKT_CURVE_BN254)
+        return debug_wire_elimination_t<Bn254Fr>(selectors, w, n_rows, n_vars, pi_pos, n_pi, K, out_kind, out_free, out_n_free, out_term_v,
+                                                 out_term_f, out_term_coef, out_n_terms, out_kappa);
+    if (curve == ZKT_CURVE_BLS12_381)
+        return debug_wire_elimination_t<Bls381Fr>(selectors, w, n_rows, n_vars, pi_pos, n_pi, K, out_kind, out_free, out_n_free, out_term_v,
+                                                  out_term_f, out_term_coef, out_n_terms, out_kappa);
+    return ZKT_ERR_INVALID_ARGUMENT;
+}
diff --git a/zkt-plonk_amd/csrc/msm.hpp b/zkt-plonk_amd/csrc/msm.hpp
--- a/zkt-plonk_amd/csrc/msm.hpp
+++ b/zkt-plonk_amd/csrc/msm.hpp
@@ -63,6 +63,10 @@
     uint32_t* u[3] = {};
     size_t cnt[3] = {};
     bool use[3] = {};
+    bool elim[3] = {};
+    bool has_c[3] = {};
+    bool elim_wanted = false;
+    std::vector<size_t> pi_pos;
     bool built = false;
     bool borrowed = false;
     bool stale = false;
@@ -90,7 +94,9 @@
     uint64_t* wb_dig = nullptr;
     uint64_t* wb_pin = nullptr;
     const void* tbl_table(int tbl) const { return tbl >= MSM_TBL_WIRE ? wb.table[tbl - MSM_TBL_WIRE] : tbl ? table2 : table; }
-    size_t tbl_count(int tbl) const { return tbl >= MSM_TBL_WIRE ? wb.cnt[tbl - MSM_TBL_WIRE] + 2 : tbl ? count2 : count; }
+    size_t tbl_count(int tbl) const {
+        return tbl >= MSM_TBL_WIRE ? wb.cnt[tbl - MSM_TBL_WIRE] + (wb.has_c[tbl - MSM_TBL_WIRE] ? 1 : 0) + 2 : tbl ? count2 : count;
+    }
     uint32_t* params[11] = {};
     uint32_t* vals2 = nullptr;
     void* pairs = nullptr;
@@ -165,8 +171,14 @@
 int lagrange_ensure(zkt_ctx* c, int log_n);
 bool lagrange_ready(const zkt_ctx* c, int log_n);
 size_t lagrange_bases(const zkt_ctx* c);
-int wire_bases_prepare(zkt_ctx* c, int log_n, const uint32_t* const* d_idx, size_t n_rows, size_t n_vars);
+struct WireElimKeys {
+    const void* pk[5];
+    const size_t* pi_pos;
+    size_t n_pi;
+};
+int wire_bases_prepare(zkt_ctx* c, int log_n, const uint32_t* const* d_idx, size_t n_rows, size_t n_vars, const WireElimKeys* elim = nullptr);
 bool wire_bases_use(const zkt_ctx* c, int k);
+int wire_bases_route(const zkt_ctx* c, int k);
 int wire_bases_digest(zkt_ctx* c, const uint32_t* const* d_idx, size_t n_rows);
 int wire_bases_lens(zkt_ctx* c, const uint32_t* d_lens);
 int wire_bases_scalars(zkt_ctx* c, int k, const void* d_vars, const void* d_blinders, size_t n, const void** out, size_t* len);
diff --git a/zkt-plonk_amd/csrc/poly.hpp b/zkt-plonk_amd/csrc/poly.hpp
--- a/zkt-plonk_amd/csrc/poly.hpp
+++ b/zkt-plonk_amd/csrc/poly.hpp
@@ -83,6 +83,7 @@
     const void* q_lookup_ev;
     const void* sigma_ev[3];
 };
+int selector_evals_enqueue(zkt_ctx* c, int log_n, const void* const* pk, void* const* outs);
 int witness_check(zkt_ctx* c, const WitnessCheckKeys& keys, const zkt_prove_inputs& in, int flags, zkt_witness_report* out);
 int gen_powers(zkt_ctx* c, void* out, size_t n, const uint32_t base[8], const uint32_t scale[8]);
 int lookup_count(zkt_ctx* c, const void* f, size_t n, const void* d_sorted_keys, const uint32_t* d_perm, uint32_t nkeys,
diff --git a/zkt-plonk_amd/csrc/prover.hip b/zkt-plonk_amd/csrc/prover.hip
--- a/zkt-plonk_amd/csrc/prover.hip
+++ b/zkt-plonk_amd/csrc/prover.hip
@@ -78,6 +78,7 @@
     bool keys_borrowed = false;
     bool wire_route[3] = {};
     bool wire_dense_only = false;
+    int wire_elim_force = -1;
 };
 
 template <class P>
@@ -128,6 +129,8 @@
     out.insert(out.end(), b.begin(), b.end());
 }
 
+constexpr int WIRE_ELIM_MIN_LOG_N = 17;
+
 template <class C>
 struct Prover {
     using R = typename C::Fr;
@@ -272,7 +275,7 @@
             if (took) took[k] = 0;
             if (!routed) continue;
             if (wire_bases_check(c, k, S.n)) {
-                if (took) took[k] = 1;
+                if (took) took[k] = wire_bases_route(c, k);
                 continue;
             }
             static const int slot[1] = {0};
@@ -482,7 +485,13 @@
         bool wire_tables = from_vars && in.wires_on_device && !c->sharded() && !c->lagrange_off && !S.wire_dense_only &&
                            lagrange_ready(c, S.log_n) && in.n_rows > 0;
         if (wire_tables) {
-            if ((rc = wire_bases_prepare(c, S.log_n, d_idx, in.n_rows, in.n_vars))) return rc;
+            const bool eliminate = S.wire_elim_force >= 0 ? S.wire_elim_force != 0
+                                                          : c->wire_elim_mode == 2 || (c->wire_elim_mode == 1 && S.log_n >= WIRE_ELIM_MIN_LOG_N);
+            WireElimKeys ek{};
+            for (int k = 0; k < 5; ++k) ek.pk[k] = S.pk[PK_QM + k];
+            ek.pi_pos = in.pi_pos;
+            ek.n_pi = in.pi_pos ? in.n_pi : 0;
+            if ((rc = wire_bases_prepare(c, S.log_n, d_idx, in.n_rows, in.n_vars, eliminate ? &ek : nullptr))) return rc;
             wire_tables = wire_bases_use(c, 0) || wire_bases_use(c, 1) || wire_bases_use(c, 2);
             if (wire_tables && (rc = wire_bases_digest(c, d_idx, in.n_rows))) return rc;
         }
@@ -1534,6 +1543,14 @@
     return ZKT_OK;
 }
 
+int zkt_ctx_set_wire_elimination(zkt_ctx* c, int mode) {
+    if (!c) return ZKT_ERR_INVALID_ARGUMENT;
+    if (mode < 0 || mode > 2) return set_err(c, ZKT_ERR_INVALID_ARGUMENT, "mode: 0 off, 1 automatic, 2 whenever a table can be built");
+    c->wire_elim_mode = mode;
+    ++c->msm_epoch;
+    return ZKT_OK;
+}
+
 int zkt_lagrange_info(zkt_ctx* c, int* log_n, size_t* bases) {
     if (!c) return ZKT_ERR_INVALID_ARGUMENT;
     const bool ready = c->circuit && lagrange_ready(c, c->circuit->log_n) && !c->lagrange_off;
@@ -1855,8 +1872,10 @@
     MerlinHostTranscript tr("zkt_debug_commit_wires_dev");
     Prover<C> p(c, S, tr);
     S.wire_dense_only = route == 0;
+    S.wire_elim_force = route == 2 ? 1 : 0;
     int rc = p.enqueue_round_1(in);
     S.wire_dense_only = false;
+    S.wire_elim_force = -1;
     Affine<Q> cm[3];
     static const int slots[3] = {0, 1, 2};
     int took[3] = {0, 0, 0};
@@ -1881,8 +1900,17 @@
 int zkt_debug_commit_wires_dev(zkt_ctx* c, const void* d_variables, size_t n_vars, const uint32_t* d_w_l, const uint32_t* d_w_r,
                                const uint32_t* d_w_o, size_t n_rows, const uint64_t* blinders, int route, uint64_t* out_xy,
                                int* out_is_infinity, int* out_route) {
-    if (!c || !d_variables || !blinders || !out_xy) return set_err(c, ZKT_ERR_INVALID_ARGUMENT, "null pointer");
     if (route != 0 && route != 1) return set_err(c, ZKT_ERR_INVALID_ARGUMENT, "route: 0 coefficients, 1 wire base tables");
+    return zkt_debug_commit_wires_pi_dev(c, d_variables, n_vars, d_w_l, d_w_r, d_w_o, n_rows, blinders, route, nullptr, 0, out_xy,
+                                         out_is_infinity, out_route);
+}
+
+int zkt_debug_commit_wires_pi_dev(zkt_ctx* c, const void* d_variables, size_t n_vars, const uint32_t* d_w_l, const uint32_t* d_w_r,
+                                  const uint32_t* d_w_o, size_t n_rows, const uint64_t* blinders, int route, const size_t* pi_pos,
+                                  size_t n_pi, uint64_t* out_xy, int* out_is_infinity, int* out_route) {
+    if (!c || !d_variables || !blinders || !out_xy || (n_pi && !pi_pos)) return set_err(c, ZKT_ERR_INVALID_ARGUMENT, "null pointer");
+    if (route < 0 || route > 2)
+        return set_err(c, ZKT_ERR_INVALID_ARGUMENT, "route: 0 coefficients, 1 wire base tables, 2 tables over free variables");
     if (!c->circuit) return set_err(c, ZKT_ERR_NOT_LOADED, "no circuit loaded (the domain comes from it)");
     if (!c->msm) return set_err(c, ZKT_ERR_NOT_LOADED, "no SRS loaded (zkt_srs_load)");
     if (c->sharded()) return set_err(c, ZKT_ERR_INVALID_ARGUMENT, "not available on a sharded key");
@@ -1890,7 +1918,7 @@
     if (S.has_next) return set_err(c, ZKT_ERR_INVALID_ARGUMENT, "zkt_debug_commit_wires_dev: a next proof is announced");
     (void)hipSetDevice(c->device);
     S.prefetch_stage = 0;
-    if (route == 1 && !c->lagrange_off)
+    if (route >= 1 && !c->lagrange_off)
         if (int rc1 = lagrange_ensure(c, S.log_n)) return rc1;
     uint64_t bl[19 * 4] = {};
     memcpy(bl, blinders, 6 * 32);
@@ -1901,6 +1929,8 @@
     in.n_rows = n_rows;
     in.wires_on_device = 1;
     in.blinders = bl;
+    in.pi_pos = pi_pos;
+    in.n_pi = n_pi;
     if (c->curve == ZKT_CURVE_BN254) return debug_commit_wires_t<Bn254Curve>(c, in, route, out_xy, out_is_infinity, out_route);
     return debug_commit_wires_t<Bls381Curve>(c, in, route, out_xy, out_is_infinity, out_route);
 }
diff --git a/zkt-plonk_amd/csrc/wire_elim.hpp b/zkt-plonk_amd/csrc/wire_elim.hpp
--- /dev/null
+++ b/zkt-plonk_amd/csrc/wire_elim.hpp
@@ -0,0 +1,103 @@
+#pragma once
+#include "fp.hpp"
+
+#include <cstddef>
+#include <cstdint>
+#include <vector>
+
+namespace zkt {
+
+constexpr int WIRE_ELIM_K = 16;
+constexpr int WIRE_ELIM_K_MAX = 64;
+
+template <class R>
+struct WireElim {
+    using F = Fe<R>;
+    std::vector<uint8_t> kind;
+    std::vector<uint32_t> free_vars;
+    std::vector<uint32_t> def_vars;
+    std::vector<uint32_t> def_id;
+    std::vector<uint64_t> def_start;
+    std::vector<uint32_t> term_f;
+    std::vector<F> term_c;
+    std::vector<F> kappa;
+};
+
+template <class R>
+void wire_eliminate(const Fe<R>* const* sel, const uint32_t* const* w, size_t n_rows, size_t n_vars, const size_t* pi_pos, size_t n_pi,
+                    int K, WireElim<R>& E) {
+    using F = Fe<R>;
+    E = WireElim<R>{};
+    E.kind.assign(n_vars, 0);
+    E.def_id.assign(n_vars, 0);
+    E.def_start.push_back(0);
+    std::vector<bool> is_pi(n_rows, false);
+    for (size_t k = 0; k < n_pi; ++k)
+        if (pi_pos[k] < n_rows) is_pi[pi_pos[k]] = true;
+    const F one = fe_one<R>(), minus_one = fe_neg<R>(fe_one<R>());
+    auto touch = [&](uint32_t v) {
+        if (v < n_vars && E.kind[v] == 0) {
+            E.kind[v] = 1;
+            E.free_vars.push_back(v);
+        }
+    };
+    uint32_t fa[WIRE_ELIM_K_MAX], fb[WIRE_ELIM_K_MAX], fo[2 * WIRE_ELIM_K_MAX];
+    F ca[WIRE_ELIM_K_MAX], cb[WIRE_ELIM_K_MAX], co[2 * WIRE_ELIM_K_MAX];
+    for (size_t i = 0; i < n_rows; ++i) {
+        const uint32_t a = w[0][i], b = w[1][i], o = w[2][i];
+        const F qo = sel[3][i];
+        const bool plus = fe_eq<R>(qo, one);
+        const bool cand = o < n_vars && E.kind[o] == 0 && o != a && o != b && !is_pi[i] && fe_is_zero<R>(sel[0][i]) &&
+                          (plus || fe_eq<R>(qo, minus_one));
+        touch(a);
+        touch(b);
+        if (!cand) {
+            touch(o);
+            continue;
+        }
+        F kap = plus ? fe_neg<R>(sel[4][i]) : sel[4][i];
+        auto scaled = [&](uint32_t v, const F& q, uint32_t* f, F* cf) -> int {
+            if (v >= n_vars || fe_is_zero<R>(q)) return 0;
+            const F s = plus ? fe_neg<R>(q) : q;
+            if (E.kind[v] == 1) {
+                f[0] = v;
+                cf[0] = s;
+                return 1;
+            }
+            const uint32_t d = E.def_id[v];
+            int m = 0;
+            for (uint64_t t = E.def_start[d]; t < E.def_start[d + 1]; ++t, ++m) {
+                f[m] = E.term_f[t];
+                cf[m] = fe_mul<R>(s, E.term_c[t]);
+            }
+            kap = fe_add<R>(kap, fe_mul<R>(s, E.kappa[d]));
+            return m;
+        };
+        const int na = scaled(a, sel[1][i], fa, ca), nb = scaled(b, sel[2][i], fb, cb);
+        int ia = 0, ib = 0, no = 0;
+        while (ia < na || ib < nb) {
+            if (ib == nb || (ia < na && fa[ia] < fb[ib])) {
+                fo[no] = fa[ia]; co[no++] = ca[ia++];
+            } else if (ia == na || fb[ib] < fa[ia]) {
+                fo[no] = fb[ib]; co[no++] = cb[ib++];
+            } else {
+                const F s = fe_add<R>(ca[ia], cb[ib]);
+                if (!fe_is_zero<R>(s)) { fo[no] = fa[ia]; co[no++] = s; }
+                ++ia; ++ib;
+            }
+        }
+        if (no > K) {
+            touch(o);
+            continue;
+        }
+        E.kind[o] = 2;
+        E.def_id[o] = (uint32_t)E.def_vars.size();
+        E.def_vars.push_back(o);
+        E.term_f.insert(E.term_f.end(), fo, fo + no);
+        E.term_c.insert(E.term_c.end(), co, co + no);
+        E.def_start.push_back(E.term_f.size());
+        E.kappa.push_back(kap);
+    }
+}
+
+}
```

Result: faster. 60.98 proofs/s, median of 6 (+10.1%).
